# blairstar/NaturalDiffusion

Hardware: AMD Instinct MI355X
Metric: images/sec at 15-step Natural Inference (CIFAR10 32x32, NCSN++), 3-stream throughput (higher is better)
Workload: dtype bf16; 1 GPU; CIFAR10 NI 15-step step_15_weight_173.npz B=512/GPU NCSN++ 61.8M bf16, ni_step fp64 history; nfe=15, batch_per_gpu=512, streams=3

## Files before the change

### include/natinf_ncsnpp.h

```cpp
#ifndef NATINF_NCSNPP_H
#define NATINF_NCSNPP_H

#include <stdint.h>
#include "natinf.h"

#ifdef __cplusplus
extern "C" {
#endif

typedef struct natinf_ncsnpp* natinf_ncsnpp_t;

#define NATINF_NCSNPP_KEEP_ACTIVATIONS 1
#define NATINF_NCSNPP_DDPM 2

int64_t natinf_ncsnpp_param_count(void);
int64_t natinf_ncsnpp_packed_bytes(void);
int64_t natinf_ncsnpp_handle_param_count(natinf_ncsnpp_t h);
int64_t natinf_ncsnpp_handle_packed_bytes(natinf_ncsnpp_t h);
int64_t natinf_ncsnpp_workspace_bytes(natinf_ncsnpp_t h, int max_batch);

int natinf_ncsnpp_create(natinf_ncsnpp_t* out, int flags);
int natinf_ncsnpp_destroy(natinf_ncsnpp_t h);

int natinf_ncsnpp_describe(natinf_ncsnpp_t h, char* buf, int cap);

int natinf_ncsnpp_load(natinf_ncsnpp_t h, const float* params_f32, int64_t n_params,
                       void* packed, int64_t packed_bytes, natinf_stream_t stream);

int natinf_ncsnpp_share(natinf_ncsnpp_t h, natinf_ncsnpp_t loaded);

int natinf_ncsnpp_forward(natinf_ncsnpp_t h, const float* x, const float* labels, float* out, int B,
                          void* workspace, int64_t workspace_bytes, natinf_stream_t stream);

int natinf_ncsnpp_describe_gemms(natinf_ncsnpp_t h, int B, char* buf, int cap);

int natinf_debug_gemm(int variant, int M, int N, int K0, int K1, int taps, int logW, int batch,
                      const void* a0, const void* a1, const void* b, const float* bias_n, void* c, int c_f32, float scale,
                      int iters, natinf_stream_t stream);
int natinf_debug_quant_fp8_rows(const float* w, void* q, float* row_scale, int rows, int cols, natinf_stream_t stream);
int natinf_debug_gemm_fused(int variant, int M, int N, int K, const void* a, const void* b, const float* bias_n, const float* bias_m,
                            const float* rowvec, const float* gate, int log_rows_per_sample, const void* resid_bf16, const float* resid_f32,
                            float scale, int act, void* c, int c_f32, float* gn_part, int* bm_out, int fp32_slab, natinf_stream_t stream);
int natinf_debug_set_conv_operand(int logW, const void* a1, int c1);
int natinf_debug_gemm_fp8(int M, int N, int K, const void* a8, const float* a_scale, const void* a_mx, const void* b8, const float* b_scale,
                          const float* bias_n, void* c, void* c_mx, int c_mode, int iters, natinf_stream_t stream);
int natinf_debug_conv_gn_up(int flags);
int natinf_debug_conv_gn(int res, int B, int N, int cin, int c1, const void* x, const float* scale, const float* shift, const void* w_packed, void* w_frag,
                         const void* a1, const float* bias_n, const void* resid, float out_scale, void* out, float* gn_part, int iters,
                         natinf_stream_t stream);
#define NATINF_ATTN_BLOCK_OFF_WQKV 0
#define NATINF_ATTN_BLOCK_OFF_W3 393216
#define NATINF_ATTN_BLOCK_OFF_FOLD_WQK 524288
#define NATINF_ATTN_BLOCK_OFF_FOLD_WVO 786432
#define NATINF_ATTN_BLOCK_OFF_FOLD_CQ 1048576
#define NATINF_ATTN_BLOCK_OFF_FOLD_BO 1049600
#define NATINF_ATTN_BLOCK_OFF_WQK_PACKED 1050624
#define NATINF_ATTN_BLOCK_OFF_WVO_PACKED 1181696
#define NATINF_ATTN_BLOCK_PACKED_BYTES 1312768
#define NATINF_ATTN_BLOCK_SCRATCH_BYTES_PER_SAMPLE 393216
int natinf_debug_attn_block(int plan, int B, const void* x, int x_ld, const float* scale, const float* shift, const float* w, const float* bias,
                            void* packed, void* scratch, void* out, int o_ld, float out_scale, float* gn_part, natinf_stream_t stream);
int natinf_set_gemm_variant(int variant);
int natinf_set_gemm_epilogue(int fp32_slab);
int natinf_set_gemm_pref512(int on);
int natinf_set_gemm_half_issue(int on);
int natinf_set_gemm_round_model(int on);
int natinf_set_gemm_w128(int on);
int natinf_set_gemm_raster(int rows);
int natinf_set_fuse_gn(int on);
int natinf_set_conv_gn_wide(int mask);
int natinf_set_conv_gn_w128(int mask);
int natinf_set_conv_gn_w128_min_k(int shape, int k);
int natinf_set_conv_gn_regw(int on);
int natinf_set_fuse_up(int on);
int natinf_set_fuse_head(int on);
int natinf_set_fuse_gn8(int on);
int natinf_set_fuse_gn4(int on);
int natinf_set_fuse_fin(int on);
int natinf_set_conv_gn_warm(int mask);
int natinf_set_attn256(int on);
int natinf_set_attn_proj(int on);
int natinf_set_attn_waves8(int on);
int natinf_set_attn_block(int on);
int natinf_set_attn_qkv(int on);
int natinf_set_conv_gn8_tile(int one_image);
int natinf_set_gemm_splitk(int on);
int natinf_debug_set_splitk_workspace(float* ws, int max_slices);
int natinf_debug_timestamps(void* dev_buf16);

int natinf_ncsnpp_profile(natinf_ncsnpp_t h, int enable);
int natinf_ncsnpp_profile_read(natinf_ncsnpp_t h, double* ms_by_class , int64_t* launches_by_class );

int natinf_gemm_profile(int enable);
int natinf_gemm_profile_read(char* buf, int cap);

int natinf_ncsnpp_debug_tap(natinf_ncsnpp_t h, int module_idx, float* out, int64_t capacity_elems,
                            natinf_stream_t stream);

#ifdef __cplusplus
}
#endif
#endif
```

### naturaldiffusion_amd/_lib.py

```python
from __future__ import annotations

import ctypes as C
import os
from pathlib import Path

os.environ.setdefault("GPU_MAX_HW_QUEUES", "8")

_HERE = Path(__file__).resolve().parent
LIB_PATH = Path(os.environ.get("NATINF_LIB", _HERE / "libnatinf.so"))

if not LIB_PATH.exists():
    raise ImportError(
        f"{LIB_PATH} not found: build it with `make -C {_HERE / 'csrc'}` "
        "(or `python -c 'import __graft_entry__ as g; g.build()'`). "
        "naturaldiffusion_amd has no CPU or eager-PyTorch fallback.")

lib = C.CDLL(str(LIB_PATH))

_p, _i32, _i64, _f32, _f64 = C.c_void_p, C.c_int, C.c_int64, C.c_float, C.c_double

SIGNATURES = {
    "natinf_abi_version": (C.c_int, []),
    "natinf_strerror": (C.c_char_p, [_i32]),
    "natinf_probe": (C.c_int, []),
    "natinf_step_f64hist": (C.c_int, [_p, _p, _p, _p, _p, _p, _p, _i32, _f64, _i32, _f64, _f64, _f32, _f32, _i64, _p]),
    "natinf_step_f32hist": (C.c_int, [_p, _p, _p, _p, _p, _p, _p, _i32, _f32, _i32, _f32, _f32, _f32, _f32, _i64, _p]),
    "natinf_weighted_sum_f64": (C.c_int, [_p, _p, _p, _p, _i32, _i64, _p]),
    "natinf_randn_philox_f32": (C.c_int, [_p, _i64, _i64, _p, _i64, _i64, C.c_uint64, _p]),
    "natinf_randn_philox_col_f32": (C.c_int, [_p, _i64, _i64, _p, _i64, _i64, C.c_uint64, C.c_uint32, _p]),
    "natinf_step_f64hist_noise": (C.c_int, [_p, _p, _p, _p, _p, _p, _p, _i32, _f64, _p, _p, _i32, _i32, _f64, _f64, _f32,
                                            C.c_uint64, _p, _i64, _i64, _i64, _i64, _p]),
    "natinf_known_blend_f32": (C.c_int, [_p, _p, _p, _p, _i64, _i64, _f32, _f32, C.c_uint32, C.c_uint64, _p, _i64, _i64, _i64, _i64, _p]),
    "natinf_step_f64hist_inpaint": (C.c_int, [_p, _p, _p, _p, _p, _p, _p, _i32, _f64, _p, _p, _i32, _i32, _f64, _f64, _f32,
                                              C.c_uint64, _p, _i64, _i64, _i64, _i64, _p, _p, _i64, _i64, _f32, _f32, C.c_uint32, _p]),
    "natinf_color_blend_f32": (C.c_int, [_p, _p, _p, _i64, _p, _p, _f32, _f32, C.c_uint32, C.c_uint64, _p, _i64, _i64, _i64, _i64, _p]),
    "natinf_step_f64hist_colorize": (C.c_int, [_p, _p, _p, _p, _p, _p, _p, _i32, _f64, _p, _p, _i32, _i32, _f64, _f64, _f32,
                                               C.c_uint64, _p, _i64, _i64, _i64, _i64, _p, _i64, _p, _p, _f32, _f32, C.c_uint32, _p]),
    "natinf_to_pixel_u8": (C.c_int, [_p, _p, _i32, _i32, _i32, _i32, _i32, _p]),
    "natinf_step_f32prod": (C.c_int, [_p, _p, _p, _f32, _i64, _i64, _p, _p, _p, _p, _p, _i32, _f32, _p, _p, _i32,
                                      _i32, _f32, _f32, _i64, _p]),
    "natinf_step_f32prod_noise": (C.c_int, [_p, _p, _p, _f32, _i64, _i64, _p, _p, _p, _p, _p, _i32, _f32, _p, _p, _i32,
                                            _i32, _f32, _f32, C.c_uint64, _p, _i64, _i64, _i64, _p]),
    "natinf_step_f32prod_noise_guided": (C.c_int, [_p, _p, _p, _p, _p, _i32, _i64, _i64, _p, _p, _p, _p, _p, _i32, _f32, _p, _p, _i32,
                                                   _i32, _f32, _f32, C.c_uint64, _p, _i64, _i64, _i64, _p]),
    "natinf_weighted_sum_f32prod": (C.c_int, [_p, _p, _p, _p, _i32, _i64, _p]),
    "natinf_step_f16chain": (C.c_int, [_p, _p, _p, _p, _p, _p, _p, _p, _p, _i32, _f32, _f32, _i32, _f32, _f32, _f32,
                                       _f32, _i32, _i64, _p]),
    "natinf_step_f16chain_guided": (C.c_int, [_p, _p, _p, _p, _p, _i32, _i64, _p, _p, _p, _p, _p, _p, _i32, _f32, _f32, _i32, _f32, _f32,
                                              _f32, _i32, _i64, _p]),
    "natinf_weighted_mean_f16": (C.c_int, [_p, _p, _p, _p, _i32, _f32, _i64, _p]),
    "natinf_flow_input_f16": (C.c_int, [_p, _p, _p, _f32, _f32, _i64, _p]),
    "natinf_ncsnpp_param_count": (C.c_int64, []),
    "natinf_ncsnpp_workspace_bytes": (C.c_int64, [_p, _i32]),
    "natinf_ncsnpp_packed_bytes": (C.c_int64, []),
    "natinf_ncsnpp_handle_param_count": (_i64, [_p]),
    "natinf_ncsnpp_handle_packed_bytes": (_i64, [_p]),
    "natinf_ncsnpp_create": (C.c_int, [C.POINTER(_p), _i32]),
    "natinf_ncsnpp_describe": (C.c_int, [_p, C.c_char_p, _i32]),
    "natinf_ncsnpp_destroy": (C.c_int, [_p]),
    "natinf_ncsnpp_load": (C.c_int, [_p, _p, _i64, _p, _i64, _p]),
    "natinf_ncsnpp_share": (C.c_int, [_p, _p]),
    "natinf_ncsnpp_forward": (C.c_int, [_p, _p, _p, _p, _i32, _p, _i64, _p]),
    "natinf_ncsnpp_debug_tap": (C.c_int, [_p, _i32, _p, _i64, _p]),
    "natinf_ncsnpp_describe_gemms": (C.c_int, [_p, _i32, C.c_char_p, _i32]),
    "natinf_debug_gemm": (C.c_int, [_i32, _i32, _i32, _i32, _i32, _i32, _i32, _i32, _p, _p, _p, _p, _p, _i32, _f32, _i32, _p]),
    "natinf_set_gemm_variant": (C.c_int, [_i32]),
    "natinf_debug_timestamps": (C.c_int, [_p]),
    "natinf_set_gemm_epilogue": (C.c_int, [_i32]),
    "natinf_debug_gemm_fused": (C.c_int, [_i32, _i32, _i32, _i32, _p, _p, _p, _p, _p, _p, _i32, _p, _p, _f32, _i32, _p, _i32, _p, _p, _i32, _p]),
    "natinf_set_gemm_pref512": (C.c_int, [_i32]),
    "natinf_set_gemm_half_issue": (C.c_int, [_i32]),
    "natinf_set_gemm_raster": (C.c_int, [_i32]),
    "natinf_set_gemm_round_model": (C.c_int, [_i32]),
    "natinf_set_gemm_w128": (C.c_int, [_i32]),
    "natinf_set_fuse_gn": (C.c_int, [_i32]),
    "natinf_set_conv_gn_wide": (C.c_int, [_i32]),
    "natinf_set_attn_block": (C.c_int, [_i32]),
    "natinf_set_conv_gn_w128": (C.c_int, [_i32]),
    "natinf_set_conv_gn_w128_min_k": (C.c_int, [_i32, _i32]),
    "natinf_set_conv_gn_regw": (C.c_int, [_i32]),
    "natinf_set_fuse_up": (C.c_int, [_i32]),
    "natinf_set_fuse_head": (C.c_int, [_i32]),
    "natinf_set_fuse_gn8": (C.c_int, [_i32]),
    "natinf_set_fuse_gn4": (C.c_int, [_i32]),
    "natinf_set_fuse_fin": (C.c_int, [_i32]),
    "natinf_set_attn_proj": (C.c_int, [_i32]),
    "natinf_set_attn_waves8": (C.c_int, [_i32]),
    "natinf_set_attn_qkv": (C.c_int, [_i32]),
    "natinf_set_conv_gn_warm": (C.c_int, [_i32]),
    "natinf_set_attn256": (C.c_int, [_i32]),
    "natinf_set_conv_gn8_tile": (C.c_int, [_i32]),
    "natinf_set_gemm_splitk": (C.c_int, [_i32]),
    "natinf_debug_set_splitk_workspace": (C.c_int, [_p, _i32]),
    "natinf_debug_set_conv_operand": (C.c_int, [_i32, _p, _i32]),
    "natinf_debug_conv_gn": (C.c_int, [_i32, _i32, _i32, _i32, _i32, _p, _p, _p, _p, _p, _p, _p, _p, _f32, _p, _p, _i32, _p]),
    "natinf_debug_conv_gn_up": (C.c_int, [_i32]),
    "natinf_debug_attn_block": (C.c_int, [_i32, _i32, _p, _i32, _p, _p, _p, _p, _p, _p, _p, _i32, _f32, _p, _p]),
    "natinf_ncsnpp_profile": (C.c_int, [_p, _i32]),
    "natinf_ncsnpp_profile_read": (C.c_int, [_p, C.POINTER(C.c_double), C.POINTER(C.c_int64)]),
    "natinf_debug_quant_fp8_rows": (C.c_int, [_p, _p, _p, _i32, _i32, _p]),
    "natinf_debug_gemm_fp8": (C.c_int, [_i32, _i32, _i32, _p, _p, _p, _p, _p, _p, _p, _p, _i32, _i32, _p]),
    "natinf_dit_create": (C.c_int, [C.POINTER(_p), _i32, _i32, _i32, _i32]),
    "natinf_dit_create_sized": (C.c_int, [C.POINTER(_p), _i32, _i32, _i32, _i32, _i32]),
    "natinf_dit_input_size": (C.c_int, [_p]),
    "natinf_dit_attention_bf16": (C.c_int, [_p, _p, _p, _i32, _p, _i32, _i32, _i32, _i32, _i32, _i32, _p]),
    "natinf_dit_destroy": (C.c_int, [_p]),
    "natinf_dit_param_count": (C.c_int64, [_p]),
    "natinf_dit_packed_bytes": (C.c_int64, [_p]),
    "natinf_dit_workspace_bytes": (C.c_int64, [_p, _i32]),
    "natinf_dit_load": (C.c_int, [_p, _p, _i64, _p, _i64, _p]),
    "natinf_dit_forward": (C.c_int, [_p, _p, _p, _p, _p, _i32, _p, _i64, _p]),
    "natinf_dit_stream_sites": (C.c_int, [_p]),
    "natinf_dit_stream_status_reset": (C.c_int, [_p, _p, _p]),
    "natinf_dit_stream_status": (C.c_int, [_p, _p, _p, _p]),
    "natinf_mmdit_create": (C.c_int, [C.POINTER(_p), _i32, _i32, _i32, _i32, _i32, _i32, _i32, _i32]),
    "natinf_mmdit_destroy": (C.c_int, [_p]),
    "natinf_mmdit_param_count": (C.c_int64, [_p]),
    "natinf_mmdit_packed_bytes": (C.c_int64, [_p]),
    "natinf_mmdit_workspace_bytes": (C.c_int64, [_p, _i32]),
    "natinf_mmdit_load": (C.c_int, [_p, _p, _i64, _p, _i64, _p]),
    "natinf_mmdit_forward": (C.c_int, [_p, _p, _p, _p, _p, _p, _i32, _p, _i64, _p]),
    "natinf_mmdit_stream_sites": (C.c_int, [_p]),
    "natinf_mmdit_stream_status_reset": (C.c_int, [_p, _p, _p]),
    "natinf_mmdit_stream_status": (C.c_int, [_p, _p, _p, _p]),
    "natinf_attention_hd64_bf16": (C.c_int, [_p, _p, _i32, _i64, _p, _p, _i32, _i64, _i32, _i32, _i32, _i32, C.c_float, _p]),
    "natinf_inception_create": (C.c_int, [_p, _i32, _i32]),
    "natinf_inception_destroy": (C.c_int, [_p]),
    "natinf_set_inception_conv": (C.c_int, [_i32]),
    "natinf_debug_conv_ring": (C.c_int, [_i32] * 14 + [_p, _p, _p, _p, _p, _p, _i32, _p]),
    "natinf_inception_param_count": (_i64, [_p]),
    "natinf_inception_packed_bytes": (_i64, [_p]),
    "natinf_inception_workspace_bytes": (_i64, [_p, _i32]),
    "natinf_inception_load": (C.c_int, [_p, _p, _i64, _p, _i64, _p]),
    "natinf_inception_forward": (C.c_int, [_p, _p, _i32, _p, _i32, _p, _i64, _p]),
    "natinf_gemm_profile": (C.c_int, [_i32]),
    "natinf_gemm_profile_read": (C.c_int, [_p, _i32]),
    "natinf_set_mmdit_stream16": (C.c_int, [_i32]),
    "natinf_set_dit_stream16": (C.c_int, [_i32]),
    "natinf_set_mmdit_text_flat": (C.c_int, [_i32]),
    "natinf_attention_profile": (C.c_int, [_i32]),
    "natinf_set_mmdit_text_stream": (C.c_int, [_i32]),
    "natinf_set_flash_mode": (C.c_int, [_i32]),
    "natinf_attention_profile_read": (C.c_int, [_p, _p]),
    "natinf_vae_create": (C.c_int, [C.POINTER(_p), _i32, _i32]),
    "natinf_vae_destroy": (C.c_int, [_p]),
    "natinf_vae_param_count": (C.c_int64, [_p]),
    "natinf_vae_packed_bytes": (C.c_int64, [_p]),
    "natinf_vae_workspace_bytes": (C.c_int64, [_p, _i32]),
    "natinf_vae_load": (C.c_int, [_p, _p, _i64, _p, _i64, _p]),
    "natinf_vae_decode": (C.c_int, [_p, _p, _p, _i32, _p, _i64, _p]),
    "natinf_vae_enc_create": (C.c_int, [C.POINTER(_p), _i32, _i32]),
    "natinf_vae_enc_destroy": (C.c_int, [_p]),
    "natinf_vae_enc_param_count": (C.c_int64, [_p]),
    "natinf_vae_enc_packed_bytes": (C.c_int64, [_p]),
    "natinf_vae_enc_workspace_bytes": (C.c_int64, [_p, _i32]),
    "natinf_vae_enc_load": (C.c_int, [_p, _p, _i64, _p, _i64, _p]),
    "natinf_vae_posterior_f32": (C.c_int, [_p, _p, _i64, _i32, _i64, _i32, _f32, _f32, C.c_uint64, _p, _i64, _i64, _p]),
    "natinf_vae_encode": (C.c_int, [_p, _p, _p, _p, _i32, _i32, _f32, _f32, C.c_uint64, _p, _i64, _i64, _p, _i64, _p]),
}

for _name, (_res, _args) in SIGNATURES.items():
    try:
        _fn = getattr(lib, _name)
    except AttributeError as e:
        raise ImportError(f"{LIB_PATH} does not export {_name}; rebuild it") from e
    _fn.restype, _fn.argtypes = _res, _args

SD3_CFG_ON_VELOCITY = 1
DIT_UNFUSED_ATTENTION = 1
DIT_FP8 = 2
DIT_STREAM_GUARD = 16
MMDIT_FP8 = 1
MMDIT_STREAM_GUARD = 2


def check(rc: int, what: str) -> None:
    if rc != 0:
        raise RuntimeError(f"{what} failed: {lib.natinf_strerror(rc).decode()} ({rc})")


def stream_ptr(stream=None) -> int:
    import torch
    s = stream if stream is not None else torch.cuda.current_stream()
    return int(s.cuda_stream)


def ptr(t) -> int:
    return 0 if t is None else int(t.data_ptr())


class StreamGuardStatus:
    _guard_api = ""
    guard = False

    def _guard_entry(self, name):
        if not self.guard:
            raise RuntimeError("this engine was created without guard=True: it keeps no stream status")
        return getattr(lib, f"{self._guard_api}_{name}")

    @property
    def site_names(self):
        n = self._guard_entry("stream_sites")(self._h)
        check(min(n, 0), f"{self._guard_api}_stream_sites")
        return ["patch_embed"] + [f"blocks.{i // 2}.{'mlp' if i % 2 else 'attn'}" for i in range(n - 1)]

    def reset_stream_status(self) -> None:
        import torch
        with torch.cuda.device(self._ws.device):
            check(self._guard_entry("stream_status_reset")(self._h, ptr(self._ws), stream_ptr()), f"{self._guard_api}_stream_status_reset")

    def stream_status(self):
        import torch
        n = len(self.site_names)
        buf = torch.empty(2 * n, dtype=torch.int32, device=self._ws.device)
        with torch.cuda.device(self._ws.device):
            check(self._guard_entry("stream_status")(self._h, ptr(self._ws), ptr(buf), stream_ptr()), f"{self._guard_api}_stream_status")
        raw = buf.cpu().numpy().view("uint32").reshape(n, 2)
        return {"max_abs": raw[:, 0].copy().view("float32"), "clamped": raw[:, 1].copy()}


def require_gpu() -> None:
    import torch
    if not torch.cuda.is_available():
        raise RuntimeError("naturaldiffusion_amd needs an MI355X (gfx950) GPU: torch.cuda.is_available() is False "
                           "and there is no CPU fallback")
    check(lib.natinf_probe(), "natinf_probe")
```

### naturaldiffusion_amd/csrc/gemm_dma.h

```cpp
#pragma once
#include "ncsnpp_kernels.h"

#ifndef NATINF_SETPRIO
#define NATINF_SETPRIO 0
#endif

namespace ncsn {

template <int WM, int WN, int TM, int TN, int AVAIL>
struct EpiCfg {
    static constexpr int CROW = WN * TN * 16 + 4;
    static constexpr int bytes(int rb) { return WM * rb * 16 * CROW * 4; }
    static constexpr int RB = bytes(TM) <= AVAIL ? TM : (bytes(TM / 2) <= AVAIL ? TM / 2 : (bytes(TM / 4) <= AVAIL ? TM / 4 : 1));
    static constexpr int SLAB_ROWS = WM * RB * 16;
    static constexpr int SLAB_BYTES = bytes(RB);
    static_assert(TM % RB == 0 && SLAB_BYTES <= AVAIL, "epilogue staging does not fit");
    static constexpr int PROW = WN * TN * 16 * 2 + 16;
    static constexpr int PACK_SLAB = WM * TM * 16 * PROW;
    static constexpr int PACK_BYTES = PACK_SLAB + WM * WN * TN * 4 * 8;
    static constexpr bool PACK_OK = PACK_BYTES <= AVAIL;
    static constexpr int NEED = PACK_OK && PACK_BYTES > SLAB_BYTES ? PACK_BYTES : SLAB_BYTES;
};

template <int WM, int WN, int TM, int TN>
struct DmaCfg {
    static constexpr int NW = WM * WN, THREADS = NW * 64;
    static constexpr int BM_ = WM * TM * 16, BN_ = WN * TN * 16;
    static constexpr int STAGE_BYTES = (BM_ + BN_) * BK * 2;
    static constexpr int PA = BM_ / 8 / NW, PB = BN_ / 8 / NW;
    using Epi = EpiCfg<WM, WN, TM, TN, 2 * STAGE_BYTES + 8192>;
    static constexpr int LDS_BYTES = Epi::NEED > 2 * STAGE_BYTES ? Epi::NEED : 2 * STAGE_BYTES;
    static_assert(BM_ % (8 * NW) == 0 && BN_ % (8 * NW) == 0, "DMA pieces must divide evenly over the waves");
};

#ifdef NATINF_DEV
#define NATINF_TS(i) do { if (g.dbg_ts && tid == 0 && blockIdx.x == 0) g.dbg_ts[i] = __builtin_amdgcn_s_memtime(); } while (0)
#else
#define NATINF_TS(i) do { } while (0)
#endif
__device__ __forceinline__ float dpp_row_sum(float v) {
    asm volatile("s_nop 4" : "+v"(v));
    v += __builtin_bit_cast(float, __builtin_amdgcn_update_dpp(0, __builtin_bit_cast(int, v), 0xB1, 0xF, 0xF, true));
    asm volatile("" : "+v"(v));
    v += __builtin_bit_cast(float, __builtin_amdgcn_update_dpp(0, __builtin_bit_cast(int, v), 0x4E, 0xF, 0xF, true));
    asm volatile("" : "+v"(v));
    v += __builtin_bit_cast(float, __builtin_amdgcn_update_dpp(0, __builtin_bit_cast(int, v), 0x141, 0xF, 0xF, true));
    asm volatile("" : "+v"(v));
    v += __builtin_bit_cast(float, __builtin_amdgcn_update_dpp(0, __builtin_bit_cast(int, v), 0x140, 0xF, 0xF, true));
    asm volatile("" : "+v"(v));
    return v;
}
typedef __bf16 bf16x4_t __attribute__((ext_vector_type(4)));
template <class T> __device__ __forceinline__ __attribute__((address_space(1))) T* as_global(T* p) { return (__attribute__((address_space(1))) T*)p; }
typedef unsigned gu32x4 __attribute__((ext_vector_type(4)));
typedef float gf32x4 __attribute__((ext_vector_type(4)));
__device__ __forceinline__ uint4 gload_u4(const void* p) { const gu32x4 t = *as_global(reinterpret_cast<const gu32x4*>(p)); return make_uint4(t[0], t[1], t[2], t[3]); }
__device__ __forceinline__ float4 gload_f4(const void* p) { const gf32x4 t = *as_global(reinterpret_cast<const gf32x4*>(p)); return make_float4(t[0], t[1], t[2], t[3]); }
__device__ __forceinline__ void gstore_u4(void* p, uint4 v) { *as_global(reinterpret_cast<gu32x4*>(p)) = gu32x4{v.x, v.y, v.z, v.w}; }
template <int SW, int NSW, int RPS, int PROW, bool EDGE>
struct SlabCopy {
    template <class T>
    static __device__ __forceinline__ void run(const unsigned char* src, T* dst, int64_t ld, int m, int M) {
        const uint4 v = *reinterpret_cast<const uint4*>(src + SW * RPS * PROW);
        SlabCopy<SW + 1, NSW, RPS, PROW, EDGE>::run(src, dst, ld, m, M);
        if (!EDGE || m + SW * RPS < M) gstore_u4(dst + (int64_t)(SW * RPS) * ld, v);
    }
};
template <int NSW, int RPS, int PROW, bool EDGE>
struct SlabCopy<NSW, NSW, RPS, PROW, EDGE> {
    template <class T> static __device__ __forceinline__ void run(const unsigned char*, T*, int64_t, int, int) {}
};
template <int WM, int WN, int TM, int TN, class Cfg, int ACT, bool GN, bool RES, bool DEQ = false, bool OUT8 = false, int NSAMP = 1, bool FIN = false, bool PAIR = false, bool SCALE_ALWAYS = false>
__device__ __forceinline__ void packed_tile_epilogue(const GemmArgs& g, unsigned char* smem, f32x4 (&acc)[TM][TN],
                                                     int m0, int n0, int z, int tid, int lane, int wm, int wn)
{
    constexpr int BN_ = WN * TN * 16, BM_ = WM * TM * 16, THREADS = WM * WN * 64, PROW = OUT8 ? BN_ + 16 : Cfg::PROW;
    static_assert(!OUT8 || (!GN && !RES && TN % 2 == 0), "fp8 output: plain column terms only");
    static_assert(!PAIR || (TN % 2 == 0 && !OUT8 && !DEQ), "interleaved n-tile pairs: bf16 output");
    static_assert(NSAMP == 1 || ((NSAMP == 2 || NSAMP == 4) && WM == 1 && TM % NSAMP == 0 && !DEQ && !OUT8), "several samples per tile: one wave row, bf16 output");
    constexpr bool ACT8 = (ACT == ACT_GELU_TANH || ACT == ACT_SILU) && !GN && TN % 2 == 0 && NSAMP == 1;
    const int r = lane & 15, q = lane >> 4;
    auto ncol = [&](int j) __attribute__((always_inline)) { return PAIR ? 32 * (j >> 1) + 8 * q + 4 * (j & 1) : 16 * j + 4 * q; };
    float dn[DEQ ? TN : 1][4], rsc[DEQ ? TM : 1], rbm[DEQ ? TM : 1];
    if constexpr (DEQ) {
#pragma unroll
        for (int j = 0; j < TN; ++j) {
            const int n = n0 + wn * TN * 16 + j * 16 + q * 4;
            float4 d = make_float4(1.f, 1.f, 1.f, 1.f);
            if (g.deq_n && n < g.N) d = *reinterpret_cast<const float4*>(g.deq_n + (int64_t)z * g.deq_n_bs + n);
            dn[j][0] = d.x; dn[j][1] = d.y; dn[j][2] = d.z; dn[j][3] = d.w;
        }
#pragma unroll
        for (int i = 0; i < TM; ++i) {
            const int m = min(m0 + wm * TM * 16 + i * 16 + r, g.M - 1);
            rsc[i] = g.deq_m ? g.deq_m[(int64_t)z * g.deq_m_bs + m] : 1.f;
            rbm[i] = g.bias_m ? g.bias_m[m] : 0.f;
        }
    }
    constexpr bool LAZY_RV = NSAMP > 2 && !RES;
    constexpr int NCT = (NSAMP > 1 && !RES && !LAZY_RV) ? NSAMP : 1;
    float ct[NCT][TN][4];
#pragma unroll
    for (int sm = 0; sm < NCT; ++sm)
#pragma unroll
    for (int j = 0; j < TN; ++j) {
        const int n = n0 + wn * TN * 16 + ncol(j);
        float4 b = make_float4(0.f, 0.f, 0.f, 0.f), rv = make_float4(0.f, 0.f, 0.f, 0.f);
        if (n < g.N) {
            if (g.bias_n) b = gload_f4(g.bias_n + n);
            const int srow = NSAMP > 1 ? min(m0 + sm * (BM_ / NSAMP), g.M - 1) : m0;
            if (g.rowvec && !LAZY_RV) rv = gload_f4(g.rowvec + (int64_t)((srow >> g.log_rows_per_sample) + z * g.z_samples) * g.rowvec_ld + n);
        }
        ct[sm][j][0] = b.x + rv.x; ct[sm][j][1] = b.y + rv.y; ct[sm][j][2] = b.z + rv.z; ct[sm][j][3] = b.w + rv.w;
    }
    uint2 rs[RES ? TM : 1][RES ? TN : 1];
    if constexpr (RES) {
        const bf16* rb = g.resid + (int64_t)z * g.c_bs + n0 + wn * TN * 16;
#pragma unroll
        for (int i = 0; i < TM; ++i) {
            const int m = min(m0 + wm * TM * 16 + i * 16 + r, g.M - 1);
            if constexpr (PAIR) {
#pragma unroll
                for (int p = 0; p < TN / 2; ++p) {
                    const uint4 v = n0 + wn * TN * 16 + ncol(2 * p) < g.N ? gload_u4(rb + (int64_t)m * g.resid_ld + ncol(2 * p)) : make_uint4(0u, 0u, 0u, 0u);
                    rs[i][2 * p] = make_uint2(v.x, v.y); rs[i][2 * p + 1] = make_uint2(v.z, v.w);
                }
            } else {
#pragma unroll
                for (int j = 0; j < TN; ++j)
                    rs[i][j] = n0 + wn * TN * 16 + ncol(j) < g.N ? *reinterpret_cast<const uint2*>(rb + (int64_t)m * g.resid_ld + ncol(j)) : make_uint2(0u, 0u);
            }
        }
    }
    float gs[NSAMP][TN], gq[NSAMP][TN];
#pragma unroll
    for (int sm = 0; sm < NSAMP; ++sm)
#pragma unroll
        for (int j = 0; j < TN; ++j) { gs[sm][j] = 0.f; gq[sm][j] = 0.f; }
    const float scale = g.scale;
    float4 lrv[LAZY_RV ? TN : 1];
    auto fetch_rowvec = [&](int i) __attribute__((always_inline)) {
        if constexpr (LAZY_RV) {
            const int srow = min(m0 + (i / (TM / NSAMP)) * (BM_ / NSAMP), g.M - 1);
#pragma unroll
            for (int j = 0; j < TN; ++j) {
                const int n = n0 + wn * TN * 16 + ncol(j);
                lrv[j] = (g.rowvec && n < g.N) ? *reinterpret_cast<const float4*>(g.rowvec + (int64_t)(srow >> g.log_rows_per_sample) * g.rowvec_ld + n) : make_float4(0.f, 0.f, 0.f, 0.f);
            }
        }
    };
    auto value = [&](int i, int j, float (&v)[4]) __attribute__((always_inline)) {
        const int sm = NSAMP > 1 ? i / (TM / NSAMP) : 0;
        const int sc_ = NCT > 1 ? sm : 0;
#pragma unroll
        for (int e = 0; e < 4; ++e) {
            if constexpr (DEQ) v[e] = __builtin_fmaf(acc[i][j][e] * rsc[i], dn[j][e], ct[sc_][j][e]);
            else v[e] = acc[i][j][e] + ct[sc_][j][e];
        }
        if constexpr (DEQ && !OUT8) {
            if (g.bias_m) {
                asm volatile("");
#pragma unroll
                for (int e = 0; e < 4; ++e) v[e] += rbm[i];
            }
        }
        if constexpr (LAZY_RV) { v[0] += lrv[j].x; v[1] += lrv[j].y; v[2] += lrv[j].z; v[3] += lrv[j].w; }
        if constexpr (RES) {
            const bf16x4_t x = __builtin_bit_cast(bf16x4_t, rs[i][j]);
#pragma unroll
            for (int e = 0; e < 4; ++e) v[e] += (float)x[e];
        }
        if constexpr (SCALE_ALWAYS) {
#pragma unroll
            for (int e = 0; e < 4; ++e) v[e] *= scale;
        } else if (!OUT8 && scale != 1.0f) {
            asm volatile("");
#pragma unroll
            for (int e = 0; e < 4; ++e) v[e] *= scale;
        }
        if constexpr (ACT != ACT_NONE && !ACT8) apply_act4(v, ACT);
        if constexpr (GN) {
            gs[sm][j] += (v[0] + v[1]) + (v[2] + v[3]);
            gq[sm][j] += (v[0] * v[0] + v[1] * v[1]) + (v[2] * v[2] + v[3] * v[3]);
        }
    };
    auto act8 = [&](float (&v0)[4], float (&v1)[4]) __attribute__((always_inline)) {
        float v8[8] = {v0[0], v0[1], v0[2], v0[3], v1[0], v1[1], v1[2], v1[3]};
        if constexpr (ACT == ACT_GELU_TANH) gelu_tanh_fast8(v8); else silu_fast8(v8);
#pragma unroll
        for (int e = 0; e < 4; ++e) { v0[e] = v8[e]; v1[e] = v8[4 + e]; }
    };
    constexpr int EB = OUT8 ? 1 : 2;
    unsigned char* wbase = smem + (wm * TM * 16 + r) * PROW + (wn * TN * 16 + q * 4) * EB;
    if constexpr (!OUT8 && PAIR) {
        unsigned char* wb2 = smem + (wm * TM * 16 + r) * PROW + (wn * TN * 16) * 2;
#pragma unroll
        for (int i = 0; i < TM; ++i) {
            fetch_rowvec(i);
#pragma unroll
            for (int p = 0; p < TN / 2; ++p) {
                float v0[4], v1[4];
                value(i, 2 * p, v0);
                value(i, 2 * p + 1, v1);
                if constexpr (ACT8) act8(v0, v1);
                bf16x4_t o0, o1;
#pragma unroll
                for (int e = 0; e < 4; ++e) { o0[e] = (bf16)v0[e]; o1[e] = (bf16)v1[e]; }
                const uint2 a = __builtin_bit_cast(uint2, o0), b = __builtin_bit_cast(uint2, o1);
                *reinterpret_cast<uint4*>(wb2 + i * 16 * PROW + ncol(2 * p) * 2) = make_uint4(a.x, a.y, b.x, b.y);
            }
        }
    } else if constexpr (!OUT8) {
#pragma unroll
        for (int i = 0; i < TM; ++i) {
            fetch_rowvec(i);
            if constexpr (ACT8) {
#pragma unroll
                for (int j = 0; j < TN; j += 2) {
                    float v0[4], v1[4];
                    value(i, j, v0);
                    value(i, j + 1, v1);
                    act8(v0, v1);
                    bf16x4_t o0, o1;
#pragma unroll
                    for (int e = 0; e < 4; ++e) { o0[e] = (bf16)v0[e]; o1[e] = (bf16)v1[e]; }
                    *reinterpret_cast<uint2*>(wbase + i * 16 * PROW + j * 32) = __builtin_bit_cast(uint2, o0);
                    *reinterpret_cast<uint2*>(wbase + i * 16 * PROW + (j + 1) * 32) = __builtin_bit_cast(uint2, o1);
                }
            } else {
#pragma unroll
            for (int j = 0; j < TN; ++j) {
                float v[4];
                value(i, j, v);
                bf16x4_t o;
#pragma unroll
                for (int e = 0; e < 4; ++e) o[e] = (bf16)v[e];
                *reinterpret_cast<uint2*>(wbase + i * 16 * PROW + j * 32) = __builtin_bit_cast(uint2, o);
            }
            }
        }
    } else {
#pragma unroll
        for (int i = 0; i < TM; ++i) {
            const int m = m0 + wm * TM * 16 + i * 16 + r;
            unsigned e8pair = 0;
#pragma unroll
            for (int b = 0; b < TN / 2; ++b) {
                float v0[4], v1[4];
                value(i, 2 * b, v0);
                value(i, 2 * b + 1, v1);
                if constexpr (ACT8) act8(v0, v1);
                float amax = fmaxf(fmaxf(fmaxf(fabsf(v0[0]), fabsf(v0[1])), fmaxf(fabsf(v0[2]), fabsf(v0[3]))),
                                   fmaxf(fmaxf(fabsf(v1[0]), fabsf(v1[1])), fmaxf(fabsf(v1[2]), fabsf(v1[3]))));
                amax = group4_max_nonneg(amax);
                float inv;
                const unsigned e8 = mx_scale_of(amax, inv);
                *reinterpret_cast<unsigned*>(wbase + i * 16 * PROW + (2 * b) * 16) = pack_fp8x4<false>(v0[0] * inv, v0[1] * inv, v0[2] * inv, v0[3] * inv);
                *reinterpret_cast<unsigned*>(wbase + i * 16 * PROW + (2 * b + 1) * 16) = pack_fp8x4<false>(v1[0] * inv, v1[1] * inv, v1[2] * inv, v1[3] * inv);
                e8pair |= e8 << (8 * b);
            }
            static_assert(TN == 4, "scale bytes are stored as one 16-bit pair per row and wave");
            const int nb = n0 + wn * 64;
            if (q == 0 && m < g.M && nb < g.N)
                *reinterpret_cast<unsigned short*>(g.c_mx + (int64_t)z * g.c_mx_bs + ((int64_t)(nb >> 7) * g.c_mx_ld + m) * 4 + ((nb >> 5) & 3)) = (unsigned short)e8pair;
        }
    }
    float2* const sred = reinterpret_cast<float2*>(smem + Cfg::PACK_SLAB);
    if constexpr (GN) {
#pragma unroll
        for (int sm = 0; sm < NSAMP; ++sm)
#pragma unroll
            for (int j = 0; j < TN; ++j) { gs[sm][j] = dpp_row_sum(gs[sm][j]); gq[sm][j] = dpp_row_sum(gq[sm][j]); }
        if (r == 0) {
#pragma unroll
            for (int sm = 0; sm < NSAMP; ++sm)
#pragma unroll
                for (int j = 0; j < TN; ++j) sred[(NSAMP > 1 ? sm : wm) * (BN_ / 4) + wn * TN * 4 + (ncol(j) >> 2)] = make_float2(gs[sm][j], gq[sm][j]);
        }
    }
    __syncthreads();
    NATINF_TS(3);
    constexpr int CPR = BN_ * EB / 16, RPS = THREADS / CPR, NSW = BM_ / RPS;
    const int cchunk = tid % CPR, rsub = tid / CPR, n = n0 + cchunk * (16 / EB);
    if (n < g.N) {
        const unsigned char* src = smem + rsub * PROW + cchunk * 16;
        if constexpr (OUT8) {
            uint8_t* dst = reinterpret_cast<uint8_t*>(g.c) + (int64_t)z * g.c_bs + (int64_t)(m0 + rsub) * g.c_ld + n;
            if (m0 + BM_ <= g.M) SlabCopy<0, NSW, RPS, PROW, false>::run(src, dst, g.c_ld, m0 + rsub, g.M);
            else SlabCopy<0, NSW, RPS, PROW, true>::run(src, dst, g.c_ld, m0 + rsub, g.M);
        } else {
            bf16* dst = reinterpret_cast<bf16*>(g.c) + (int64_t)z * g.c_bs + (int64_t)(m0 + rsub) * g.c_ld + n;
            if (m0 + BM_ <= g.M) SlabCopy<0, NSW, RPS, PROW, false>::run(src, dst, g.c_ld, m0 + rsub, g.M);
            else SlabCopy<0, NSW, RPS, PROW, true>::run(src, dst, g.c_ld, m0 + rsub, g.M);
        }
    }
    NATINF_TS(4);
    if constexpr (GN) {
        if (tid < BN_ / 4 && n0 + tid * 4 < g.N) {
            if constexpr (NSAMP > 1) {
#pragma unroll
                for (int sm = 0; sm < NSAMP; ++sm)
                    if (m0 + sm * (BM_ / NSAMP) < g.M)
                        reinterpret_cast<float2*>(g.gn_part)[(int64_t)((m0 / BM_) * NSAMP + sm) * g.gn_quads + (n0 >> 2) + tid] = sred[sm * (BN_ / 4) + tid];
            } else {
                float s = 0.f, qq = 0.f;
#pragma unroll
                for (int w = 0; w < WM; ++w) { s += sred[w * (BN_ / 4) + tid].x; qq += sred[w * (BN_ / 4) + tid].y; }
                reinterpret_cast<float2*>(g.gn_part)[(int64_t)(m0 / BM_) * g.gn_quads + (n0 >> 2) + tid] = make_float2(s, qq);
            }
        }
        if constexpr (FIN) {
            static_assert((WM == 1 || NSAMP == 1) && BN_ <= THREADS, "one channel per thread; several samples per tile: one wave row");
            const int n = n0 + tid;
            if (g.fin_scale && tid < BN_ && n < g.N) {
                constexpr int HWS = BM_ / NSAMP;
                const int cg = g.fin_cg, qpg = cg >> 2, q0 = (n / cg) * qpg - (n0 >> 2);
                const float inv = 1.0f / (float)(cg * HWS), ga = g.fin_gamma[n], be = g.fin_beta[n];
#pragma unroll
                for (int sm = 0; sm < NSAMP; ++sm) {
                    if (m0 + sm * HWS >= g.M) break;
                    float s = 0.f, qq = 0.f;
                    for (int i = 0; i < qpg; ++i) {
                        if constexpr (NSAMP == 1 && WM > 1) {
                            float ps = 0.f, pq = 0.f;
#pragma unroll
                            for (int w = 0; w < WM; ++w) { ps += sred[w * (BN_ / 4) + q0 + i].x; pq += sred[w * (BN_ / 4) + q0 + i].y; }
                            s += ps; qq += pq;
                        } else { const float2 v = sred[sm * (BN_ / 4) + q0 + i]; s += v.x; qq += v.y; }
                    }
                    const float mean = s * inv;
                    float var = qq * inv - mean * mean;
                    var = var < 0.f ? 0.f : var;
                    const float sc = (1.0f / sqrtf(var + g.fin_eps)) * ga;
                    const int64_t o = (int64_t)(m0 / HWS + sm) * g.fin_ld + n;
                    g.fin_scale[o] = sc * g.fin_mul;
                    g.fin_shift[o] = (be - mean * sc) * g.fin_mul;
                }
            }
        }
    }
}

template <int WM, int WN, int TM, int TN, class Cfg>
__device__ __forceinline__ void dma_tile_epilogue(const GemmArgs& g, unsigned char* smem, f32x4 (&acc)[TM][TN],
                                                  int m0, int n0, int z, int tid, int lane, int wm, int wn)
{
    constexpr int BN_ = WN * TN * 16, BM_ = WM * TM * 16, THREADS = WM * WN * 64;
    float* sC = reinterpret_cast<float*>(smem);
    NATINF_TS(2);
#ifdef NATINF_DEV
    if (g.c_mode == 102) {
        float t = 0.f;
#pragma unroll
        for (int i = 0; i < TM; ++i)
#pragma unroll
            for (int j = 0; j < TN; ++j) t += acc[i][j][0] + acc[i][j][1] + acc[i][j][2] + acc[i][j][3];
        if (t == 123.456f) reinterpret_cast<float*>(g.c)[tid] = t;
        return;
    }
#endif
    float st[4] = {0.f, 0.f, 0.f, 0.f};
    constexpr int CROW = Cfg::CROW, RB = Cfg::RB, CPR = BN_ / 8;
    constexpr int ROWS_PER_SWEEP = THREADS / CPR;
    constexpr int NP = TM / RB, NSW = Cfg::SLAB_ROWS / ROWS_PER_SWEEP;
    uint4 keep[NSW][2];
    const int cchunk = tid % CPR, rsub = tid / CPR;
    const int n = n0 + cchunk * 8;
    const bool n_in = n < g.N;
    float bn[8];
#pragma unroll
    for (int q = 0; q < 8; ++q) bn[q] = 0.f;
    if (g.bias_n && n_in && g.c_mode != OUT_F32_NCHW) {
        const float4 u = *reinterpret_cast<const float4*>(g.bias_n + n), w = *reinterpret_cast<const float4*>(g.bias_n + n + 4);
        bn[0] = u.x; bn[1] = u.y; bn[2] = u.z; bn[3] = u.w; bn[4] = w.x; bn[5] = w.y; bn[6] = w.z; bn[7] = w.w;
    }
    float dn[8];
#pragma unroll
    for (int q = 0; q < 8; ++q) dn[q] = 1.f;
    if (g.deq_n && n_in) {
        const float* pd = g.deq_n + (int64_t)z * g.deq_n_bs + n;
        const float4 u = *reinterpret_cast<const float4*>(pd), w = *reinterpret_cast<const float4*>(pd + 4);
        dn[0] = u.x; dn[1] = u.y; dn[2] = u.z; dn[3] = u.w; dn[4] = w.x; dn[5] = w.y; dn[6] = w.z; dn[7] = w.w;
    }
    asm volatile("s_waitcnt vmcnt(0)" : "+v"(dn[0]), "+v"(dn[1]), "+v"(dn[2]), "+v"(dn[3]), "+v"(dn[4]), "+v"(dn[5]), "+v"(dn[6]), "+v"(dn[7]));
    asm volatile("s_waitcnt vmcnt(0)" : "+v"(bn[0]), "+v"(bn[1]), "+v"(bn[2]), "+v"(bn[3]), "+v"(bn[4]), "+v"(bn[5]), "+v"(bn[6]), "+v"(bn[7]));
#pragma unroll
    for (int pass = 0; pass < NP; ++pass) {
        if (pass) __syncthreads();
#pragma unroll
        for (int ii = 0; ii < RB; ++ii)
#pragma unroll
            for (int j = 0; j < TN; ++j)
                *reinterpret_cast<f32x4*>(sC + (wm * RB * 16 + ii * 16 + (lane & 15)) * CROW + wn * TN * 16 + j * 16 + (lane >> 4) * 4) = acc[pass * RB + ii][j];
        __syncthreads();
        NATINF_TS(3 + 3 * pass);
        if (g.c_mode == OUT_F32_NCHW) {
            float* out = reinterpret_cast<float*>(g.c);
            const int nvalid = min(BN_, g.N - n0);
            for (int e = tid; e < Cfg::SLAB_ROWS * nvalid; e += THREADS) {
                const int s = e % Cfg::SLAB_ROWS, nn = e / Cfg::SLAB_ROWS;
                const int m = m0 + (s / (RB * 16)) * (TM * 16) + pass * RB * 16 + s % (RB * 16);
                if (m < g.M) {
                    float v = sC[s * CROW + nn];
                    if (g.bias_n) v += g.bias_n[n0 + nn];
                    v *= g.scale;
                    const int b = m >> g.logHW, p = m & ((1 << g.logHW) - 1);
                    out[((int64_t)b * g.N + n0 + nn) * ((int64_t)1 << g.logHW) + p] = v;
                }
            }
            continue;
        }
#pragma unroll
        for (int sw = 0; sw < NSW; ++sw) {
            const int s = sw * ROWS_PER_SWEEP + rsub;
            const int m = m0 + (s / (RB * 16)) * (TM * 16) + pass * RB * 16 + s % (RB * 16);
            if (m >= g.M || !n_in) continue;
            const float4 u = *reinterpret_cast<const float4*>(sC + s * CROW + cchunk * 8);
            const float4 w = *reinterpret_cast<const float4*>(sC + s * CROW + cchunk * 8 + 4);
            float v[8] = {u.x, u.y, u.z, u.w, w.x, w.y, w.z, w.w};
            if (g.deq_m || g.deq_n) {
                const float dm = g.deq_m ? g.deq_m[(int64_t)z * g.deq_m_bs + m] : 1.f;
#pragma unroll
                for (int q = 0; q < 8; ++q) v[q] *= dm * dn[q];
            }
#pragma unroll
            for (int q = 0; q < 8; ++q) v[q] += bn[q];
            if (g.bias_m) {
                const float bm = g.bias_m[m];
#pragma unroll
                for (int q = 0; q < 8; ++q) v[q] += bm;
            }
            if (g.rowvec) {
                const float* rv = g.rowvec + (int64_t)((m >> g.log_rows_per_sample) + z * g.z_samples) * g.rowvec_ld + n;
                const float4 s4 = *reinterpret_cast<const float4*>(rv), t4 = *reinterpret_cast<const float4*>(rv + 4);
                v[0] += s4.x; v[1] += s4.y; v[2] += s4.z; v[3] += s4.w; v[4] += t4.x; v[5] += t4.y; v[6] += t4.z; v[7] += t4.w;
            }
            if (g.gate) {
                const float* gv = g.gate + (int64_t)((m >> g.log_rows_per_sample) + z * g.z_samples) * g.gate_ld + n;
                const float4 s4 = *reinterpret_cast<const float4*>(gv), t4 = *reinterpret_cast<const float4*>(gv + 4);
                v[0] *= s4.x; v[1] *= s4.y; v[2] *= s4.z; v[3] *= s4.w; v[4] *= t4.x; v[5] *= t4.y; v[6] *= t4.z; v[7] *= t4.w;
            }
            if (g.resid) {
                const bf16x8 rs = *reinterpret_cast<const bf16x8*>(g.resid + (int64_t)z * g.c_bs + (int64_t)m * g.resid_ld + n);
#pragma unroll
                for (int q = 0; q < 8; ++q) v[q] += (float)rs[q];
            }
            if (g.resid_f32) {
                const float* rp = g.resid_f32 + (int64_t)z * g.c_bs + (int64_t)m * g.resid_f32_ld + n;
                const float4 s4 = *reinterpret_cast<const float4*>(rp), t4 = *reinterpret_cast<const float4*>(rp + 4);
                v[0] += s4.x; v[1] += s4.y; v[2] += s4.z; v[3] += s4.w; v[4] += t4.x; v[5] += t4.y; v[6] += t4.z; v[7] += t4.w;
            }
#pragma unroll
            for (int q = 0; q < 8; ++q) v[q] *= g.scale;
            apply_act8(v, g.act);
            if (g.gn_part) {
                st[0] += (v[0] + v[1]) + (v[2] + v[3]); st[1] += (v[0] * v[0] + v[1] * v[1]) + (v[2] * v[2] + v[3] * v[3]);
                st[2] += (v[4] + v[5]) + (v[6] + v[7]); st[3] += (v[4] * v[4] + v[5] * v[5]) + (v[6] * v[6] + v[7] * v[7]);
            }
            if (g.c_mode == OUT_BF16) {
                bf16x8 o;
#pragma unroll
// ... 41 lines not shown
    if (g.gn_part) {
        __syncthreads();
        float* sred = reinterpret_cast<float*>(smem);
        *reinterpret_cast<float4*>(sred + (rsub * CPR + cchunk) * 4) = make_float4(st[0], st[1], st[2], st[3]);
        __syncthreads();
        if (tid < CPR * 2 && n0 + tid * 4 < g.N) {
            const int ch = tid >> 1, hf = (tid & 1) * 2;
            float s = 0.f, q = 0.f;
#pragma unroll 4
            for (int r = 0; r < ROWS_PER_SWEEP; ++r) { s += sred[(r * CPR + ch) * 4 + hf]; q += sred[(r * CPR + ch) * 4 + hf + 1]; }
            reinterpret_cast<float2*>(g.gn_part)[(int64_t)(m0 / BM_) * g.gn_quads + (n0 >> 2) + tid] = make_float2(s, q);
        }
    }
}

template <int WM, int WN, int TM, int TN, bool DEQ = false, int HI_ = 0, bool GUARD = false>
__device__ __forceinline__ void direct_f32_epilogue(const GemmArgs& g, f32x4 (&acc)[TM][TN], int m0, int n0, int z, int lane, int wm, int wn)
{
    const int r = lane & 15, q = lane >> 4;
    const int64_t sample = (int64_t)((m0 >> g.log_rows_per_sample) + z * g.z_samples);
    float ct[TN][4], gt[TN][4];
    float dn[DEQ ? TN : 1][4], rsc[DEQ ? TM : 1];
    if constexpr (DEQ) {
#pragma unroll
        for (int j = 0; j < TN; ++j) {
            const int n = n0 + wn * TN * 16 + j * 16 + q * 4;
            float4 d = make_float4(1.f, 1.f, 1.f, 1.f);
            if (g.deq_n && n < g.N) d = *reinterpret_cast<const float4*>(g.deq_n + (int64_t)z * g.deq_n_bs + n);
            dn[j][0] = d.x; dn[j][1] = d.y; dn[j][2] = d.z; dn[j][3] = d.w;
        }
#pragma unroll
        for (int i = 0; i < TM; ++i)
            rsc[i] = g.deq_m ? g.deq_m[(int64_t)z * g.deq_m_bs + min(m0 + wm * TM * 16 + i * 16 + r, g.M - 1)] : 1.f;
    }
    bool n_ok[TN];
#pragma unroll
    for (int j = 0; j < TN; ++j) {
        const int n = n0 + wn * TN * 16 + j * 16 + q * 4;
        n_ok[j] = n < g.N;
        float4 b = make_float4(0.f, 0.f, 0.f, 0.f), rv = make_float4(0.f, 0.f, 0.f, 0.f), gv = make_float4(1.f, 1.f, 1.f, 1.f);
        if (n_ok[j]) {
            if (g.bias_n) b = gload_f4(g.bias_n + n);
            if (g.rowvec) rv = *reinterpret_cast<const float4*>(g.rowvec + sample * g.rowvec_ld + n);
            if (g.gate) gv = *reinterpret_cast<const float4*>(g.gate + sample * g.gate_ld + n);
        }
        ct[j][0] = b.x + rv.x; ct[j][1] = b.y + rv.y; ct[j][2] = b.z + rv.z; ct[j][3] = b.w + rv.w;
        gt[j][0] = gv.x; gt[j][1] = gv.y; gt[j][2] = gv.z; gt[j][3] = gv.w;
    }
    const float scale = g.scale;
    const int64_t eoff = (int64_t)z * g.c_bs + n0 + wn * TN * 16 + q * 4;
    constexpr int HI = HI_ > 0 ? HI_ : (DEQ ? (TM > 2 ? 2 : TM) : (TM > 4 ? TM / 2 : TM));
    typedef _Float16 f16x4_ds __attribute__((ext_vector_type(4)));
    StreamGuardAcc ga;
    auto sweep = [&](auto f16_tag) __attribute__((always_inline)) {
        constexpr bool F16 = decltype(f16_tag)::value;
        const float* rb = g.resid_f32 + eoff;
        float* cb = reinterpret_cast<float*>(g.c) + eoff;
        const _Float16* rbh = reinterpret_cast<const _Float16*>(g.resid_f32) + eoff;
        _Float16* cbh = reinterpret_cast<_Float16*>(g.c) + eoff;
#pragma unroll
        for (int h = 0; h < TM / HI; ++h) {
            f32x4 rs[F16 ? 1 : HI][F16 ? 1 : TN];
            uint2 rh[F16 ? HI : 1][F16 ? TN : 1];
#pragma unroll
            for (int i = 0; i < HI; ++i) {
                const int m = min(m0 + wm * TM * 16 + (h * HI + i) * 16 + r, g.M - 1);
#pragma unroll
                for (int j = 0; j < TN; ++j) {
                    if constexpr (F16) rh[i][j] = n_ok[j] ? *reinterpret_cast<const uint2*>(rbh + (int64_t)m * g.resid_f32_ld + j * 16) : make_uint2(0u, 0u);
                    else rs[i][j] = n_ok[j] ? *reinterpret_cast<const f32x4*>(rb + (int64_t)m * g.resid_f32_ld + j * 16) : f32x4{0.f, 0.f, 0.f, 0.f};
                }
            }
#pragma unroll
            for (int i = 0; i < HI; ++i) {
                const int m = m0 + wm * TM * 16 + (h * HI + i) * 16 + r;
#pragma unroll
                for (int j = 0; j < TN; ++j) {
                    f32x4 v;
                    f16x4_ds xh;
                    if constexpr (F16) xh = __builtin_bit_cast(f16x4_ds, rh[i][j]);
#pragma unroll
                    for (int e = 0; e < 4; ++e) {
                        const float a0 = DEQ ? acc[h * HI + i][j][e] * (rsc[h * HI + i] * dn[j][e]) : acc[h * HI + i][j][e];
                        float x_;
                        if constexpr (F16) x_ = (float)xh[e]; else x_ = rs[i][j][e];
                        v[e] = ((a0 + ct[j][e]) * gt[j][e] + x_) * scale;
                    }
                    if (m < g.M && n_ok[j]) {
                        if constexpr (GUARD) {
#pragma unroll
                            for (int e = 0; e < 4; ++e) v[e] = stream_guard_value<F16>(ga, v[e]);
                        }
                        if constexpr (F16) {
                            const f16x4_ds o = {(_Float16)v[0], (_Float16)v[1], (_Float16)v[2], (_Float16)v[3]};
                            *reinterpret_cast<uint2*>(cbh + (int64_t)m * g.c_ld + j * 16) = __builtin_bit_cast(uint2, o);
                        } else *reinterpret_cast<f32x4*>(cb + (int64_t)m * g.c_ld + j * 16) = v;
                    }
                }
            }
        }
    };
    auto sweep16 = [&]() __attribute__((always_inline)) {
        static_assert(TN % 2 == 0 || TN == 1, "tile pairs");
        const int jt_off = (q & 1) * 16 + (q >> 1) * 8 - q * 4;
        const _Float16* rbh = reinterpret_cast<const _Float16*>(g.resid_f32) + eoff + jt_off;
        _Float16* cbh = reinterpret_cast<_Float16*>(g.c) + eoff + jt_off;
        constexpr int NP = TN / 2 > 0 ? TN / 2 : 1;
#pragma unroll
        for (int h = 0; h < TM / HI; ++h) {
            uint4 rq[HI][NP];
#pragma unroll
            for (int i = 0; i < HI; ++i) {
                const int m = min(m0 + wm * TM * 16 + (h * HI + i) * 16 + r, g.M - 1);
#pragma unroll
                for (int p = 0; p < NP; ++p) rq[i][p] = *reinterpret_cast<const uint4*>(rbh + (int64_t)m * g.resid_f32_ld + p * 32);
            }
#pragma unroll
            for (int i = 0; i < HI; ++i) {
                const int m = m0 + wm * TM * 16 + (h * HI + i) * 16 + r;
#pragma unroll
                for (int p = 0; p < NP; ++p) {
                    auto s0 = __builtin_amdgcn_permlane16_swap(rq[i][p].x, rq[i][p].z, false, false);
                    auto s1 = __builtin_amdgcn_permlane16_swap(rq[i][p].y, rq[i][p].w, false, false);
                    const f16x4_ds x0 = __builtin_bit_cast(f16x4_ds, make_uint2(s0[0], s1[0])), x1 = __builtin_bit_cast(f16x4_ds, make_uint2(s0[1], s1[1]));
                    f16x4_ds o0, o1;
#pragma unroll
                    for (int e = 0; e < 4; ++e) {
                        const float a0 = DEQ ? acc[h * HI + i][2 * p][e] * (rsc[h * HI + i] * dn[2 * p][e]) : acc[h * HI + i][2 * p][e];
                        const float a1 = DEQ ? acc[h * HI + i][2 * p + 1][e] * (rsc[h * HI + i] * dn[2 * p + 1][e]) : acc[h * HI + i][2 * p + 1][e];
                        float v0 = ((a0 + ct[2 * p][e]) * gt[2 * p][e] + (float)x0[e]) * scale, v1 = ((a1 + ct[2 * p + 1][e]) * gt[2 * p + 1][e] + (float)x1[e]) * scale;
                        if constexpr (GUARD) {
                            if (m < g.M) { v0 = stream_guard_value<true>(ga, v0); v1 = stream_guard_value<true>(ga, v1); }
                        }
                        o0[e] = (_Float16)v0;
                        o1[e] = (_Float16)v1;
                    }
                    const uint2 u0 = __builtin_bit_cast(uint2, o0), u1 = __builtin_bit_cast(uint2, o1);
                    auto t0 = __builtin_amdgcn_permlane16_swap(u0.x, u1.x, false, false);
                    auto t1 = __builtin_amdgcn_permlane16_swap(u0.y, u1.y, false, false);
                    if (m < g.M) *reinterpret_cast<uint4*>(cbh + (int64_t)m * g.c_ld + p * 32) = make_uint4(t0[0], t1[0], t0[1], t1[1]);
                }
            }
        }
    };
    if (g.stream_f16) {
        bool wide = false;
        if constexpr (TN % 2 == 0) wide = n0 + (wn + 1) * TN * 16 <= g.N && g.resid_f32_ld % 8 == 0 && g.c_ld % 8 == 0;
        if (wide) { if constexpr (TN % 2 == 0) sweep16(); }
        else sweep(std::integral_constant<bool, true>{});
    } else sweep(std::integral_constant<bool, false>{});
    if constexpr (GUARD) stream_guard_commit(ga, g.stream_guard);
}

template <int WM, int WN, int TM, int TN, class Cfg, int EPI, int NSAMP = 1, bool FIN = false, bool PAIR = false>
__device__ __forceinline__ void tile_epilogue(const GemmArgs& g, unsigned char* smem, f32x4 (&acc)[TM][TN],
                                              int m0, int n0, int z, int tid, int lane, int wm, int wn)
{
    if constexpr (EPI == 0) dma_tile_epilogue<WM, WN, TM, TN, Cfg>(g, smem, acc, m0, n0, z, tid, lane, wm, wn);
    else if constexpr (EPI == 7) direct_f32_epilogue<WM, WN, TM, TN>(g, acc, m0, n0, z, lane, wm, wn);
    else if constexpr (EPI == 10) direct_f32_epilogue<WM, WN, TM, TN, false, 0, true>(g, acc, m0, n0, z, lane, wm, wn);
    else {
        static_assert(Cfg::PACK_OK, "packed epilogue needs the whole bf16 tile in LDS");
        NATINF_TS(2);
        packed_tile_epilogue<WM, WN, TM, TN, Cfg, EPI == 3 ? ACT_SILU : (EPI == 4 ? ACT_GELU_TANH : ACT_NONE), EPI == 2 || EPI == 6, EPI == 5 || EPI == 6, EPI == 8, false, NSAMP, FIN && (EPI == 2 || EPI == 6), PAIR>(
            g, smem, acc, m0, n0, z, tid, lane, wm, wn);
    }
}

typedef unsigned u32x4 __attribute__((ext_vector_type(4)));
template <int OFF> __device__ __forceinline__ u32x4 lds_read16(unsigned addr) {
    u32x4 v;
    asm volatile(NATINF_PAD_PRE "ds_read_b128 %0, %1 offset:%2" NATINF_PAD_POST : "=v"(v) : "v"(addr), "n"(OFF) : "memory");
    return v;
}
template <int N> __device__ __forceinline__ void wait_lgkmcnt() {
    asm volatile("s_waitcnt lgkmcnt(%0)" :: "n"(N) : "memory");
    __builtin_amdgcn_sched_barrier(0);
}
constexpr int pipe_lgkm_after(int TM, int st) {
    int n = 6, pos_fa[40] = {4, 5}, pos_fb1_last = -1;
    for (int s = 0; s <= st; ++s) {
        if (s + 2 < 2 * TM) pos_fa[s + 2] = n++;
        if (s / TM == 0 && s % TM >= TM - 4) pos_fb1_last = n++;
    }
    int need = pos_fa[st];
    if (st >= TM && pos_fb1_last > need) need = pos_fb1_last;
    return n - 1 - need;
}
template <int TM, int ST>
struct PipeStep {
    static __device__ __forceinline__ void run(u32x4 (&fa)[3], u32x4 (&fb)[2][4], f32x4 (&acc)[TM][4],
                                               unsigned a0, unsigned a1, unsigned b1) {
        constexpr int S = 2 * TM, ks = ST / TM, i = ST % TM;
        if constexpr (ST + 2 < S) {
            constexpr int ks2 = (ST + 2) / TM, i2 = (ST + 2) % TM;
            fa[(ST + 2) % 3] = lds_read16<i2 * 2048>(ks2 ? a1 : a0);
        }
        if constexpr (ks == 0 && i >= TM - 4) fb[1][i - (TM - 4)] = lds_read16<(i - (TM - 4)) * 2048>(b1);
        wait_lgkmcnt<pipe_lgkm_after(TM, ST)>();
#pragma unroll
        for (int j = 0; j < 4; ++j)
            acc[i][j] = __builtin_amdgcn_mfma_f32_16x16x32_bf16(__builtin_bit_cast(bf16x8, fb[ks][j]),
                                                                __builtin_bit_cast(bf16x8, fa[ST % 3]), acc[i][j], 0, 0, 0);
        if constexpr (ST + 1 < S) PipeStep<TM, ST + 1>::run(fa, fb, acc, a0, a1, b1);
    }
};

template <int WM, int WN, int TM, int TN, int SPREAD = 0, int EPI = 0>
__global__ __launch_bounds__(WM * WN * 64, 2) void k_gemm_dma(const GemmArgs g)
{
    static_assert(SPREAD == 2 || SPREAD == 6, "the shipped K loops: hand pipeline (2), one issuing wave per SIMD (6)");
    using Cfg = DmaCfg<WM, WN, TM, TN>;
    constexpr int BM_ = Cfg::BM_, BN_ = Cfg::BN_, THREADS = Cfg::THREADS;
    extern __shared__ __attribute__((aligned(16))) unsigned char smem[];
    lds_poison();
    const int tid = threadIdx.x, lane = tid & 63;
    const int wave = __builtin_amdgcn_readfirstlane(tid >> 6);
    const int wm = wave / WN, wn = wave % WN;
    const int nN = (g.N + BN_ - 1) / BN_, nM = (g.M + BM_ - 1) / BM_;
    const int tile = xcd_remap(blockIdx.x, nM * nN);
    NATINF_TS(0);
    int mt_, nt_;
    tile_coords(tile, nM, nN, g.raster_g, mt_, nt_);
    const int m0 = mt_ * BM_, n0 = nt_ * BN_;
    const int z = blockIdx.z;

    const bf16* a0 = g.a0 + (int64_t)z * g.a_bs;
    const bf16* a1 = g.a1 ? g.a1 + (int64_t)z * g.a_bs : nullptr;
    const bf16* bp = g.b + (int64_t)z * g.b_bs;
    const int K0 = g.taps * g.a0_C, K1 = g.a1 ? g.a1_C : 0;
    const int nk0 = K0 / BK, nk = nk0 + K1 / BK;
    const int Wp = (1 << g.logW) + 2, Hp = (1 << (g.logHW - g.logW)) + 2;

    constexpr bool HALF = SPREAD == 6;
    constexpr int PAI = HALF ? 2 * Cfg::PA : Cfg::PA, PBI = HALF ? 2 * Cfg::PB : Cfg::PB;
    const bool issuer = !HALF || wave < Cfg::NW / 2;
    uint64_t a_row[PAI], a_delta[PAI], b_row[PBI];
    typedef __attribute__((address_space(3))) void lds_void;
    const int64_t ashift0 = g.taps == 9 ? (int64_t)(-Wp - 1) * g.a0_ld * 2 : 0;
#pragma unroll
    for (int j = 0; j < PAI; ++j) {
        const int r = (wave * PAI + j) * 8 + (lane >> 3);
        const int lchunk = ((lane & 7) ^ ((r >> 1) & 7)) << 3;
        const int m = min(m0 + r, g.M - 1);
        int64_t off0;
        if (g.taps == 9) {
            const int b = m >> g.logHW, p = m & ((1 << g.logHW) - 1), y = p >> g.logW, x = p & ((1 << g.logW) - 1);
            off0 = ((int64_t)(b * Hp + y + 1) * Wp + x + 1) * g.a0_ld;
        } else {
            off0 = (int64_t)m * g.a0_ld;
        }
        a_row[j] = reinterpret_cast<uint64_t>(a0 + off0 + lchunk);
        a_delta[j] = a1 ? reinterpret_cast<uint64_t>(a1 + (int64_t)m * g.a1_ld + lchunk) - a_row[j] : 0;
        if (issuer)
            __builtin_amdgcn_global_load_lds(reinterpret_cast<const void*>(a_row[j] + (uint64_t)ashift0),
                                             (lds_void*)(smem + wave * (PAI * 1024) + j * 1024), 16, 0, 0);
    }
#pragma unroll
    for (int j = 0; j < PBI; ++j) {
        const int r = (wave * PBI + j) * 8 + (lane >> 3);
        const int lchunk = ((lane & 7) ^ ((r >> 1) & 7)) << 3;
        b_row[j] = reinterpret_cast<uint64_t>(bp + (int64_t)min(n0 + r, g.N - 1) * g.b_ld + lchunk);
        if (issuer)
            __builtin_amdgcn_global_load_lds(reinterpret_cast<const void*>(b_row[j]), (lds_void*)(smem + BM_ * BK * 2 + wave * (PBI * 1024) + j * 1024), 16, 0, 0);
    }

    f32x4 acc[TM][TN];
#pragma unroll
    for (int i = 0; i < TM; ++i)
#pragma unroll
        for (int j = 0; j < TN; ++j) acc[i][j] = f32x4{0.f, 0.f, 0.f, 0.f};

    asm volatile("s_waitcnt vmcnt(0)" ::: "memory");
    __syncthreads();
    NATINF_TS(1);

    const int frow = lane & 15, fq = lane >> 4, fswz = (frow >> 1) & 7;
    constexpr int NP = PAI + PBI;
    for (int kt = 0; kt < nk; ++kt) {
        const int cur = kt & 1;
        const bool more = kt + 1 < nk;
        const int kn = kt + 1;
        const bool seg0n = kn < nk0;
        int64_t ashiftn; int kkn;
        if (seg0n) {
            int tap = 0, c0 = kn * BK;
            if (g.taps == 9) { const int cch = kn / 9; tap = kn - 9 * cch; c0 = cch * BK; }
            const int dy = g.taps == 9 ? tap / 3 - 1 : 0, dx = g.taps == 9 ? tap % 3 - 1 : 0;
            ashiftn = ((int64_t)(dy * Wp + dx) * g.a0_ld + c0) * 2; kkn = kn * BK;
        } else {
            ashiftn = (int64_t)(kn - nk0) * BK * 2; kkn = K0 + (kn - nk0) * BK;
        }
        unsigned char* dAn = smem + (cur ^ 1) * Cfg::STAGE_BYTES + wave * (PAI * 1024);
        unsigned char* dBn = smem + (cur ^ 1) * Cfg::STAGE_BYTES + BM_ * BK * 2 + wave * (PBI * 1024);
        auto issue_piece = [&](int p) __attribute__((always_inline)) {
            if (p < PAI) {
                const uint64_t pa = a_row[p] + (seg0n ? 0 : a_delta[p]) + (uint64_t)ashiftn;
                __builtin_amdgcn_global_load_lds(reinterpret_cast<const void*>(pa), (lds_void*)(dAn + p * 1024), 16, 0, 0);
            } else {
                const uint64_t pb = b_row[p - PAI] + (uint64_t)kkn * 2;
                __builtin_amdgcn_global_load_lds(reinterpret_cast<const void*>(pb), (lds_void*)(dBn + (p - PAI) * 1024), 16, 0, 0);
            }
        };
        if (more && issuer) {
#pragma unroll
            for (int p = 0; p < NP; ++p) issue_piece(p);
        }
        const bf16* ta = reinterpret_cast<const bf16*>(smem + cur * Cfg::STAGE_BYTES) + (wm * TM * 16 + frow) * LDS_ROW;
        const bf16* tb = reinterpret_cast<const bf16*>(smem + cur * Cfg::STAGE_BYTES + BM_ * BK * 2) + (wn * TN * 16 + frow) * LDS_ROW;
        {
            static_assert(TN == 4, "the hand-counted pipeline is written for TN = 4");
            typedef __attribute__((address_space(3))) unsigned char lds_u8;
            const unsigned a_lds = (unsigned)(uintptr_t)((lds_u8*)(unsigned char*)const_cast<bf16*>(ta));
            const unsigned b_lds = (unsigned)(uintptr_t)((lds_u8*)(unsigned char*)const_cast<bf16*>(tb));
            const unsigned ko0 = ((0 | fq) ^ fswz) << 4, ko1 = ((4 | fq) ^ fswz) << 4;
            u32x4 fa[3], fb[2][4];
            fb[0][0] = lds_read16<0>(b_lds + ko0); fb[0][1] = lds_read16<2048>(b_lds + ko0);
            fb[0][2] = lds_read16<4096>(b_lds + ko0); fb[0][3] = lds_read16<6144>(b_lds + ko0);
            fa[0] = lds_read16<0>(a_lds + ko0); fa[1] = lds_read16<2048>(a_lds + ko0);
            PipeStep<TM, 0>::run(fa, fb, acc, a_lds + ko0, a_lds + ko1, b_lds + ko1);
        }
        asm volatile("s_waitcnt vmcnt(0)" ::: "memory");
        __syncthreads();
    }
    tile_epilogue<WM, WN, TM, TN, typename Cfg::Epi, EPI>(g, smem, acc, m0, n0, z, tid, lane, wm, wn);
}


template <int WM, int WN, int TM, int TN, int NS>
struct RingCfg {
    static constexpr int BKR = 32;
    static constexpr int NW = WM * WN, THREADS = NW * 64;
    static constexpr int BM_ = WM * TM * 16, BN_ = WN * TN * 16;
    static constexpr int STAGE_BYTES = (BM_ + BN_) * BKR * 2;
    static constexpr int PA = BM_ / 16 / NW, PB = BN_ / 16 / NW;
    static constexpr int DPT = PA + PB;
    using Epi = EpiCfg<WM, WN, TM, TN, NS * STAGE_BYTES + 4096>;
    static constexpr int LDS_BYTES = Epi::NEED > NS * STAGE_BYTES ? Epi::NEED : NS * STAGE_BYTES;
    static_assert(BM_ % (16 * NW) == 0 && BN_ % (16 * NW) == 0, "DMA pieces must divide evenly over the waves");
    static_assert((NS - 2) * DPT <= 63 && NS >= 3, "vmcnt immediate is 6 bits");
};

template <int N> __device__ __forceinline__ void wait_vmcnt_barrier() {
    asm volatile("s_waitcnt vmcnt(%0)\n\ts_barrier" :: "n"(N) : "memory");
}

template <int WM, int WN, int TM, int TN, int NS, int EPI = 0>
__global__ __launch_bounds__(WM * WN * 64, 2) void k_gemm_ring(const GemmArgs g)
{
    using Cfg = RingCfg<WM, WN, TM, TN, NS>;
    constexpr int BM_ = Cfg::BM_, BN_ = Cfg::BN_, BKR = Cfg::BKR, ROW = 32;
    extern __shared__ __attribute__((aligned(16))) unsigned char smem[];
    lds_poison();
    const int tid = threadIdx.x, lane = tid & 63;
    const int wave = __builtin_amdgcn_readfirstlane(tid >> 6);
    const int wm = wave / WN, wn = wave % WN;
    const int nN = (g.N + BN_ - 1) / BN_, nM = (g.M + BM_ - 1) / BM_;
    const int tile = xcd_remap(blockIdx.x, nM * nN);
    int mt_, nt_;
    tile_coords(tile, nM, nN, g.raster_g, mt_, nt_);
    const int m0 = mt_ * BM_, n0 = nt_ * BN_;
    const int z = EPI == 9 ? 0 : blockIdx.z;

    const bf16* a0 = g.a0 + (int64_t)z * g.a_bs;
    const bf16* a1 = g.a1 ? g.a1 + (int64_t)z * g.a_bs : nullptr;
    const bf16* bp = g.b + (int64_t)z * g.b_bs;
    const int K0 = g.taps * g.a0_C, K1 = g.a1 ? g.a1_C : 0;
    const int nk0 = K0 / BKR, nk_all = nk0 + K1 / BKR;
    const int Wp = (1 << g.logW) + 2, Hp = (1 << (g.logHW - g.logW)) + 2;
    const int kt_lo = EPI == 9 ? (int)((int64_t)nk_all * blockIdx.z / g.splitk) : 0;
    const int nk = EPI == 9 ? (int)((int64_t)nk_all * (blockIdx.z + 1) / g.splitk) - kt_lo : nk_all;

    uint64_t a_row[Cfg::PA], a_delta[Cfg::PA], b_row[Cfg::PB];
#pragma unroll
    for (int j = 0; j < Cfg::PA; ++j) {
        const int r = (wave * Cfg::PA + j) * 16 + (lane >> 2);
        const int t4 = (r >> 2) & 3;
        const int lchunk = ((lane & 3) ^ ((0x1320 >> (t4 * 4)) & 3)) << 3;
        const int m = min(m0 + r, g.M - 1);
        int64_t off0;
        if (g.taps == 9) {
            const int b = m >> g.logHW, p = m & ((1 << g.logHW) - 1), y = p >> g.logW, x = p & ((1 << g.logW) - 1);
            off0 = ((int64_t)(b * Hp + y + 1) * Wp + x + 1) * g.a0_ld;
        } else {
            off0 = (int64_t)m * g.a0_ld;
        }
        a_row[j] = reinterpret_cast<uint64_t>(a0 + off0 + lchunk);
        a_delta[j] = a1 ? reinterpret_cast<uint64_t>(a1 + (int64_t)m * g.a1_ld + lchunk) - a_row[j] : 0;
    }
#pragma unroll
    for (int j = 0; j < Cfg::PB; ++j) {
        const int r = (wave * Cfg::PB + j) * 16 + (lane >> 2);
        const int t4 = (r >> 2) & 3;
        const int lchunk = ((lane & 3) ^ ((0x1320 >> (t4 * 4)) & 3)) << 3;
        b_row[j] = reinterpret_cast<uint64_t>(bp + (int64_t)min(n0 + r, g.N - 1) * g.b_ld + lchunk);
    }

    typedef __attribute__((address_space(3))) void lds_void;
    auto issue_tile = [&](int kt_rel) __attribute__((always_inline)) {
        const int slot = kt_rel % NS, kt = kt_lo + kt_rel;
        unsigned char* dA = smem + slot * Cfg::STAGE_BYTES + wave * (Cfg::PA * 1024);
        unsigned char* dB = smem + slot * Cfg::STAGE_BYTES + BM_ * BKR * 2 + wave * (Cfg::PB * 1024);
        const bool seg0 = kt < nk0;
        int64_t ashift;
        if (seg0) {
            int tap = 0, c0 = kt * BKR;
            if (g.taps == 9) { const int q = kt >> 1, cch = q / 9; tap = q - 9 * cch; c0 = cch * 64 + (kt & 1) * BKR; }
            const int dy = g.taps == 9 ? tap / 3 - 1 : 0, dx = g.taps == 9 ? tap % 3 - 1 : 0;
            ashift = ((int64_t)(dy * Wp + dx) * g.a0_ld + c0) * 2;
        } else {
            ashift = (int64_t)(kt - nk0) * BKR * 2;
        }
        const uint64_t kk2 = (uint64_t)kt * BKR * 2;
#pragma unroll
        for (int j = 0; j < Cfg::PA; ++j) {
            const uint64_t pa = a_row[j] + (seg0 ? 0 : a_delta[j]) + (uint64_t)ashift;
            __builtin_amdgcn_global_load_lds(reinterpret_cast<const void*>(pa), (lds_void*)(dA + j * 1024), 16, 0, 0);
        }
#pragma unroll
        for (int j = 0; j < Cfg::PB; ++j)
            __builtin_amdgcn_global_load_lds(reinterpret_cast<const void*>(b_row[j] + kk2), (lds_void*)(dB + j * 1024), 16, 0, 0);
    };

    f32x4 acc[TM][TN];
#pragma unroll
    for (int i = 0; i < TM; ++i)
#pragma unroll
        for (int j = 0; j < TN; ++j) acc[i][j] = f32x4{0.f, 0.f, 0.f, 0.f};

#pragma unroll
    for (int t = 0; t < NS - 1; ++t)
        if (t < nk) issue_tile(t);

    const int frow = lane & 15, fq = lane >> 4;
    const int fko = (fq ^ ((0x1320 >> (((frow >> 2) & 3) * 4)) & 3)) << 3;
    for (int kt = 0; kt < nk; ++kt) {
        if (kt + NS - 1 <= nk) wait_vmcnt_barrier<(NS - 2) * Cfg::DPT>();
        else                   wait_vmcnt_barrier<0>();
        if (kt + NS - 1 < nk) issue_tile(kt + NS - 1);
        const int slot = kt % NS;
        const bf16* ta = reinterpret_cast<const bf16*>(smem + slot * Cfg::STAGE_BYTES) + (wm * TM * 16 + frow) * ROW + fko;
        const bf16* tb = reinterpret_cast<const bf16*>(smem + slot * Cfg::STAGE_BYTES + BM_ * BKR * 2) + (wn * TN * 16 + frow) * ROW + fko;
        bf16x8 fb[TN];
#pragma unroll
        for (int j = 0; j < TN; ++j) fb[j] = *reinterpret_cast<const bf16x8*>(tb + j * 16 * ROW);
#if NATINF_SETPRIO
        __builtin_amdgcn_s_setprio(1);
#endif
#pragma unroll
        for (int i = 0; i < TM; ++i) {
            const bf16x8 fa = *reinterpret_cast<const bf16x8*>(ta + i * 16 * ROW);
#pragma unroll
            for (int j = 0; j < TN; ++j)
                acc[i][j] = __builtin_amdgcn_mfma_f32_16x16x32_bf16(fb[j], fa, acc[i][j], 0, 0, 0);
        }
#if NATINF_SETPRIO
        __builtin_amdgcn_s_setprio(0);
#endif
    }
    __syncthreads();
    if constexpr (EPI == 9) {
        float* part = reinterpret_cast<float*>(g.c) + (int64_t)blockIdx.z * g.M * g.N;
        const int r = lane & 15, q = lane >> 4;
#pragma unroll
        for (int i = 0; i < TM; ++i) {
            const int m = m0 + wm * TM * 16 + i * 16 + r;
#pragma unroll
            for (int j = 0; j < TN; ++j) {
                const int n = n0 + wn * TN * 16 + j * 16 + q * 4;
                if (m < g.M && n < g.N) *reinterpret_cast<f32x4*>(part + (int64_t)m * g.N + n) = acc[i][j];
            }
        }
    } else {
        tile_epilogue<WM, WN, TM, TN, typename Cfg::Epi, EPI>(g, smem, acc, m0, n0, z, tid, lane, wm, wn);
    }
}

constexpr int SPLITK_ROWS = 16;
__global__ __launch_bounds__(256) void k_splitk_reduce(const float* __restrict__ part, int S, int M, int N, const float* __restrict__ bias_n,
// ... 57 lines not shown
```

### naturaldiffusion_amd/csrc/gemm_launch.h

```cpp
#pragma once
#include <hip/hip_runtime.h>
#include <stdint.h>
#include <stdio.h>
#include <string.h>
#include <string>
#include <type_traits>
#include <utility>
#include <vector>

#include "ncsnpp_kernels.h"
#include "gemm_dma.h"
#include "gemm_w128.h"
#include "conv_gn2.h"
#include "gemm_fp8.h"

using namespace ncsn;

bool configure_conv_ring();
namespace { bool configure_ncsnpp_kernels();
            bool configure_dit_attention();
            bool configure_flash_attention(); }
namespace ncsn_sg { bool configure(); bool has_tile(int variant); void launch_tile(const void* gemm_args, int variant, int raster, void* stream);
                    void launch_fp8(const void* gemm_args, int mxa, int w128, int raster, void* stream); void launch_splitk_reduce(const void* gemm_args, int slices, void* stream);
                    void launch_patch_embed(const float* z, const float* Wt, const float* bias, const float* pos, float* x, int C, int g, int D, int64_t rows, int x_f16, uint32_t* guard, void* stream); }
namespace ncsn_cg3 { bool configure(); int tile_rows(int shape); int tile_cols(int shape); void launch(const void* gemm_args, int shape, int epi, void* stream); }

namespace {

int g_epi_fp32_slab = 0;
GemmArgs gemm_defaults() {
    GemmArgs g;
    memset(&g, 0, sizeof(g));
    g.epi_fp32_slab = g_epi_fp32_slab;
    g.taps = 1; g.batch = 1; g.scale = 1.0f; g.act = ACT_NONE; g.c_mode = OUT_BF16;
    return g;
}
constexpr int NUM_CU = 256;
enum GemmVariant {
    V_AUTO = 0, V_GENERIC = 1,
    V_DMA_256x256 = 2, V_DMA_256x128 = 3, V_DMA_128x128 = 4,
    V_RING_256x256 = 5, V_RING_256x128 = 6, V_RING_128x128 = 7,
    V_RING_64x128 = 8,
    V_RING_256x128_W4 = 9,
    V_DMA_256x128_W4 = 10,
    V_DMA_256x256_S = 11, V_DMA_128x128_S = 12,
    V_DMA_512x128 = 13,
    V_PATCH_256x256 = 14, V_PATCH_256x128 = 15,
    V_DMA_256x256_P = 16, V_DMA_256x128W4_P = 18,
    V_DMA_128x128_P = 17,
    V_8PH_256x256 = 19, V_8PH_NOPRIO = 20, V_8PH_READFIRST = 21, V_8PH_BOTH = 22,
    V_FP8_256x256 = 23,
    V_ABL_NODMA = 24, V_ABL_NOMFMA = 25,
    V_DMA_256x256_H = 26, V_DMA_512x128_H = 27,
    V_CONV_GN = 28,
    V_W128 = 29,
    V_W128_A = 30, V_W128_D = 31, V_W128_X = 32,
    V_COUNT
};
const char* variant_name(int v) {
    static const char* n[] = {"auto", "generic128", "dma256x256", "dma256x128", "dma128x128", "ring256x256", "ring256x128",
                              "ring128x128", "ring64x128", "ring256x128w4", "dma256x128w4", "dma256x256s", "dma128x128s", "dma512x128", "patch256x256", "patch256x128", "dma256x256p", "dma128x128p", "dma256x128w4p", "gemm8ph", "gemm8ph_np", "gemm8ph_rf", "gemm8ph_nprf", "fp8_256x256", "abl_nodma", "abl_nomfma", "dma256x256h", "dma512x128h", "conv_gn", "w128_256x256", "w128_a", "w128_d", "w128_x"};
    return v >= 0 && v < V_COUNT ? n[v] : "?";
}
unsigned long long* g_dbg_ts = nullptr;
int g_force_variant = V_AUTO;
int g_round_model = 1;
int g_round_model_w128 = 13;
int g_pref_512 = 1;
std::string* g_record = nullptr;

int g_raster_g = 8;
template <class Cfg, class K>
inline void launch_tiles(K kernel, const GemmArgs& g0, hipStream_t s) {
    const int nM = (g0.M + Cfg::BM_ - 1) / Cfg::BM_, nN = (g0.N + Cfg::BN_ - 1) / Cfg::BN_;
    GemmArgs g = g0;
    g.raster_g = (g_raster_g > 1 && nN >= 8 && nM >= g_raster_g) ? g_raster_g : 0;
    hipLaunchKernelGGL(kernel, dim3(nM * nN, 1, g.batch), dim3(Cfg::THREADS), Cfg::LDS_BYTES, s, g);
}
template <class Cfg, class K>
inline bool set_lds(K kernel) {
    return hipFuncSetAttribute(reinterpret_cast<const void*>(kernel), hipFuncAttributeMaxDynamicSharedMemorySize, Cfg::LDS_BYTES) == hipSuccess;
}
int g_cg_warm = 15;

constexpr unsigned EPI_ALL = 0x1FF;
template <unsigned MASK, int E, class F> inline void epi_case(F&& f) { if constexpr ((MASK >> E) & 1u) f(std::integral_constant<int, E>{}); }
template <unsigned MASK, class F> inline bool for_each_epi(F&& f) {
    bool ok = true;
    auto one = [&](auto tag) { ok = ok && f(tag); };
    epi_case<MASK, 0>(one); epi_case<MASK, 1>(one); epi_case<MASK, 2>(one); epi_case<MASK, 3>(one); epi_case<MASK, 4>(one);
    epi_case<MASK, 5>(one); epi_case<MASK, 6>(one); epi_case<MASK, 7>(one); epi_case<MASK, 8>(one);
    return ok;
}
#define NATINF_EPI_OF(tag) decltype(tag)::value

template <class... F> struct FamList {};
template <class Fam> bool configure_family() {
    return for_each_epi<Fam::EPI>([](auto t) { return set_lds<typename Fam::Cfg>(Fam::template kernel<NATINF_EPI_OF(t)>()); });
}
template <class... F> bool configure_families(FamList<F...>) { return (configure_family<F>() && ...); }
template <class Fam> void launch_family(int e, const GemmArgs& g, hipStream_t s) {
    for_each_epi<Fam::EPI>([&](auto t) {
        if (NATINF_EPI_OF(t) != e) return true;
        launch_tiles<typename Fam::Cfg>(Fam::template kernel<NATINF_EPI_OF(t)>(), g, s);
        return false;
    });
}

using CfgD256x256 = DmaCfg<2, 4, 8, 4>;
struct FamD128  { static constexpr int V = V_DMA_128x128_P;    using Cfg = DmaCfg<2, 2, 4, 4>;     static constexpr unsigned EPI = EPI_ALL;
                  template <int E> static constexpr auto kernel() { return &k_gemm_dma<2, 2, 4, 4, 2, E>; } };
struct FamRW4   { static constexpr int V = V_RING_256x128_W4;  using Cfg = RingCfg<2, 2, 8, 4, 3>; static constexpr unsigned EPI = EPI_ALL & ~(1u << 3);
                  template <int E> static constexpr auto kernel() { return &k_gemm_ring<2, 2, 8, 4, 3, E>; } };
struct FamR64   { static constexpr int V = V_RING_64x128;      using Cfg = RingCfg<2, 2, 2, 4, 4>; static constexpr unsigned EPI = EPI_ALL;
                  template <int E> static constexpr auto kernel() { return &k_gemm_ring<2, 2, 2, 4, 4, E>; } };
struct FamD256H { static constexpr int V = V_DMA_256x256_H;    using Cfg = CfgD256x256;            static constexpr unsigned EPI = EPI_ALL & ~(1u << 3);
                  template <int E> static constexpr auto kernel() { return &k_gemm_dma<2, 4, 8, 4, 6, E>; } };
struct FamD512H { static constexpr int V = V_DMA_512x128_H;    using Cfg = DmaCfg<4, 2, 8, 4>;     static constexpr unsigned EPI = EPI_ALL & ~((1u << 3) | (1u << 4) | (1u << 7) | (1u << 8));
                  template <int E> static constexpr auto kernel() { return &k_gemm_dma<4, 2, 8, 4, 6, E>; } };
struct FamW128  { static constexpr int V = V_W128;             using Cfg = W128Cfg;                static constexpr unsigned EPI = EPI_ALL & ~((1u << 2) | (1u << 3) | (1u << 6));
                  template <int E> static constexpr auto kernel() { return &k_gemm_w128<E>; } };
using GemmFamilies = FamList<FamD128, FamRW4, FamR64, FamD256H, FamD512H, FamW128>;
using CfgR128x128 = RingCfg<2, 2, 4, 4, 4>;

template <class F, class... Fam> constexpr bool with_family(int v, F&& f, FamList<Fam...>) { return ((v == Fam::V && (f(Fam{}), true)) || ...); }
template <class F> constexpr bool with_family(int v, F&& f) { return with_family(v, f, GemmFamilies{}); }
constexpr bool variant_shipped(int v) {
    return v == V_AUTO || v == V_GENERIC || v == V_FP8_256x256 || v == V_CONV_GN || with_family(v, [](auto) {});
}
constexpr unsigned epi_mask(int v) { unsigned m = 1u; with_family(v, [&](auto f) { m = decltype(f)::EPI; }); return m; }
constexpr int variant_bm(int v) {
    int bm = (v == V_CONV_GN || v == V_FP8_256x256) ? 256 : 128;
    with_family(v, [&](auto f) { bm = decltype(f)::Cfg::BM_; });
    return bm;
}
static_assert(variant_bm(V_RING_64x128) == 64 && variant_bm(V_DMA_128x128_P) == 128 && variant_bm(V_RING_256x128_W4) == 256 && variant_bm(V_DMA_256x256_H) == 256 &&
              variant_bm(V_DMA_512x128_H) == 512 && variant_bm(V_W128) == 256 && variant_bm(V_GENERIC) == 128, "the block-tile rows choose_variant and the GroupNorm partial tables count on");
static_assert(variant_shipped(V_W128) && !variant_shipped(V_DMA_256x256) && !variant_shipped(V_W128_X) && epi_mask(V_GENERIC) == 1u, "retired ids stay refused");

constexpr unsigned EPI_CONV_GN = (1u << 1) | (1u << 2) | (1u << 5) | (1u << 6);
template <int RES_, bool WIDE, int TM = 8, int NG = 1, int TN = 4> struct CgShape {
    static constexpr int RES = RES_; using Cfg = ConvGn2Cfg<RES_, WIDE, TM, NG, TN>; static constexpr unsigned EPI = EPI_CONV_GN;
    template <int E> static constexpr auto kernel() { return &k_conv_gn2<RES_, WIDE, E, TM, NG, TN>; }
    static bool takes(int res, int bm) { return res == RES_ && (RES_ <= 8 || WIDE == (bm == 128)); }
};
using CgH4T = CgShape<4, true, 4, 2, 2>;
using ConvGnShapes = FamList<CgShape<32, false>, CgShape<32, true>, CgShape<16, false>, CgShape<16, true>, CgShape<8, true, 4>, CgH4T>;
template <class... S> void launch_conv_gn2(FamList<S...>, int res, int bm, int e, const GemmArgs& g, hipStream_t s) {
    ((S::takes(res, bm) && (launch_family<S>(e, g, s), true)) || ...);
}

constexpr unsigned EPI_FP8 = 0xF;
template <bool MXA> struct FamF8     { using Cfg = CfgD256x256; static constexpr unsigned EPI = EPI_FP8; template <int E> static constexpr auto kernel() { return &k_gemm_fp8<MXA, E>; } };
template <bool MXA> struct FamF8W128 { using Cfg = W128F8Cfg;   static constexpr unsigned EPI = EPI_FP8; template <int E> static constexpr auto kernel() { return &k_gemm_w128_fp8<MXA, E>; } };
using Fp8Families = FamList<FamF8<false>, FamF8<true>, FamF8W128<false>, FamF8W128<true>>;

bool configure_gemm_kernels() {
    bool ok = hipFuncSetAttribute(reinterpret_cast<const void*>(&k_gemm_bf16), hipFuncAttributeMaxDynamicSharedMemorySize,
                                  GEMM_LDS_BYTES) == hipSuccess;
    ok = ok && set_lds<CfgR128x128>(&k_gemm_ring<2, 2, 4, 4, 4, 9>) && set_lds<W128Cfg>(&k_gemm_w128<9>) &&
         configure_families(GemmFamilies{}) && configure_families(ConvGnShapes{}) && configure_families(Fp8Families{}) &&
         ncsn_cg3::configure() && ncsn_sg::configure() && ::configure_conv_ring() && configure_ncsnpp_kernels() && configure_dit_attention() && configure_flash_attention();
    if (!ok) (void)hipGetLastError();
    return ok;
}


int packed_epi(const GemmArgs& g, int bm);
int g_cg3 = 7;
int g_cg_wide = 3;
int g_cg3_min_k[3] = {2304, 0, 2304};
inline int conv_gn3_shape(const GemmArgs& g) {
    const int res = 1 << g.logW;
    if (!g_cg3 || !g.b_frag || g.N % 128) return -1;
    int sh = -1;
    if (res == 32) sh = g.N % 256 ? ((g_cg3 & 1) ? 0 : -1) : ((g_cg3 & 2) ? 1 : -1);
    else if (res == 16) sh = (g.N % 256 == 0 && (g_cg3 & 4)) ? 2 : -1;
    if (sh >= 0 && 9 * g.a0_C + (g.a1 ? g.a1_C : 0) < g_cg3_min_k[sh]) sh = -1;
    return sh;
}
inline int conv_gn_bm(const GemmArgs& g) {
    const int res = 1 << g.logW;
    if (const int sh3 = conv_gn3_shape(g); sh3 >= 0) return ncsn_cg3::tile_rows(sh3);
    if (res == 8 || res == 4) return 64;
    if (res == 32) return ((g_cg_wide & 2) && g.N % 256 == 0 && g.b_frag) ? 128 : 256;
    return ((g_cg_wide & 1) && res == 16 && g.N % 256 == 0) ? 128 : 256;
}
inline int conv_gn_part_rows(const GemmArgs& g) { const int res = 1 << g.logW; return res <= 8 ? res * res : conv_gn_bm(g); }
inline bool conv_gn_regw(const GemmArgs& g) { return g.b_frag && (conv_gn3_shape(g) >= 0 || g.N % ((conv_gn_bm(g) <= 128 && (1 << g.logW) != 4) ? 256 : 128) == 0); }
inline int conv_gn_epi(const GemmArgs& g) { GemmArgs t = g; t.epi_fp32_slab = 0; return packed_epi(t, conv_gn_part_rows(g)); }
inline bool conv_gn_ok(const GemmArgs& g) {
    if (!g.gn_scale || !g.gn_shift || !g.gn_folded || g.taps != 9 || g.batch != 1 || g.a0_C % BK || (g.a1 && g.a1_C % BK)) return false;
    const int res = 1 << g.logW;
    if (g.logHW != 2 * g.logW || (res != 32 && res != 16 && res != 8 && res != 4) || g.N % 8) return false;
    if (res == 4 && (g.a0_C % (64 * CgH4T::Cfg::NG) || (g.a1 && g.a1_C % (64 * CgH4T::Cfg::NG)))) return false;
    if (res <= 8 ? (g.M % (res * res) || g.N % (res == 4 ? 128 : 256) || g.a0_up || g.a1_up || (g.resid && g.rowvec)) : g.M % std::max(256, conv_gn_bm(g)) != 0) return false;
    if (!conv_gn_regw(g)) return false;
    const int e = conv_gn_epi(g);
    return e == 1 || e == 2 || e == 5 || e == 6;
}
int g_w128 = 1;
bool w128_ok(const GemmArgs& g) {
    if (g.taps != 1 || g.a1 || g.gn_scale || g.deq_m || g.deq_n || g.splitk > 1) return false;
    if (g.a0_C % BK || g.a0_C < 2 * BK || g.N % 8 || g.M % 8) return false;
    return (int64_t)g.M * g.a0_ld * 2 < (int64_t)1 << 32 && (int64_t)g.N * g.b_ld * 2 < (int64_t)1 << 32;
}
int choose_variant(const GemmArgs& g) {
    if (g.gn_scale) return V_CONV_GN;
    const int K0 = g.taps * g.a0_C, K1 = g.a1 ? g.a1_C : 0;
    const bool dma = K0 % BK == 0 && K1 % BK == 0 && (g.taps == 1 || (g.a0_padded && g.a0_C % BK == 0));
    if (!dma) return V_GENERIC;
    if (g_force_variant == V_W128) {
        if (w128_ok(g) && (!g.gn_part || (1 << g.logHW) % 256 == 0)) return V_W128;
    }
    else if (g_force_variant > V_GENERIC && g_force_variant != V_CONV_GN && g_force_variant != V_FP8_256x256) {
        if (!g.gn_part || ((g.taps == 9 || g.logHW > 0) && (1 << g.logHW) % variant_bm(g_force_variant) == 0)) return g_force_variant;
    }
    const int64_t mt256 = (g.M + 255) / 256, mt128 = (g.M + 127) / 128;
    const int64_t nt128 = (g.N + 127) / 128;
    const bool w128 = g_w128 && w128_ok(g) && (!g.gn_part || (1 << g.logHW) % 256 == 0);
    const int64_t nt256 = (g.N + 255) / 256;
    const bool n_ok256 = g.N % 256 == 0 || (w128 && g.N % 128 == 0);
    if (g_round_model && g.taps == 1 && !g.gn_part && g.batch == 1 && n_ok256 && K0 + K1 >= 1024 && mt256 * nt256 < 2 * NUM_CU) {
        const int64_t r256 = (mt256 * nt256 + NUM_CU - 1) / NUM_CU, r128 = (mt128 * nt128 + 2 * NUM_CU - 1) / (2 * NUM_CU);
        const int64_t c256 = w128 ? g_round_model_w128 : 15;
        if (mt128 * nt128 >= NUM_CU / 2) return c256 * r256 < 10 * r128 ? (w128 ? V_W128 : V_DMA_256x256_H) : V_DMA_128x128_P;
    }
    if (n_ok256 && K0 + K1 >= 1024 && mt256 * nt256 * g.batch >= NUM_CU) return w128 ? V_W128 : V_DMA_256x256_H;
    if (g_pref_512 && g.N <= 128 && K0 + K1 >= 1024 && ((g.M + 511) / 512) * g.batch >= 2 * NUM_CU &&
        (!g.gn_part || (g.taps == 9 && (1 << g.logHW) % 512 == 0)))
        return V_DMA_512x128_H;
    if (mt256 * nt128 * g.batch >= 2 * NUM_CU) return V_RING_256x128_W4;
    if (mt128 * nt128 * g.batch >= NUM_CU) return V_DMA_128x128_P;
    return V_RING_64x128;
}

int fp8_epi(const GemmArgs& g) {
    if (g.epi_fp32_slab || g.resid || g.gn_part) return 0;
    if ((g.rowvec || g.gate) && g.log_rows_per_sample < 30 && ((1 << g.log_rows_per_sample) % 256 != 0)) return 0;
    if (g.c_mode == OUT_F32 && g.resid_f32 && !g.bias_m && g.act == ACT_NONE && g.resid_f32_ld % 4 == 0 && g.c_ld % 4 == 0) return 3;
    if (g.resid_f32 || g.gate) return 0;
    if (g.c_mode == OUT_BF16 && g.act == ACT_NONE) return 1;
    if (g.c_mode == OUT_FP8_MX && g.act == ACT_GELU_TANH && g.c_mx && g.N % 32 == 0 && !g.bias_m && g.scale == 1.0f) return 2;
    return 0;
}
bool w128_fp8_ok(const GemmArgs& g) {
    return g.taps == 1 && !g.a1 && g.a0_C % 256 == 0 && g.N % 8 == 0 && g.M % 8 == 0 && (!g.a_mx || g.M % 256 == 0) &&
           (int64_t)g.M * g.a0_ld < (int64_t)1 << 32 && (int64_t)g.N * g.b_ld < (int64_t)1 << 32;
}
bool fp8_on_w128(const GemmArgs& g) { return g_w128 && w128_fp8_ok(g) && (fp8_epi(g) != 2 || g_w128 != 2); }
template <bool MXA>
void launch_gemm_fp8_t(const GemmArgs& g, hipStream_t s) {
    if (fp8_on_w128(g)) launch_family<FamF8W128<MXA>>(fp8_epi(g), g, s);
    else launch_family<FamF8<MXA>>(fp8_epi(g), g, s);
}
std::string gemm_row(int M, int N, int K0, int K1, int taps, int batch, const std::string& name, int epi) {
    char line[160];
    snprintf(line, sizeof(line), "%d %d %d %d %d %d %s/e%d", M, N, K0, K1, taps, batch, name.c_str(), epi);
    return line;
}
void record_gemm(const GemmArgs& g, const std::string& name, int epi) { *g_record += gemm_row(g.M, g.N, g.taps * g.a0_C, g.a1 ? g.a1_C : 0, g.taps, g.batch, name, epi) + "\n"; }
struct GemmProf {
    struct Rec { hipEvent_t a, b; std::string tag; };
    bool on = false; std::vector<Rec> ev; std::vector<std::pair<hipEvent_t, hipEvent_t>> pool;
    bool begin(Rec& r, hipStream_t s) {
        r.a = r.b = nullptr;
        if (!pool.empty()) { r.a = pool.back().first; r.b = pool.back().second; pool.pop_back(); }
        else if (hipEventCreate(&r.a) != hipSuccess || hipEventCreate(&r.b) != hipSuccess) { r.a = r.b = nullptr; (void)hipGetLastError(); return false; }
        (void)hipEventRecord(r.a, s);
        return true;
    }
    void end(Rec& r, hipStream_t s) { (void)hipEventRecord(r.b, s); ev.push_back(std::move(r)); }
} g_gemm_prof;
thread_local int g_launch_error = 0;
void launch_gemm_fp8(const GemmArgs& g, hipStream_t s) {
    if (g.stream_guard && fp8_epi(g) != 3) { g_launch_error = 1; return; }
    GemmProf::Rec r;
    const bool prof = g_gemm_prof.on && !g_record && g_gemm_prof.begin(r, s);
    if (prof) r.tag = gemm_row(g.M, g.N, g.taps * g.a0_C, 0, g.taps, g.batch, std::string(fp8_on_w128(g) ? "w128_fp8" : "fp8_256x256") + (g.a_mx ? "_mxa" : ""), g.stream_guard ? 4 : fp8_epi(g));
    if (g.stream_guard) ncsn_sg::launch_fp8(&g, g.a_mx != nullptr, fp8_on_w128(g), g_raster_g, (void*)s);
    else if (g.a_mx) launch_gemm_fp8_t<true>(g, s); else launch_gemm_fp8_t<false>(g, s);
    if (prof) g_gemm_prof.end(r, s);
}

int packed_epi(const GemmArgs& g, int bm) {
    if (g.epi_fp32_slab || g.deq_m || g.deq_n || g.act == ACT_RELU) return 0;
    if (g.bias_m) return (g.c_mode == OUT_BF16 && !g.resid && !g.resid_f32 && !g.gate && !g.rowvec && !g.gn_part && g.act == ACT_NONE) ? 8 : 0;
    if ((g.rowvec || g.gate) && g.log_rows_per_sample < 30 && ((1 << g.log_rows_per_sample) % bm != 0)) return 0;
    if (g.c_mode == OUT_F32 && g.resid_f32 && !g.resid && !g.gn_part && g.act == ACT_NONE && g.resid_f32_ld % 4 == 0 && g.c_ld % 4 == 0) return 7;
    if (g.c_mode != OUT_BF16 || g.resid_f32 || g.gate) return 0;
    if (g.resid && (g.act != ACT_NONE || g.resid_ld % 4 != 0)) return 0;
    if (g.gn_part) return (g.act == ACT_NONE && g.M % bm == 0) ? (g.resid ? 6 : 2) : 0;
    if (g.resid) return 5;
    return g.act == ACT_NONE ? 1 : (g.act == ACT_SILU ? 3 : 4);
}
inline int effective_epi(int v, const GemmArgs& g) { const int e = packed_epi(g, variant_bm(v)); return ((epi_mask(v) >> e) & 1u) ? e : 0; }

thread_local bool g_fin_written = false;
int g_splitk = 1;
float* g_dbg_splitk_ws = nullptr; int g_dbg_splitk_max = 0;
int splitk_slices(const GemmArgs& g) {
    if (!g_splitk || !g.splitk_ws || g.splitk_max < 2 || g.batch != 1 || g.gn_scale || g.c_mode != OUT_BF16 || g.N % 8 || 256 % (g.N / 8)) return 1;
    if (g.gn_part && (g.M % SPLITK_ROWS || g.act != ACT_NONE || (g.taps == 9 && (1 << g.logHW) % SPLITK_ROWS))) return 1;
    if (g.bias_m || g.gate || g.resid_f32 || g.deq_m || g.deq_n) return 1;
    const int K0 = g.taps * g.a0_C, K1 = g.a1 ? g.a1_C : 0;
    if (K0 % 64 || K1 % 64 || (g.taps == 9 && !g.a0_padded) || K0 + K1 < 2048) return 1;
    const int64_t tiles = ((g.M + 127) / 128) * ((g.N + 127) / 128);
    if (tiles >= 2 * NUM_CU) return 1;
    int S = (int)((2 * NUM_CU + tiles - 1) / tiles);
    if (S > g.splitk_max) S = g.splitk_max;
    while (S > 1 && (K0 + K1) / 32 / S < 16) --S;
    return S;
}
int w128_splitk_slices(const GemmArgs& g) {
    if (!g_splitk || !g_w128 || !g.splitk_ws || g.splitk_max < 2 || g.batch != 1 || !w128_ok(g) || g.a0_C < 3072) return 1;
    if (g.c_mode != OUT_F32 || !g.resid_f32 || g.resid || g.rowvec || g.bias_m || g.gn_part || g.act != ACT_NONE || g.epi_fp32_slab || g.N % 4 || g.c_ld % 4 || g.resid_f32_ld % 4) return 1;
    const int64_t tiles = (int64_t)((g.M + 255) / 256) * ((g.N + 255) / 256) * g.batch;
    if (tiles * 2 > NUM_CU) return 1;
    int S = (int)(NUM_CU / tiles);
    if (S > g.splitk_max) S = g.splitk_max;
    while (S > 1 && g.a0_C / BK / S < 16) --S;
    return S;
}
int launch_gemm_run(const GemmArgs& g0, hipStream_t s);
int launch_gemm(const GemmArgs& g0, hipStream_t s) {
    if (!g_gemm_prof.on || g_record) return launch_gemm_run(g0, s);
    GemmProf::Rec r;
    std::string tag;
    g_record = &tag; (void)launch_gemm_run(g0, s); g_record = nullptr;
    while (!tag.empty() && tag.back() == '\n') tag.pop_back();
    if (!g_gemm_prof.begin(r, s)) return launch_gemm_run(g0, s);
    r.tag = std::move(tag);
    const int bm = launch_gemm_run(g0, s);
    g_gemm_prof.end(r, s);
    return bm;
}
int launch_gemm_run(const GemmArgs& g0, hipStream_t s) {
    if (g_force_variant == V_AUTO) {
        const int S8 = w128_splitk_slices(g0);
        if (S8 > 1) {
            if (g_record) { record_gemm(g0, "splitk" + std::to_string(S8) + "_w128_256x256", 7); return 256; }
            GemmArgs p = g0;
            p.splitk = S8; p.c = g0.splitk_ws; p.c_mode = OUT_F32;
            const int nM = (p.M + 255) / 256, nN = (p.N + 255) / 256;
            p.raster_g = 0;
            hipLaunchKernelGGL((k_gemm_w128<9>), dim3(nM * nN, S8, p.batch), dim3(256), W128Cfg::LDS_BYTES, s, p);
            const int64_t per = (int64_t)g0.M * (g0.N / 4);
            if (g0.stream_guard) ncsn_sg::launch_splitk_reduce(&g0, S8, (void*)s);
            else
            hipLaunchKernelGGL(k_splitk_reduce_f32, dim3((unsigned)((per + 255) / 256), (unsigned)g0.batch), dim3(256), 0, s, g0.splitk_ws, S8, (int64_t)g0.batch * g0.M * g0.N, g0.M, g0.N,
                               g0.bias_n, g0.gate, g0.gate_ld, g0.log_rows_per_sample, g0.z_samples, g0.resid_f32, g0.resid_f32_ld, g0.c_bs, g0.scale,
                               reinterpret_cast<float*>(g0.c), g0.c_ld, g0.stream_f16);
            return 256;
        }
    }
    const int S = g_force_variant == V_AUTO ? splitk_slices(g0) : 1;
    if (S > 1) {
        if (g_record) { record_gemm(g0, "splitk" + std::to_string(S) + "_ring128x128", 9); return SPLITK_ROWS; }
        GemmArgs p = g0;
        p.splitk = S; p.c = g0.splitk_ws; p.c_mode = OUT_F32; p.batch = S;
        p.bias_n = nullptr; p.rowvec = nullptr; p.resid = nullptr; p.scale = 1.0f; p.act = ACT_NONE; p.gn_part = nullptr;
        launch_tiles<CfgR128x128>(&k_gemm_ring<2, 2, 4, 4, 4, 9>, p, s);
        hipLaunchKernelGGL(k_splitk_reduce, dim3((unsigned)((g0.M + SPLITK_ROWS - 1) / SPLITK_ROWS)), dim3(256), 0, s, g0.splitk_ws, S, g0.M, g0.N,
                           g0.bias_n, g0.rowvec, g0.rowvec_ld, g0.log_rows_per_sample, reinterpret_cast<const bf16*>(g0.resid), g0.resid_ld, g0.scale,
                           g0.act, reinterpret_cast<bf16*>(g0.c), g0.c_ld, reinterpret_cast<float2*>(g0.gn_part), g0.gn_quads);
        return SPLITK_ROWS;
    }
    const GemmArgs& g = g0;
    const int v = choose_variant(g);
    if (g.taps == 9 && v != V_CONV_GN && g.a0_C % BK) {
        if (g_record) record_gemm(g, "invalid_conv3x3", 0); else g_launch_error = 1;
        return 256;
    }
    if (v == V_CONV_GN && !conv_gn_ok(g)) {
        if (g_record) record_gemm(g, "invalid_conv_gn", 0); else g_launch_error = 1;
        return 256;
    }
    const bool guarded = g.stream_guard != nullptr;
    if (guarded && !g_record && (!ncsn_sg::has_tile(v) || effective_epi(v, g) != 7)) { g_launch_error = 1; return 256; }
    if (g_record) {
        record_gemm(g, v == V_CONV_GN && conv_gn3_shape(g) >= 0 ? "conv_gn3" : variant_name(v), v == V_CONV_GN ? conv_gn_epi(g) : (guarded && effective_epi(v, g) == 7 ? 10 : effective_epi(v, g)));
        return v == V_CONV_GN ? conv_gn_part_rows(g) : variant_bm(v);
    }
    if (guarded) ncsn_sg::launch_tile(&g, v, g_raster_g, (void*)s);
    else if (v == V_GENERIC) {
        const int nM = (g.M + BM - 1) / BM, nN = (g.N + BN - 1) / BN;
        hipLaunchKernelGGL(k_gemm_bf16, dim3(nM * nN, 1, g.batch), dim3(256), GEMM_LDS_BYTES, s, g);
    } else if (v == V_CONV_GN) {
        GemmArgs gw = g0;
        gw.w_warm = (g_cg_warm >> (g0.logW - 2)) & 1;
        const int e = conv_gn_epi(gw);
        if (const int sh3 = conv_gn3_shape(gw); sh3 >= 0) {
            ncsn_cg3::launch(&gw, sh3, e, (void*)s);
            g_fin_written = sh3 == 2 && gw.fin_scale && (e == 2 || e == 6) && gw.N == 256;
        } else launch_conv_gn2(ConvGnShapes{}, 1 << gw.logW, conv_gn_bm(gw), e, gw, s);
        return conv_gn_part_rows(gw);
    } else with_family(v, [&](auto f) { launch_family<decltype(f)>(effective_epi(v, g), g, s); });
    return variant_bm(v);
}
inline int grid1d(int64_t n, int block = 256, int cap = 4096) {
    int64_t g = (n + block - 1) / block; return (int)(g < 1 ? 1 : (g > cap ? cap : g));
}

}
```

### naturaldiffusion_amd/csrc/ncsnpp.hip

```cpp
#include <hip/hip_runtime.h>
#include <stdint.h>
#include <stdio.h>
#include <string.h>
#include <stdlib.h>
#include <functional>
#include <map>
#include <memory>
#include <string>
#include <vector>

#include "natinf_ncsnpp.h"
#include "gemm_launch.h"
#include "engine_core.h"
#include "head_conv.h"
#include "attn256.h"
#include "attn_qkv.h"
#include "attn_blk256.h"

namespace {

constexpr int NF = 128, IMG = 32, TEMB = 512, NLEVEL = 4;
constexpr int CH_MULT[NLEVEL] = {1, 2, 2, 2};
constexpr float GN_EPS = 1e-6f;
constexpr float INV_SQRT2 = 0.70710678118654752440f;
inline bool attn_at(int res) { return res == 16; }

enum Kind { K_LIN, K_CONV, K_RES, K_ATTN, K_GN, K_DOWN, K_UP };
const char* kind_name(int k) { static const char* n[] = {"lin", "conv", "res", "attn", "gn", "down", "up"}; return n[k]; }

struct Mod { int idx, kind, cin, cout, up, down, res; int64_t poff; };

enum { CLS_GEMM = 0, CLS_OTHER = 1, CLS_CONV_GN = 2, CLS_CONV_GN8 = 3, N_CLS = 4 };

int g_fuse_head = 1;
constexpr int ATTN_BLK_DEFAULT = 2;
int g_attn_blk = ATTN_BLK_DEFAULT;
int g_attn_qkv = 1;
int g_attn_w8 = 1;
int g_attn_proj = 1;
int g_fuse_gn8 = 1;
int g_fuse_fin = 3;
int g_fuse_gn4 = 1;
int g_fuse_gn = 1;
int g_fuse_up = 1;

}

struct natinf_ncsnpp : EngineCore {
    int flags = 0;
    std::vector<Mod> mods;
    std::vector<int> op_cls;
    bool prof = false;
    struct Rec { hipEvent_t a, b; int cls; };
    std::vector<Rec> recs;
    std::vector<hipEvent_t> pool;
    std::map<int, TRef> taps;
    uint64_t plan_sig = 0;
    int last_B = 0; unsigned char* last_ws = nullptr;
    std::vector<unsigned char> fin_done;
};

namespace {

bool configure_ncsnpp_kernels() {
    return hipFuncSetAttribute(reinterpret_cast<const void*>(&k_head_conv), hipFuncAttributeMaxDynamicSharedMemorySize, HeadConvCfg::LDS_BYTES) == hipSuccess &&
           hipFuncSetAttribute(reinterpret_cast<const void*>(&k_qkv256), hipFuncAttributeMaxDynamicSharedMemorySize, QKV_LDS_BYTES) == hipSuccess &&
           hipFuncSetAttribute(reinterpret_cast<const void*>(&k_attn256<false>), hipFuncAttributeMaxDynamicSharedMemorySize, A256_LDS_BYTES) == hipSuccess &&
           hipFuncSetAttribute(reinterpret_cast<const void*>(&k_attn256<true>), hipFuncAttributeMaxDynamicSharedMemorySize, A256_LDS_BYTES) == hipSuccess &&
           hipFuncSetAttribute(reinterpret_cast<const void*>(&k_attn256<true, 8>), hipFuncAttributeMaxDynamicSharedMemorySize, A256_LDS_BYTES) == hipSuccess &&
           hipFuncSetAttribute(reinterpret_cast<const void*>(&k_attn_blk256), hipFuncAttributeMaxDynamicSharedMemorySize, ABLK_LDS_BYTES) == hipSuccess &&
           hipFuncSetAttribute(reinterpret_cast<const void*>(&k_attn_blk256_v2), hipFuncAttributeMaxDynamicSharedMemorySize, ABLK2_LDS_BYTES) == hipSuccess;
}

struct AttnBlk256 {
    int plan = 0;
    int B = 0;
    const bf16* x = nullptr; int x_ld = 0;
    const float* sc = nullptr; const float* sh = nullptr;
    const bf16* wqkvf = nullptr; const float* bqk = nullptr; const float* bv = nullptr; bf16* qk = nullptr; bf16* vT = nullptr;
    const bf16* w3f = nullptr; const float* b3 = nullptr;
    const bf16* wqf2 = nullptr; const float* cq2 = nullptr; const bf16* wvof2 = nullptr; const float* bo2 = nullptr;
    bf16* out = nullptr; int o_ld = 0; float out_scale = 1.0f;
    float2* gn_part = nullptr; int gn_quads = 0;
};
void pack_attn_qkv_w(const float* w0, const float* w1, const float* w2, bf16* wqkvf, hipStream_t s) {
    hipLaunchKernelGGL(k_pack_qkv_w, dim3(3 * 256), dim3(256), 0, s, w0, w1, w2, wqkvf);
}
void pack_attn_w3(const float* w3, bf16* w3f, hipStream_t s) { hipLaunchKernelGGL(k_pack_attn_w3, dim3(256), dim3(256), 0, s, w3, w3f); }
void pack_attn_fold(const float* w0, const float* w1, const float* w2, const float* w3, const float* b0, const float* b2, const float* b3,
                    float* fq, float* cq, float* fv, float* bo, bf16* wqf2, bf16* wvof2, hipStream_t s) {
    hipLaunchKernelGGL(k_attn_fold_w, dim3(257), dim3(256), 0, s, w0, w1, w2, w3, b0, b2, b3, fq, cq, fv, bo);
    hipLaunchKernelGGL(k_pack_qkv_w, dim3(256), dim3(256), 0, s, (const float*)fq, (const float*)fq, (const float*)fq, wqf2, 1);
    hipLaunchKernelGGL(k_pack_attn_w3, dim3(256), dim3(256), 0, s, (const float*)fv, wvof2);
}
void launch_attn_qkv256(const AttnBlk256& a, hipStream_t s) {
    hipLaunchKernelGGL(k_qkv256, dim3((unsigned)a.B), dim3(512), QKV_LDS_BYTES, s, a.x, a.x_ld, a.sc, a.sh, a.wqkvf, a.bqk, a.bv, a.qk, a.vT);
}
int launch_attn_blk256(const AttnBlk256& a, hipStream_t s) {
    constexpr int C = 256;
    if (a.plan == 2) {
        hipLaunchKernelGGL(k_attn_blk256_v2, dim3((unsigned)a.B), dim3(512), ABLK2_LDS_BYTES, s, a.x, a.x_ld, a.sc, a.sh,
                           a.wqf2, a.cq2, 1.0f / sqrtf((float)C), a.wvof2, a.bo2, a.out, a.o_ld, a.out_scale, a.gn_part, a.gn_quads);
        return 256;
    }
    if (a.plan == 1) {
        hipLaunchKernelGGL(k_attn_blk256, dim3((unsigned)a.B), dim3(512), ABLK_LDS_BYTES, s, a.x, a.x_ld, a.sc, a.sh,
                           a.wqkvf, a.bqk, a.bv, a.qk, a.vT, 1.0f / sqrtf((float)C), a.w3f, a.b3, a.out, a.o_ld, a.out_scale, a.gn_part, a.gn_quads);
        return 256;
    }
    if (g_attn_w8) {
        hipLaunchKernelGGL((k_attn256<true, 8>), dim3((unsigned)a.B), dim3(512), A256_LDS_BYTES, s, (const bf16*)a.qk, 2 * C, C, (const bf16*)a.vT, a.out, a.o_ld,
                           1.0f / sqrtf((float)C), a.w3f, a.b3, a.x, a.x_ld, a.out_scale, a.gn_part, a.gn_quads);
        return 256;
    }
    hipLaunchKernelGGL(k_attn256<true>, dim3((unsigned)(2 * a.B)), dim3(256), A256_LDS_BYTES, s, (const bf16*)a.qk, 2 * C, C, (const bf16*)a.vT, a.out, a.o_ld,
                       1.0f / sqrtf((float)C), a.w3f, a.b3, a.x, a.x_ld, a.out_scale, a.gn_part, a.gn_quads);
    return 128;
}

struct Builder : PlanBuilder {
    natinf_ncsnpp& E;
    int dense_total = 0; int64_t dense_w = 0, dense_b = 0, dense_out = 0;

    const bool ddpm;
    const int NUM_RES;
    const float res_scale;
    explicit Builder(natinf_ncsnpp& e) : PlanBuilder(e), E(e), ddpm((e.flags & NATINF_NCSNPP_DDPM) != 0), NUM_RES(ddpm ? 2 : 4), res_scale(ddpm ? 1.0f : INV_SQRT2) {
        arena.keep = (e.flags & NATINF_NCSNPP_KEEP_ACTIVATIONS) != 0;
    }

    void op(int cls, OpFn f) { E.ops.push_back(std::move(f)); E.op_cls.push_back(cls); }

    void pack_conv(int64_t src, int64_t dst, int N, int Cin, int taps, int dst_ld, int koff, int tapstride, float wmul = 1.0f) {
        const int chunked = taps == 9 && Cin % BK == 0;
        E.packs.push_back([=](const PackCtx& p) {
            const int64_t n = (int64_t)N * Cin * taps;
            hipLaunchKernelGGL(k_pack_conv, dim3(grid1d(n, 256, 1 << 30)), dim3(256), 0, p.stream, p.params + src,
                               reinterpret_cast<bf16*>(p.packed + dst), N, Cin, taps, dst_ld, koff, tapstride, chunked, wmul);
        });
    }
    void pack_frag(int64_t src_packed, int64_t dst, int N, int ld, int cin, int c1) {
        E.packs.push_back([=](const PackCtx& p) {
            const int64_t n = (int64_t)(N / 16) * (9 * (cin / 32) + c1 / 32) * 64;
            hipLaunchKernelGGL(k_pack_frag, dim3(grid1d(n, 256, 1 << 30)), dim3(256), 0, p.stream, reinterpret_cast<const bf16*>(p.packed + src_packed),
                               reinterpret_cast<bf16*>(p.packed + dst), N, ld, cin, c1);
        });
    }
    void pack_transpose(int64_t src, int64_t dst, int K, int N, int dst_ld) {
        E.packs.push_back([=](const PackCtx& p) {
            hipLaunchKernelGGL(k_pack_transpose, dim3(grid1d((int64_t)K * N, 256, 1 << 30)), dim3(256), 0, p.stream,
                               p.params + src, reinterpret_cast<bf16*>(p.packed + dst), K, N, dst_ld);
        });
    }
    void pack_zero(int64_t dst, int64_t n) {
        E.packs.push_back([=](const PackCtx& p) {
            hipLaunchKernelGGL(k_fill_bf16_zero, dim3(grid1d(n, 256, 1 << 30)), dim3(256), 0, p.stream,
                               reinterpret_cast<bf16*>(p.packed + dst), n);
        });
    }

    struct GN { int64_t gamma, beta; };
    GN take_gn(int C) { GN g; g.gamma = pack_f32(take(C), C); g.beta = pack_f32(take(C), C); return g; }

    void emit_gn_stats(const TRef& x, GN gn, int64_t& sc, int64_t& sh, float out_mul = 1.0f) {
        if (emit_gn_from_parts(x, gn, sc, sh, out_mul)) return;
        const int HW = x.res * x.res;
        op(CLS_OTHER, [=](const Ctx& c) {
            hipLaunchKernelGGL(k_gn_stats, dim3(c.B), dim3(256), 0, c.stream, c.act(x), x.ld, x.C, HW,
                               c.w<float>(gn.gamma), c.w<float>(gn.beta), c.at<float>(sc), c.at<float>(sh), GN_EPS, out_mul);
        });
    }
    void emit_gn_apply(const TRef& x, int64_t sc, int64_t sh, const TRef& y, const TRef* xr, int act, int mode) {
        const int logW = ilog2(x.res), logHW = 2 * logW;
        const int rd = mode == RS_UP ? 2 * x.res : (mode == RS_DOWN ? x.res / 2 : x.res);
        const int rows_per_img = rd + 2 * y.pad;
        const TRef xrr = xr ? *xr : TRef();
        op(CLS_OTHER, [=](const Ctx& c) {
            hipLaunchKernelGGL(k_gn_apply, dim3((unsigned)((rows_per_img + GN_ROWS - 1) / GN_ROWS), (unsigned)c.B), dim3(256), 0, c.stream, c.act(x), x.ld, x.C,
                               logW, logHW, c.at<float>(sc), c.at<float>(sh), c.act(y),
                               xrr.off >= 0 ? c.act(xrr) : (bf16*)nullptr, act, mode, y.pad);
        });
    }
    TRef new_act(int res, int C, int pad = 0) {
        TRef t; t.off = arena.alloc((int64_t)(res + 2 * pad) * (res + 2 * pad) * C * 2); t.C = C; t.ld = C; t.res = res; t.pad = pad;
        return t;
    }

    void emit_res(const Mod& m, const TRef& x, const TRef& out) {
        const int cin = m.cin, cout = m.cout;
        const int ro = m.up ? m.res * 2 : (m.down ? m.res / 2 : m.res);
        const bool shortcut = cin != cout || m.up || m.down;
        const GN gn0 = take_gn(cin);
        const int64_t p_c0w = take((int64_t)cout * cin * 9), p_c0b = take(cout);
        const int64_t p_dw = take((int64_t)cout * TEMB), p_db = take(cout);
        const GN gn1 = take_gn(cout);
        const int64_t p_c1w = take((int64_t)cout * cout * 9), p_c1b = take(cout);
        const int64_t p_c2w = shortcut ? take((int64_t)cout * cin) : -1, p_c2b = shortcut ? take(cout) : -1;

        const int K0a = 9 * cin, K1tot = 9 * cout + (shortcut ? cin : 0);
        const bool fusable_res = g_fuse_gn && (ro == 32 || ro == 16 || (ro == 8 && g_fuse_gn8 && cout % 256 == 0) || (ro == 4 && g_fuse_gn4 && cout % 256 == 0));
        const bool fuse1 = fusable_res && cout % BK == 0;
        const bool fuse_up = fuse1 && ro > 8 && g_fuse_up && m.up && cin % BK == 0 && cout % 128 == 0;
        const bool fuse = (fusable_res && !m.up && !m.down && cin % BK == 0) || fuse_up;
        const float LOG2E = 1.4426950408889634f, LN2 = 0.6931471805599453f;
        const float gn_mul = fuse ? -LOG2E : 1.0f, w_mul = fuse ? -LN2 : 1.0f, gn_mul1 = fuse1 ? -LOG2E : 1.0f, w_mul1 = fuse1 ? -LN2 : 1.0f;
        const int64_t w0 = wres((int64_t)cout * K0a * 2), w1 = wres((int64_t)cout * K1tot * 2);
        pack_conv(p_c0w, w0, cout, cin, 9, K0a, 0, cin, w_mul);
        pack_conv(p_c1w, w1, cout, cout, 9, K1tot, 0, cout, w_mul1);
        if (shortcut && !ddpm) pack_conv(p_c2w, w1, cout, cin, 1, K1tot, 9 * cout, cin);
        if (shortcut && ddpm) pack_transpose(p_c2w, w1 + (int64_t)9 * cout * 2, cin, cout, K1tot);
        const int64_t w0f = (fuse && cout % 16 == 0) ? wres((int64_t)cout * K0a * 2) : -1, w1f = (fuse1 && cout % 16 == 0) ? wres((int64_t)cout * K1tot * 2) : -1;
        if (w0f >= 0) pack_frag(w0, w0f, cout, K0a, cin, 0);
        if (w1f >= 0) pack_frag(w1, w1f, cout, K1tot, cout, shortcut ? cin : 0);
        const int64_t b0 = pack_f32(p_c0b, cout), b1 = pack_f32(p_c1b, cout, shortcut ? p_c2b : -1);
        const int drow = dense_rows_next;
        pack_conv(p_dw, dense_w + (int64_t)drow * TEMB * 2, cout, TEMB, 1, TEMB, 0, TEMB);
        pack_f32_at(p_db, cout, dense_b + (int64_t)drow * 4);
        dense_rows_next += cout;

        const int64_t own_sc = arena.alloc((int64_t)std::max(cin, cout) * 4), own_sh = arena.alloc((int64_t)std::max(cin, cout) * 4);
        int64_t sc = own_sc, sh = own_sh;
        emit_gn_stats(x, gn0, sc, sh, gn_mul);
        TRef h, xr;
        if (!fuse) {
            h = new_act(ro, cin, 1);
            if (m.up || m.down) xr = new_act(ro, cin);
            emit_gn_apply(x, sc, sh, h, (m.up || m.down) ? &xr : nullptr, ACT_SILU, m.up ? RS_UP : (m.down ? RS_DOWN : RS_NONE));
        }

        const int SK_MAX = 4;
        const int64_t skws = (ro <= 8) ? arena.alloc((int64_t)SK_MAX * ro * ro * cout * 4) : -1;
        TRef t = new_act(ro, cout);
        const Part pt = register_output(t, fuse);
        const int logW = ilog2(ro), logHW = 2 * logW, HWo = ro * ro;
        const int dtotal = dense_total; const int64_t dout = dense_out;
        op(fuse ? (ro <= 8 ? CLS_CONV_GN8 : CLS_CONV_GN) : CLS_GEMM, [=](const Ctx& c) {
            GemmArgs g = gemm_defaults();
            if (fuse) { g.a0 = c.act(x); g.a0_ld = x.ld; g.gn_scale = c.at<float>(sc); g.gn_shift = c.at<float>(sh); g.gn_ld = cin; g.gn_folded = 1; g.a0_up = fuse_up; }
            else { g.a0 = c.act(h); g.a0_ld = h.ld; g.a0_padded = 1; }
            g.a0_C = cin; g.taps = 9; g.logW = logW; g.logHW = logHW;
            g.M = c.B * HWo; g.N = cout; g.b = c.w<bf16>(w0); g.b_ld = K0a;
            if (w0f >= 0) g.b_frag = c.w<bf16>(w0f);
            g.bias_n = c.w<float>(b0);
            g.rowvec = c.at<float>(dout) + drow; g.rowvec_ld = dtotal; g.log_rows_per_sample = logHW;
            if (skws >= 0) { g.splitk_ws = c.at<float>(skws); g.splitk_max = SK_MAX; }
            g.c = c.act(t); g.c_ld = t.ld;
            if (pt.valid) { g.gn_part = c.at<float>(pt.off); g.gn_quads = pt.quads; set_fin(g, pt, c); }
            g_fin_written = false;
            const int bm = launch_gemm(g, c.stream);
            if (pt.valid) c.part_bm[pt.id] = bm;
            if (pt.fin && pt.fin->check) c.fin_done[pt.id] = g_fin_written;
        });
        if (!fuse) arena.release(h.off);
        int64_t sc1 = own_sc, sh1 = own_sh;
        emit_gn_stats(t, gn1, sc1, sh1, gn_mul1);
        TRef u;
        if (!fuse1) {
            u = new_act(ro, cout, 1);
            emit_gn_apply(t, sc1, sh1, u, nullptr, ACT_SILU, RS_NONE);
            arena.release(t.off);
        }
        if (pt.valid) arena.release(pt.off);
        const TRef xs = ((m.up || m.down) && !fuse_up) ? xr : x;
        const float rs = res_scale;
        const Part po = register_output(out, fuse1);
        op(fuse1 ? (ro <= 8 ? CLS_CONV_GN8 : CLS_CONV_GN) : CLS_GEMM, [=](const Ctx& c) {
            GemmArgs g = gemm_defaults();
            if (fuse1) { g.a0 = c.act(t); g.a0_ld = t.ld; g.gn_scale = c.at<float>(sc1); g.gn_shift = c.at<float>(sh1); g.gn_ld = cout; g.gn_folded = 1; }
            else { g.a0 = c.act(u); g.a0_ld = u.ld; g.a0_padded = 1; }
            g.a0_C = cout; g.taps = 9; g.logW = logW; g.logHW = logHW;
            if (shortcut) { g.a1 = c.act(xs); g.a1_ld = xs.ld; g.a1_C = cin; g.a1_up = fuse_up; }
            else { g.resid = c.act(xs); g.resid_ld = xs.ld; }
            g.M = c.B * HWo; g.N = cout; g.b = c.w<bf16>(w1); g.b_ld = K1tot;
            if (w1f >= 0) g.b_frag = c.w<bf16>(w1f);
            g.bias_n = c.w<float>(b1); g.scale = rs;
            if (skws >= 0) { g.splitk_ws = c.at<float>(skws); g.splitk_max = SK_MAX; }
            g.c = c.act(out); g.c_ld = out.ld;
            if (po.valid) { g.gn_part = c.at<float>(po.off); g.gn_quads = po.quads; set_fin(g, po, c); }
            g_fin_written = false;
            const int bm = launch_gemm(g, c.stream);
            if (po.valid) c.part_bm[po.id] = bm;
            if (po.fin && po.fin->check) c.fin_done[po.id] = g_fin_written;
        });
        if (skws >= 0) arena.release(skws);
        if (fuse1) arena.release(t.off); else arena.release(u.off);
        if ((m.up || m.down) && !fuse_up) arena.release(xr.off);
        arena.release(own_sc); arena.release(own_sh);
        if (sc != own_sc) { arena.release(sc); arena.release(sh); }
        if (sc1 != own_sc) { arena.release(sc1); arena.release(sh1); }
        E.taps[m.idx] = out;
    }

    void emit_attn(const Mod& m, const TRef& x, const TRef& out) {
        const int C = m.cin, T = m.res * m.res;
        const GN gn = take_gn(C);
        int64_t pw[4], pb[4];
        for (int i = 0; i < 4; ++i) { pw[i] = take((int64_t)C * C); pb[i] = take(C); }
        const int64_t wqk = wres((int64_t)2 * C * C * 2), wv = wres((int64_t)C * C * 2), w3 = wres((int64_t)C * C * 2);
        pack_transpose(pw[0], wqk, C, C, C);
        pack_transpose(pw[1], wqk + (int64_t)C * C * 2, C, C, C);
        pack_transpose(pw[2], wv, C, C, C);
        pack_transpose(pw[3], w3, C, C, C);
        const int64_t bqk = wres((int64_t)2 * C * 4);
        pack_f32_at(pb[0], C, bqk); pack_f32_at(pb[1], C, bqk + (int64_t)C * 4);
        const int64_t bv = pack_f32(pb[2], C), b3 = pack_f32(pb[3], C);

        const int64_t own_sc = arena.alloc((int64_t)C * 4), own_sh = arena.alloc((int64_t)C * 4);
        int64_t sc = own_sc, sh = own_sh;
        emit_gn_stats(x, gn, sc, sh);
        const bool fuse_qkv = T == 256 && C == 256 && g_attn_qkv;
        TRef h = new_act(m.res, C);
        if (!fuse_qkv) emit_gn_apply(x, sc, sh, h, nullptr, ACT_NONE, RS_NONE);
        const int64_t qk = arena.alloc((int64_t)T * 2 * C * 2), vT = arena.alloc((int64_t)C * T * 2);
        const bool blk = fuse_qkv && g_attn_proj && g_attn_w8 && g_attn_blk;
        int64_t wqkvf = -1;
        const int64_t sc_q = sc, sh_q = sh;
        if (fuse_qkv) {
            wqkvf = wres((int64_t)3 * C * C * 2);
            const int64_t s0 = pw[0], s1 = pw[1], s2 = pw[2];
            E.packs.push_back([=](const PackCtx& p) { pack_attn_qkv_w(p.params + s0, p.params + s1, p.params + s2, reinterpret_cast<bf16*>(p.packed + wqkvf), p.stream); });
            const int64_t sc_ = sc, sh_ = sh;
            if (!blk)
            op(CLS_GEMM, [=](const Ctx& c) {
                if (g_record) return;
                AttnBlk256 a;
                a.B = c.B; a.x = c.act(x); a.x_ld = x.ld; a.sc = c.at<float>(sc_); a.sh = c.at<float>(sh_);
                a.wqkvf = c.w<bf16>(wqkvf); a.bqk = c.w<float>(bqk); a.bv = c.w<float>(bv); a.qk = c.at<bf16>(qk); a.vT = c.at<bf16>(vT);
                launch_attn_qkv256(a, c.stream);
            });
        }
        if (!fuse_qkv)
        op(CLS_GEMM, [=](const Ctx& c) {
            GemmArgs g = gemm_defaults();
            g.a0 = c.act(h); g.a0_ld = C; g.a0_C = C; g.M = c.B * T; g.N = 2 * C;
            g.b = c.w<bf16>(wqk); g.b_ld = C; g.bias_n = c.w<float>(bqk);
            g.c = c.at<bf16>(qk); g.c_ld = 2 * C;
            launch_gemm(g, c.stream);
        });
        if (!fuse_qkv)
        op(CLS_GEMM, [=](const Ctx& c) {
            GemmArgs g = gemm_defaults();
            g.a0 = c.w<bf16>(wv); g.a0_ld = C; g.a0_C = C; g.a_bs = 0; g.M = C; g.N = T;
            g.b = c.act(h); g.b_ld = C; g.b_bs = (int64_t)T * C; g.bias_m = c.w<float>(bv);
            g.c = c.at<bf16>(vT); g.c_ld = T; g.c_bs = (int64_t)C * T; g.batch = c.B;
            launch_gemm(g, c.stream);
        });
        arena.release(h.off);
        const bool proj = T == 256 && C == 256 && g_attn_proj;
        int64_t w3f = -1;
        if (proj) {
            w3f = wres((int64_t)C * C * 2);
            const int64_t src = pw[3];
            E.packs.push_back([=](const PackCtx& p) { pack_attn_w3(p.params + src, reinterpret_cast<bf16*>(p.packed + w3f), p.stream); });
        }
        const bool blk2 = blk && g_attn_blk == 2;
        int64_t wqf2 = -1, wvof2 = -1, cq2 = -1, bo2 = -1;
        if (blk2) {
            const int64_t fq = wres((int64_t)C * C * 4), fv = wres((int64_t)C * C * 4);
            cq2 = wres((int64_t)C * 4); bo2 = wres((int64_t)C * 4);
            wqf2 = wres((int64_t)C * C * 2); wvof2 = wres((int64_t)C * C * 2);
            const int64_t w0_ = pw[0], w1_ = pw[1], w2_ = pw[2], w3_ = pw[3], b0_ = pb[0], b2_ = pb[2], b3_ = pb[3], cq_ = cq2, bo_ = bo2, wq_ = wqf2, wv_ = wvof2;
            E.packs.push_back([=](const PackCtx& p) {
                pack_attn_fold(p.params + w0_, p.params + w1_, p.params + w2_, p.params + w3_, p.params + b0_, p.params + b2_, p.params + b3_,
                               reinterpret_cast<float*>(p.packed + fq), reinterpret_cast<float*>(p.packed + cq_), reinterpret_cast<float*>(p.packed + fv),
                               reinterpret_cast<float*>(p.packed + bo_), reinterpret_cast<bf16*>(p.packed + wq_), reinterpret_cast<bf16*>(p.packed + wv_), p.stream);
            });
        }
        const Part po_attn = proj ? register_output(out) : Part();
        const float rs_attn = res_scale;
        TRef O = new_act(m.res, C);
        if (T == 256 && C == 256) {
            op(CLS_GEMM, [=](const Ctx& c) {
                if (g_record) return;
                if (proj) {
                    AttnBlk256 a;
                    a.plan = blk2 ? 2 : (blk ? 1 : 0); a.B = c.B; a.x = c.act(x); a.x_ld = x.ld; a.sc = c.at<float>(sc_q); a.sh = c.at<float>(sh_q);
                    if (wqkvf >= 0) a.wqkvf = c.w<bf16>(wqkvf);
                    a.bqk = c.w<float>(bqk); a.bv = c.w<float>(bv); a.qk = c.at<bf16>(qk); a.vT = c.at<bf16>(vT); a.w3f = c.w<bf16>(w3f); a.b3 = c.w<float>(b3);
                    if (blk2) { a.wqf2 = c.w<bf16>(wqf2); a.cq2 = c.w<float>(cq2); a.wvof2 = c.w<bf16>(wvof2); a.bo2 = c.w<float>(bo2); }
                    a.out = c.act(out); a.o_ld = out.ld; a.out_scale = rs_attn;
                    if (po_attn.valid) { a.gn_part = c.at<float2>(po_attn.off); a.gn_quads = po_attn.quads; }
                    const int rows = launch_attn_blk256(a, c.stream);
                    if (po_attn.valid) c.part_bm[po_attn.id] = rows;
                }
                else
                    hipLaunchKernelGGL(k_attn256<false>, dim3((unsigned)(2 * c.B)), dim3(256), A256_LDS_BYTES, c.stream, c.at<bf16>(qk), 2 * C, C, c.at<bf16>(vT), c.act(O), C,
                                       1.0f / sqrtf((float)C), (const bf16*)nullptr, (const float*)nullptr, (const bf16*)nullptr, 0, 1.0f, (float2*)nullptr, 0);
            });
            arena.release(vT); arena.release(qk);
        } else {
// ... 273 lines not shown
            pack_zero(w, (int64_t)NF * 64);
            pack_conv(pw, w, NF, 3, 9, 64, 0, 3);
            const int64_t b = pack_f32(pb, NF);
            const int64_t a0 = arena.alloc((int64_t)IMG * IMG * 64 * 2);
            const TRef dst = cur;
            const Part po = register_output(dst);
            op(CLS_OTHER, [=](const Ctx& c) {
                const int64_t rows = (int64_t)c.B * IMG * IMG;
                hipLaunchKernelGGL(k_stem_im2col, dim3((unsigned)((rows * 8 + 255) / 256)), dim3(256), 0, c.stream, c.x, c.at<bf16>(a0), rows);
            });
            op(CLS_GEMM, [=](const Ctx& c) {
                const int64_t rows = (int64_t)c.B * IMG * IMG;
                GemmArgs g = gemm_defaults();
                g.a0 = c.at<bf16>(a0); g.a0_ld = 64; g.a0_C = 64; g.M = (int)rows; g.N = NF;
                g.b = c.w<bf16>(w); g.b_ld = 64; g.bias_n = c.w<float>(b);
                g.c = c.act(dst); g.c_ld = dst.ld;
                if (po.valid) { g.gn_part = c.at<float>(po.off); g.gn_quads = po.quads; }
                const int bm = launch_gemm(g, c.stream);
                if (po.valid) c.part_bm[po.id] = bm;
            });
            arena.release(a0);
            E.taps[m.idx] = dst;
        }
        int res = IMG;
        for (int l = 0; l < NLEVEL; ++l) {
            for (int b = 0; b < NUM_RES; ++b) {
                const Mod& m = M[mi++];
                const TRef dst = skip_slot(si++);
                if (attn_at(res)) {
                    TRef tmp = new_act(res, m.cout);
                    emit_res(m, cur, tmp);
                    emit_attn(M[mi++], tmp, dst);
                    arena.release(tmp.off);
                } else {
                    emit_res(m, cur, dst);
                }
                cur = dst;
            }
            if (l != NLEVEL - 1) {
                const Mod& m = M[mi++];
                const TRef dst = skip_slot(si++);
                if (ddpm) emit_downconv(m, cur, dst); else emit_res(m, cur, dst);
                cur = dst; res /= 2;
            }
        }
        {
            TRef a = new_act(res, cur.C), b = new_act(res, cur.C);
            emit_res(M[mi++], cur, a);
            emit_attn(M[mi++], a, b);
            arena.release(a.off);
            emit_res(M[mi++], b, h_slot(0));
            arena.release(b.off);
        }
        int j = 0;
        TRef last;
        for (int l = NLEVEL - 1; l >= 0; --l) {
            for (int b = 0; b < NUM_RES + 1; ++b) {
                const Mod& m = M[mi++];
                const bool level_end = b == NUM_RES;
                TRef in = cats[j].buf;
                TRef dst = level_end ? new_act(res, m.cout) : h_slot(j + 1);
                emit_res(m, in, dst);
                arena.release(cats[j].buf.off);
                last = dst; ++j;
            }
            if (attn_at(res)) {
                TRef dst = new_act(res, last.C);
                emit_attn(M[mi++], last, dst);
                arena.release(last.off);
                last = dst;
            }
            if (l != 0) {
                const Mod& m = M[mi++];
                if (ddpm) emit_upconv(m, last, h_slot(j)); else emit_res(m, last, h_slot(j));
                arena.release(last.off);
                res *= 2;
            }
        }
        {
            const Mod& mg = M[mi++]; const Mod& mc = M[mi++];
            const GN gn = take_gn(mg.cin);
            const int64_t pw = take((int64_t)3 * mc.cin * 9), pb = take(3);
            const int Kf = 9 * mc.cin;
            const int64_t w = wres((int64_t)3 * Kf * 2);
            pack_conv(pw, w, 3, mc.cin, 9, Kf, 0, mc.cin);
            const int64_t b = pack_f32(pb, 3);
            int64_t sc = arena.alloc((int64_t)mg.cin * 4), sh = arena.alloc((int64_t)mg.cin * 4);
            const int logW = ilog2(res), cinf = mc.cin;
            if (g_fuse_head && res == HeadConvCfg::RES && mc.cin == HeadConvCfg::C) {
                const int64_t w16 = wres((int64_t)16 * Kf * 2);
                pack_zero(w16, (int64_t)16 * Kf);
                pack_conv(pw, w16, 3, mc.cin, 9, Kf, 0, mc.cin, -0.6931471805599453f);
                emit_gn_stats(last, gn, sc, sh, -1.4426950408889634f);
                const TRef src = last;
                op(CLS_GEMM, [=](const Ctx& c) {
                    if (g_record) { *g_record += gemm_row(c.B * res * res, 3, Kf, 0, 9, 1, "head_conv", 0) + "\n"; return; }
                    hipLaunchKernelGGL(k_head_conv, dim3((unsigned)(c.B * (HeadConvCfg::RES / HeadConvCfg::ROWS))), dim3(256), HeadConvCfg::LDS_BYTES, c.stream,
                                       c.act(src), src.ld, c.at<float>(sc), c.at<float>(sh), c.w<bf16>(w16), c.w<float>(b), c.out);
                });
            } else {
            emit_gn_stats(last, gn, sc, sh);
            TRef u = new_act(res, mg.cin, 1);
            emit_gn_apply(last, sc, sh, u, nullptr, ACT_SILU, RS_NONE);
            op(CLS_GEMM, [=](const Ctx& c) {
                GemmArgs g = gemm_defaults();
                g.a0 = c.act(u); g.a0_ld = u.ld; g.a0_C = cinf; g.taps = 9; g.logW = logW; g.logHW = 2 * logW; g.a0_padded = 1;
                g.M = c.B * res * res; g.N = 3; g.b = c.w<bf16>(w); g.b_ld = Kf; g.bias_n = c.w<float>(b);
                g.c = c.out; g.c_mode = OUT_F32_NCHW;
                launch_gemm(g, c.stream);
            });
            }
            E.taps[mg.idx] = last;
        }
        finish();
        E.part_bm.assign(n_parts > 0 ? n_parts : 1, 128);
        E.fin_done.assign(n_parts > 0 ? n_parts : 1, 0);
    }
};

int64_t module_param_count(const Mod& m) {
    switch (m.kind) {
        case K_LIN: return (int64_t)m.cout * m.cin + m.cout;
        case K_CONV: return (int64_t)m.cout * m.cin * 9 + m.cout;
        case K_GN: return 2 * (int64_t)m.cin;
        case K_DOWN: case K_UP: return (int64_t)m.cout * m.cin * 9 + m.cout;
        case K_ATTN: return 2 * (int64_t)m.cin + 4 * ((int64_t)m.cin * m.cin + m.cin);
        case K_RES: {
            int64_t n = 2 * (int64_t)m.cin + (int64_t)m.cout * m.cin * 9 + m.cout + (int64_t)m.cout * TEMB + m.cout +
                        2 * (int64_t)m.cout + (int64_t)m.cout * m.cout * 9 + m.cout;
            if (m.cin != m.cout || m.up || m.down) n += (int64_t)m.cout * m.cin + m.cout;
            return n;
        }
    }
    return 0;
}

natinf_ncsnpp* make_engine(int flags) {
    natinf_ncsnpp* e = new natinf_ncsnpp();
    e->flags = flags;
    Builder b(*e);
    b.build();
    int64_t off = 0;
    for (auto& m : e->mods) { m.poff = off; off += module_param_count(m); }
    if (off != e->n_params) { delete e; return nullptr; }
    return e;
}

const natinf_ncsnpp& reference_engine() {
    static natinf_ncsnpp* e = [] {
        int* knobs[] = {&g_fuse_gn, &g_fuse_up, &g_fuse_head, &g_fuse_gn8, &g_fuse_gn4, &g_fuse_fin, &g_attn_qkv, &g_attn_proj};
        int saved[sizeof(knobs) / sizeof(knobs[0])];
        for (size_t i = 0; i < sizeof(knobs) / sizeof(knobs[0]); ++i) { saved[i] = *knobs[i]; *knobs[i] = 1; }
        g_fuse_fin = 3;
        natinf_ncsnpp* r = make_engine(0);
        for (size_t i = 0; i < sizeof(knobs) / sizeof(knobs[0]); ++i) *knobs[i] = saved[i];
        return r;
    }();
    return *e;
}

}

extern "C" {

int64_t natinf_ncsnpp_param_count(void) { return reference_engine().n_params; }
int64_t natinf_ncsnpp_packed_bytes(void) { return reference_engine().packed_bytes; }

int64_t natinf_ncsnpp_handle_param_count(natinf_ncsnpp_t h) { return h ? h->n_params : NATINF_EINVAL; }
int64_t natinf_ncsnpp_handle_packed_bytes(natinf_ncsnpp_t h) { return h ? h->packed_bytes : NATINF_EINVAL; }

int64_t natinf_ncsnpp_workspace_bytes(natinf_ncsnpp_t h, int max_batch) {
    if (!h || max_batch <= 0) return NATINF_EINVAL;
    return h->ws_per_image * (int64_t)max_batch;
}

static uint64_t plan_signature() {
    const int k[] = {g_fuse_head, g_attn_qkv, g_attn_w8, g_attn_proj, g_fuse_gn8, g_fuse_fin, g_fuse_gn4, g_fuse_gn, g_cg_wide, g_fuse_up,
                     g_attn_blk , g_cg3 };
    uint64_t h = 1469598103934665603ull;
    for (int v : k) h = (h ^ (uint64_t)(v & 0xff)) * 1099511628211ull;
    return h;
}

int natinf_ncsnpp_create(natinf_ncsnpp_t* out, int flags) {
    if (!out || (flags & ~(NATINF_NCSNPP_KEEP_ACTIVATIONS | NATINF_NCSNPP_DDPM))) return NATINF_EINVAL;
    natinf_ncsnpp* e = make_engine(flags);
    if (!e) return NATINF_ESTATE;
    e->plan_sig = plan_signature();
    *out = e;
    return NATINF_OK;
}

int natinf_ncsnpp_destroy(natinf_ncsnpp_t h) {
    if (!h) return NATINF_EINVAL;
    for (auto& r : h->recs) { (void)hipEventDestroy(r.a); (void)hipEventDestroy(r.b); }
    for (auto e : h->pool) (void)hipEventDestroy(e);
    delete h;
    return NATINF_OK;
}

int natinf_ncsnpp_describe(natinf_ncsnpp_t h, char* buf, int cap) {
    if (!h || !buf || cap <= 0) return NATINF_EINVAL;
    std::string s;
    char line[160];
    for (const auto& m : h->mods) {
        snprintf(line, sizeof(line), "%d %s %d %d %d %d %d %lld\n", m.idx, kind_name(m.kind), m.cin, m.cout, m.up, m.down, m.res,
                 (long long)m.poff);
        s += line;
    }
    if ((int)s.size() + 1 > cap) return NATINF_EINVAL;
    memcpy(buf, s.c_str(), s.size() + 1);
    return (int)s.size();
}

int natinf_ncsnpp_load(natinf_ncsnpp_t h, const float* params_f32, int64_t n_params, void* packed, int64_t packed_bytes,
                       natinf_stream_t stream) {
    return h ? h->load(params_f32, n_params, packed, packed_bytes, (hipStream_t)stream) : NATINF_EINVAL;
}

int natinf_ncsnpp_share(natinf_ncsnpp_t h, natinf_ncsnpp_t loaded) {
    if (!h || !loaded || h == loaded) return NATINF_EINVAL;
    if (!loaded->packed) return NATINF_ESTATE;
    if ((h->flags & NATINF_NCSNPP_DDPM) != (loaded->flags & NATINF_NCSNPP_DDPM) || h->n_params != loaded->n_params || h->packed_bytes != loaded->packed_bytes ||
        h->packs.size() != loaded->packs.size() || h->plan_sig != loaded->plan_sig)
        return NATINF_EINVAL;
    h->packed = loaded->packed;
    return NATINF_OK;
}

int natinf_ncsnpp_forward(natinf_ncsnpp_t h, const float* x, const float* labels, float* out, int B, void* workspace,
                          int64_t workspace_bytes, natinf_stream_t stream) {
    if (!h || !x || !labels || !out || !workspace || B <= 0) return NATINF_EINVAL;
    if (!h->packed) return NATINF_ESTATE;
    if (workspace_bytes < h->ws_per_image * (int64_t)B || (int64_t)B * IMG * IMG >= (1LL << 31)) return NATINF_EINVAL;
    if (!h->configured) {
        if (!configure_gemm_kernels()) return NATINF_ENODEV;
        h->configured = true;
    }
    Ctx c{B, reinterpret_cast<unsigned char*>(workspace), h->packed, (hipStream_t)stream, x, labels, out, h->part_bm.data()};
    c.fin_done = h->fin_done.data();
    g_launch_error = 0;
    if (!h->prof) {
        for (const auto& f : h->ops) f(c);
    } else {
        for (size_t i = 0; i < h->ops.size(); ++i) {
            natinf_ncsnpp::Rec r; r.cls = h->op_cls[i];
            for (hipEvent_t* e : {&r.a, &r.b}) {
                if (!h->pool.empty()) { *e = h->pool.back(); h->pool.pop_back(); }
                else if (hipEventCreate(e) != hipSuccess) return NATINF_ELAUNCH;
            }
            (void)hipEventRecord(r.a, c.stream);
            h->ops[i](c);
            (void)hipEventRecord(r.b, c.stream);
            h->recs.push_back(r);
        }
    }
    h->last_B = B; h->last_ws = c.ws;
    if (g_launch_error) { g_launch_error = 0; return NATINF_ESTATE; }
    return hipGetLastError() == hipSuccess ? NATINF_OK : NATINF_ELAUNCH;
}

int natinf_ncsnpp_describe_gemms(natinf_ncsnpp_t h, int B, char* buf, int cap) {
    if (!h || !buf || cap <= 0 || B <= 0) return NATINF_EINVAL;
    std::string out;
    g_record = &out;
    std::vector<int> scratch_bm(h->part_bm.size(), 128);
    std::vector<unsigned char> scratch_done(h->part_bm.size(), 0);
    Ctx c{B, reinterpret_cast<unsigned char*>(4096), reinterpret_cast<const unsigned char*>(4096), nullptr, nullptr, nullptr, nullptr, scratch_bm.data()};
    c.fin_done = scratch_done.data();
    for (size_t i = 0; i < h->ops.size(); ++i)
        if (h->op_cls[i] == CLS_GEMM || h->op_cls[i] == CLS_CONV_GN || h->op_cls[i] == CLS_CONV_GN8) h->ops[i](c);
    g_record = nullptr;
    if ((int)out.size() + 1 > cap) return NATINF_EINVAL;
    memcpy(buf, out.c_str(), out.size() + 1);
    return (int)out.size();
}

int natinf_debug_gemm(int variant, int M, int N, int K0, int K1, int taps, int logW, int batch,
                      const void* a0, const void* a1, const void* b, const float* bias_n, void* c, int c_f32, float scale,
                      int iters, natinf_stream_t stream) {
    if (variant < 0 || variant >= V_COUNT || !a0 || !b || !c || M <= 0 || N <= 0 || K0 <= 0 || K1 < 0 || iters <= 0 || (taps != 1 && taps != 9)) return NATINF_EINVAL;
    if (K0 % taps || N % 8 || (a1 != nullptr) != (K1 > 0)) return NATINF_EINVAL;
    if (taps == 9 && ((K0 / 9) % BK || logW < 1 || logW > 12 || M % (1 << (2 * logW)) || batch != 1)) return NATINF_EINVAL;
    if (!variant_shipped(variant) || variant == V_CONV_GN || variant == V_FP8_256x256) return NATINF_ESTATE;
#ifndef NATINF_DEV
    if (c_f32 >= 2) return NATINF_ESTATE;
#endif
    static bool configured = false;
    if (!configured) { if (!configure_gemm_kernels()) return NATINF_ENODEV; configured = true; }
    GemmArgs g = gemm_defaults();
    g.a0 = (const bf16*)a0; g.a0_C = K0 / taps; g.a0_ld = g.a0_C; g.taps = taps; g.logW = logW; g.logHW = 2 * logW; g.a0_padded = taps == 9;
    if (a1) { g.a1 = (const bf16*)a1; g.a1_C = K1; g.a1_ld = K1; }
    g.M = M; g.N = N; g.b = (const bf16*)b; g.b_ld = K0 + (a1 ? K1 : 0); g.batch = batch;
    if (batch > 1) { g.a_bs = (int64_t)M * g.a0_ld; g.b_bs = (int64_t)N * g.b_ld; g.c_bs = (int64_t)M * N; }
    g.bias_n = bias_n; g.scale = scale; g.c = c; g.c_ld = N; g.c_mode = c_f32 == 1 ? OUT_F32 : (c_f32 >= 2 ? 100 + c_f32 : OUT_BF16);
    g.dbg_ts = g_dbg_ts;
    g.splitk_ws = g_dbg_splitk_ws; g.splitk_max = g_dbg_splitk_max;
    const int saved = g_force_variant;
    g_force_variant = variant;
    g_launch_error = 0;
    for (int i = 0; i < iters; ++i) launch_gemm(g, (hipStream_t)stream);
    g_force_variant = saved;
    if (g_launch_error) { g_launch_error = 0; return NATINF_EINVAL; }
    return hipGetLastError() == hipSuccess ? NATINF_OK : NATINF_ELAUNCH;
}

int g_dbg_conv_logW = 0; const void* g_dbg_conv_a1 = nullptr; int g_dbg_conv_c1 = 0;
int natinf_debug_set_conv_operand(int logW, const void* a1, int c1) {
    if (logW < 0 || logW > 12 || c1 < 0 || c1 % BK || (c1 > 0) != (a1 != nullptr) || (logW == 0 && a1)) return NATINF_EINVAL;
    g_dbg_conv_logW = logW; g_dbg_conv_a1 = a1; g_dbg_conv_c1 = c1;
    return NATINF_OK;
}

int natinf_debug_gemm_fused(int variant, int M, int N, int K, const void* a, const void* b, const float* bias_n, const float* bias_m,
                            const float* rowvec, const float* gate, int log_rows_per_sample, const void* resid_bf16, const float* resid_f32,
                            float scale, int act, void* c, int c_f32, float* gn_part, int* bm_out, int fp32_slab, natinf_stream_t stream) {
    const int logW = g_dbg_conv_logW, c1 = g_dbg_conv_c1;
    const void* a1 = g_dbg_conv_a1;
    g_dbg_conv_logW = 0; g_dbg_conv_a1 = nullptr; g_dbg_conv_c1 = 0;
    if (variant < 0 || variant >= V_COUNT || !a || !b || !c || M <= 0 || N <= 0 || K <= 0 || c_f32 < 0 || c_f32 > 2) return NATINF_EINVAL;
    if (c_f32 == 2) {
        if (!logW || bias_m || rowvec || gate || resid_bf16 || resid_f32 || gn_part || act != ACT_NONE) return NATINF_EINVAL;
    } else if (N % 8) return NATINF_EINVAL;
    if (logW && (K % 9 || (K / 9) % BK || M % (1 << (2 * logW)))) return NATINF_EINVAL;
    if (!variant_shipped(variant) || variant == V_CONV_GN || variant == V_FP8_256x256) return NATINF_ESTATE;
    if (!configure_gemm_kernels()) return NATINF_ENODEV;
    GemmArgs g = gemm_defaults();
    g.a0 = (const bf16*)a; g.a0_C = K; g.a0_ld = K; g.M = M; g.N = N; g.b = (const bf16*)b; g.b_ld = K;
    if (logW) {
        g.taps = 9; g.a0_C = g.a0_ld = K / 9; g.logW = logW; g.logHW = 2 * logW; g.a0_padded = 1; g.b_ld = K + c1;
        if (a1) { g.a1 = (const bf16*)a1; g.a1_C = g.a1_ld = c1; }
    }
    g.bias_n = bias_n; g.bias_m = bias_m; g.rowvec = rowvec; g.rowvec_ld = N; g.gate = gate; g.gate_ld = N; g.log_rows_per_sample = log_rows_per_sample;
    g.resid = (const bf16*)resid_bf16; g.resid_ld = N; g.resid_f32 = resid_f32; g.resid_f32_ld = N;
    g.scale = scale; g.act = act; g.c = c; g.c_ld = N; g.c_mode = c_f32 == 2 ? OUT_F32_NCHW : (c_f32 ? OUT_F32 : OUT_BF16);
    g.gn_part = gn_part; g.gn_quads = N / 4; g.epi_fp32_slab = fp32_slab != 0;
    g.splitk_ws = g_dbg_splitk_ws; g.splitk_max = g_dbg_splitk_max;
    g.dbg_ts = g_dbg_ts;
    const int saved = g_force_variant;
    g_force_variant = variant;
    g_launch_error = 0;
    const int bm = launch_gemm(g, (hipStream_t)stream);
    g_force_variant = saved;
    if (bm_out) *bm_out = bm;
    if (g_launch_error) { g_launch_error = 0; return NATINF_EINVAL; }
    return hipGetLastError() == hipSuccess ? NATINF_OK : NATINF_ELAUNCH;
}

int g_dbg_cg_up = 0;
int natinf_debug_conv_gn_up(int flags) { if (flags & ~3) return NATINF_EINVAL; g_dbg_cg_up = flags; return NATINF_OK; }
int natinf_debug_conv_gn(int res, int B, int N, int cin, int c1, const void* x, const float* scale, const float* shift, const void* w_packed,
                         void* w_frag, const void* a1, const float* bias_n, const void* resid, float out_scale, void* out, float* gn_part, int iters,
                         natinf_stream_t stream) {
    if ((res != 32 && res != 16 && res != 8 && res != 4) || B <= 0 || N <= 0 || N % 8 || cin <= 0 || cin % 64 || c1 < 0 || c1 % 64 || (c1 > 0) != (a1 != nullptr) ||
        !x || !scale || !shift || !w_packed || !out || iters <= 0) return NATINF_EINVAL;
    static bool configured = false;
    if (!configured) { if (!configure_gemm_kernels()) return NATINF_ENODEV; configured = true; }
    GemmArgs g = gemm_defaults();
    g.a0 = (const bf16*)x; g.a0_ld = cin; g.a0_C = cin; g.taps = 9; g.logW = ilog2(res); g.logHW = 2 * g.logW;
    g.gn_scale = scale; g.gn_shift = shift; g.gn_ld = cin; g.gn_folded = 1;
    if (a1) { g.a1 = (const bf16*)a1; g.a1_ld = c1; g.a1_C = c1; }
    g.M = B * res * res; g.N = N; g.b = (const bf16*)w_packed; g.b_ld = 9 * cin + c1; g.bias_n = bias_n;
    g.resid = (const bf16*)resid; g.resid_ld = N; g.scale = out_scale; g.c = out; g.c_ld = N;
    g.gn_part = gn_part; g.gn_quads = N / 4;
    g.dbg_ts = g_dbg_ts;
    g.a0_up = g_dbg_cg_up & 1; g.a1_up = (a1 && (g_dbg_cg_up & 2)) ? 1 : 0;
    if (w_frag && N % 16 == 0) g.b_frag = (const bf16*)w_frag;
    if (!conv_gn_ok(g)) return NATINF_EINVAL;
    if (g.b_frag) {
        const int64_t n = (int64_t)(N / 16) * (9 * (cin / 32) + c1 / 32) * 64;
        hipLaunchKernelGGL(k_pack_frag, dim3(grid1d(n, 256, 1 << 30)), dim3(256), 0, (hipStream_t)stream, (const bf16*)w_packed, (bf16*)w_frag, N, g.b_ld, cin, c1);
    }
    for (int i = 0; i < iters; ++i) launch_gemm(g, (hipStream_t)stream);
    return hipGetLastError() == hipSuccess ? NATINF_OK : NATINF_ELAUNCH;
}

int natinf_debug_attn_block(int plan, int B, const void* x, int x_ld, const float* scale, const float* shift, const float* w, const float* bias,
                            void* packed, void* scratch, void* out, int o_ld, float out_scale, float* gn_part, natinf_stream_t stream) {
    if (plan < 0 || plan > 2 || B < 1 || !x || !scale || !shift || !w || !bias || !packed || !out || x_ld < 256 || x_ld % 8 || o_ld < 256 || o_ld % 8 ||
        (plan != 2 && !scratch)) return NATINF_EINVAL;
    static bool configured = false;
    if (!configured) { if (!configure_gemm_kernels()) return NATINF_ENODEV; configured = true; }
    constexpr int64_t WW = 256 * 256;
    unsigned char* pk = reinterpret_cast<unsigned char*>(packed);
    hipStream_t s = (hipStream_t)stream;
    AttnBlk256 a;
    a.plan = plan; a.B = B; a.x = (const bf16*)x; a.x_ld = x_ld; a.sc = scale; a.sh = shift;
    a.out = (bf16*)out; a.o_ld = o_ld; a.out_scale = out_scale; a.gn_part = reinterpret_cast<float2*>(gn_part); a.gn_quads = 64;
    if (plan == 2) {
        float* fq = reinterpret_cast<float*>(pk + NATINF_ATTN_BLOCK_OFF_FOLD_WQK); float* fv = reinterpret_cast<float*>(pk + NATINF_ATTN_BLOCK_OFF_FOLD_WVO);
        float* cq = reinterpret_cast<float*>(pk + NATINF_ATTN_BLOCK_OFF_FOLD_CQ); float* bo = reinterpret_cast<float*>(pk + NATINF_ATTN_BLOCK_OFF_FOLD_BO);
        bf16* wqf2 = reinterpret_cast<bf16*>(pk + NATINF_ATTN_BLOCK_OFF_WQK_PACKED); bf16* wvof2 = reinterpret_cast<bf16*>(pk + NATINF_ATTN_BLOCK_OFF_WVO_PACKED);
        pack_attn_fold(w, w + WW, w + 2 * WW, w + 3 * WW, bias, bias + 512, bias + 768, fq, cq, fv, bo, wqf2, wvof2, s);
        a.wqf2 = wqf2; a.cq2 = cq; a.wvof2 = wvof2; a.bo2 = bo;
    } else {
        bf16* wqkvf = reinterpret_cast<bf16*>(pk + NATINF_ATTN_BLOCK_OFF_WQKV); bf16* w3f = reinterpret_cast<bf16*>(pk + NATINF_ATTN_BLOCK_OFF_W3);
        pack_attn_qkv_w(w, w + WW, w + 2 * WW, wqkvf, s);
        pack_attn_w3(w + 3 * WW, w3f, s);
        a.wqkvf = wqkvf; a.bqk = bias; a.bv = bias + 512; a.w3f = w3f; a.b3 = bias + 768;
        a.qk = reinterpret_cast<bf16*>(scratch); a.vT = a.qk + (int64_t)B * 256 * 512;
        if (plan == 0) launch_attn_qkv256(a, s);
    }
    launch_attn_blk256(a, s);
    return hipGetLastError() == hipSuccess ? NATINF_OK : NATINF_ELAUNCH;
}

int natinf_debug_quant_fp8_rows(const float* w, void* q, float* row_scale, int rows, int cols, natinf_stream_t stream) {
    if (!w || !q || !row_scale || rows <= 0 || cols <= 0 || cols % 2) return NATINF_EINVAL;
    hipLaunchKernelGGL(k_pack_fp8_rows, dim3((unsigned)((rows + 3) / 4)), dim3(256), 0, (hipStream_t)stream, w, (uint8_t*)q, row_scale, rows, cols);
    return hipGetLastError() == hipSuccess ? NATINF_OK : NATINF_ELAUNCH;
}

int natinf_debug_gemm_fp8(int M, int N, int K, const void* a8, const float* a_scale, const void* a_mx, const void* b8, const float* b_scale,
                          const float* bias_n, void* c, void* c_mx, int c_mode, int iters, natinf_stream_t stream) {
    if (!a8 || !b8 || !c || M <= 0 || N <= 0 || K <= 0 || K % 128 || N % 8 || iters <= 0) return NATINF_EINVAL;
    static bool configured = false;
    if (!configured) { if (!configure_gemm_kernels()) return NATINF_ENODEV; configured = true; }
    GemmArgs g = gemm_defaults();
    g.a0 = (const bf16*)a8; g.a0_C = K; g.a0_ld = K; g.M = M; g.N = N; g.b = (const bf16*)b8; g.b_ld = K;
    const int act = c_mode >> 8; c_mode &= 0xff;
    if (act != ACT_NONE && act != ACT_GELU_TANH) return NATINF_EINVAL;
    g.deq_m = a_scale; g.deq_n = b_scale; g.bias_n = bias_n; g.c = c; g.c_ld = N; g.c_mode = c_mode; g.act = act;
    g.a_mx = (const uint8_t*)a_mx; g.a_mx_ld = M; g.c_mx = (uint8_t*)c_mx; g.c_mx_ld = M;
    if ((c_mode == OUT_FP8_MX && (!c_mx || N % 32)) || c_mode < 0 || c_mode > OUT_FP8_MX || c_mode == OUT_F32_NCHW) return NATINF_EINVAL;
    for (int i = 0; i < iters; ++i) launch_gemm_fp8(g, (hipStream_t)stream);
    return hipGetLastError() == hipSuccess ? NATINF_OK : NATINF_ELAUNCH;
}

int natinf_debug_timestamps(void* dev_buf16) {
#ifdef NATINF_DEV
    g_dbg_ts = reinterpret_cast<unsigned long long*>(dev_buf16); return NATINF_OK;
#else
    (void)dev_buf16; return NATINF_ESTATE;
#endif
}

int natinf_set_gemm_raster(int rows) { g_raster_g = rows; return NATINF_OK; }
int natinf_set_fuse_gn(int on) { g_fuse_gn = on != 0; return NATINF_OK; }
int natinf_set_fuse_gn8(int on) { g_fuse_gn8 = on != 0; return NATINF_OK; }
int natinf_set_attn256(int on) { return on ? NATINF_OK : NATINF_ESTATE; }
int natinf_set_conv_gn_warm(int mask) { if (mask < 0 || mask > 15) return NATINF_EINVAL; g_cg_warm = mask; return NATINF_OK; }
int natinf_set_attn_block(int on) { g_attn_blk = on < 0 ? ATTN_BLK_DEFAULT : (on > 2 ? 2 : on); return NATINF_OK; }
int natinf_set_attn_qkv(int on) { g_attn_qkv = on != 0; return NATINF_OK; }
int natinf_set_attn_waves8(int on) { g_attn_w8 = on != 0; return NATINF_OK; }
int natinf_set_attn_proj(int on) { g_attn_proj = on != 0; return NATINF_OK; }
int natinf_set_fuse_fin(int on) {
    if (on < 0 || on > 3) return NATINF_EINVAL;
    static const int mask[4] = {0, 3, 1, 2};
    g_fuse_fin = mask[on];
    return NATINF_OK;
}
int natinf_set_gemm_round_model(int on) { g_round_model = on != 0; g_round_model_w128 = on >= 10 ? on : 13; return NATINF_OK; }
int natinf_set_gemm_w128(int on) { g_w128 = on < 0 ? 0 : (on > 2 ? 2 : on); return NATINF_OK; }
int natinf_set_fuse_gn4(int on) { g_fuse_gn4 = on != 0; return NATINF_OK; }
int natinf_set_conv_gn8_tile(int one_image) { return one_image ? NATINF_OK : NATINF_ESTATE; }
int natinf_set_fuse_head(int on) { g_fuse_head = on != 0; return NATINF_OK; }
int natinf_set_conv_gn_w128(int mask) { if (mask < 0 || mask > 7) return NATINF_EINVAL; g_cg3 = mask; return NATINF_OK; }
int natinf_set_conv_gn_w128_min_k(int shape, int k) { if (shape < 0 || shape > 2 || k < 0) return NATINF_EINVAL; g_cg3_min_k[shape] = k; return NATINF_OK; }
int natinf_set_conv_gn_wide(int mask) { if (mask < 0 || mask > 3) return NATINF_EINVAL; g_cg_wide = mask; return NATINF_OK; }
int natinf_set_conv_gn_regw(int on) { return on ? NATINF_OK : NATINF_ESTATE; }
int natinf_set_fuse_up(int on) { g_fuse_up = on != 0; return NATINF_OK; }
int natinf_set_gemm_splitk(int on) { g_splitk = on != 0; return NATINF_OK; }
int natinf_debug_set_splitk_workspace(float* ws, int max_slices) { g_dbg_splitk_ws = ws; g_dbg_splitk_max = ws ? max_slices : 0; return NATINF_OK; }
int natinf_set_gemm_half_issue(int on) { return on ? NATINF_OK : NATINF_ESTATE; }
int natinf_set_gemm_pref512(int on) { g_pref_512 = on != 0; return NATINF_OK; }
int natinf_set_gemm_epilogue(int fp32_slab) { g_epi_fp32_slab = fp32_slab != 0; return NATINF_OK; }

int natinf_set_gemm_variant(int variant) {
    if (variant < 0 || variant >= V_COUNT) return NATINF_EINVAL;
    if (!variant_shipped(variant) || variant == V_CONV_GN || variant == V_FP8_256x256) return NATINF_ESTATE;
    g_force_variant = variant;
    return NATINF_OK;
}

int natinf_gemm_profile(int enable) { g_gemm_prof.on = enable != 0; return NATINF_OK; }
int natinf_gemm_profile_read(char* buf, int cap) {
    if (!buf || cap <= 0) return NATINF_EINVAL;
    std::map<std::string, std::pair<double, int64_t>> by;
    std::vector<std::string> order;
    int rc = NATINF_OK;
    for (auto& e : g_gemm_prof.ev) {
        float ms = 0.f;
        if (hipEventSynchronize(e.b) != hipSuccess || hipEventElapsedTime(&ms, e.a, e.b) != hipSuccess) { (void)hipGetLastError(); rc = NATINF_ELAUNCH; }
        else {
            auto it = by.find(e.tag);
            if (it == by.end()) { order.push_back(e.tag); it = by.emplace(e.tag, std::make_pair(0.0, (int64_t)0)).first; }
            it->second.first += ms; it->second.second += 1;
        }
        g_gemm_prof.pool.emplace_back(e.a, e.b);
    }
    g_gemm_prof.ev.clear();
    if (rc != NATINF_OK) return rc;
    std::string out;
    for (auto& t : order) {
        char tail[64];
        snprintf(tail, sizeof(tail), " %lld %.6f\n", (long long)by[t].second, by[t].first);
        out += t + tail;
    }
    if ((int)out.size() + 1 > cap) return NATINF_EINVAL;
    memcpy(buf, out.c_str(), out.size() + 1);
    return (int)out.size();
}
int natinf_ncsnpp_profile(natinf_ncsnpp_t h, int enable) {
    if (!h) return NATINF_EINVAL;
    h->prof = enable != 0;
    return NATINF_OK;
}

int natinf_ncsnpp_profile_read(natinf_ncsnpp_t h, double* ms_by_class, int64_t* launches_by_class) {
    if (!h || !ms_by_class || !launches_by_class) return NATINF_EINVAL;
    for (int i = 0; i < N_CLS; ++i) { ms_by_class[i] = 0.0; launches_by_class[i] = 0; }
    for (const auto& r : h->recs) {
        float ms = 0.f;
        if (hipEventSynchronize(r.b) != hipSuccess || hipEventElapsedTime(&ms, r.a, r.b) != hipSuccess) {
            (void)hipGetLastError();
            return NATINF_ELAUNCH;
        }
        ms_by_class[r.cls] += ms; launches_by_class[r.cls] += 1;
        h->pool.push_back(r.a); h->pool.push_back(r.b);
    }
    h->recs.clear();
    return NATINF_OK;
}

int natinf_ncsnpp_debug_tap(natinf_ncsnpp_t h, int module_idx, float* out, int64_t capacity_elems, natinf_stream_t stream) {
    if (!h || !out) return NATINF_EINVAL;
    if (!(h->flags & NATINF_NCSNPP_KEEP_ACTIVATIONS) || !h->last_ws) return NATINF_ESTATE;
    auto it = h->taps.find(module_idx);
    if (it == h->taps.end()) return NATINF_EINVAL;
    const TRef& t = it->second;
    const int HW = t.res * t.res;
    const int64_t total = (int64_t)h->last_B * t.C * HW;
    if (capacity_elems < total) return NATINF_EINVAL;
    const bf16* src = reinterpret_cast<const bf16*>(h->last_ws + t.off * h->last_B) + t.coff;
    hipLaunchKernelGGL(k_nhwc_to_nchw_f32, dim3(grid1d(total, 256, 1 << 30)), dim3(256), 0, (hipStream_t)stream, src, t.ld, t.C, HW, out, total);
    return hipGetLastError() == hipSuccess ? NATINF_OK : NATINF_ELAUNCH;
}

}
#include "dit_engine.inc"
#include "mmdit_engine.inc"
#include "vae_engine.inc"
#include "inception_engine.inc"
```

Before: 3482 images/s.

## Fold nearest-upsample into conv weights as four-phase 2x2 conv at low resolution

For the up-sampling ResNet blocks at 32x32 with 256 output channels, the nearest-neighbour 2x upsample followed by a 3x3 conv is rewritten as four 2x2 convs evaluated on the 16x16 input. One conv runs per output phase, using pre-summed folded weights, and the epilogue scatters rows into the interleaved high-resolution output and per-phase GroupNorm partials. This cuts the K dimension from 9*Cin to 4*Cin and removes the upsampled activation reads. It adds a new kernel family, a fold packing kernel and an extra GN-apply pass on the low-res input, and the folded weights are summed before bf16 rounding, which slightly changes numerics.

```diff
diff --git a/include/natinf_ncsnpp.h b/include/natinf_ncsnpp.h
--- a/include/natinf_ncsnpp.h
+++ b/include/natinf_ncsnpp.h
@@ -73,6 +73,10 @@
 int natinf_set_conv_gn_w128_min_k(int shape, int k);
 int natinf_set_conv_gn_regw(int on);
 int natinf_set_fuse_up(int on);
+int natinf_set_fuse_up_fold(int on);
+int natinf_debug_fold_up_weights(const float* w, int N, int cin, float w_mul, float* out_f32, void* out_packed, natinf_stream_t stream);
+int natinf_debug_conv_up_fold(int B, int N, int cin, const void* x, const float* scale, const float* shift, const float* w, void* w_packed, void* h_scratch,
+                              const float* bias_n, const float* rowvec, float out_scale, void* out, float* gn_part, int iters, natinf_stream_t stream);
 int natinf_set_fuse_head(int on);
 int natinf_set_fuse_gn8(int on);
 int natinf_set_fuse_gn4(int on);
diff --git a/naturaldiffusion_amd/_lib.py b/naturaldiffusion_amd/_lib.py
--- a/naturaldiffusion_amd/_lib.py
+++ b/naturaldiffusion_amd/_lib.py
@@ -80,6 +80,9 @@
     "natinf_set_conv_gn_w128_min_k": (C.c_int, [_i32, _i32]),
     "natinf_set_conv_gn_regw": (C.c_int, [_i32]),
     "natinf_set_fuse_up": (C.c_int, [_i32]),
+    "natinf_set_fuse_up_fold": (C.c_int, [_i32]),
+    "natinf_debug_fold_up_weights": (C.c_int, [_p, _i32, _i32, _f32, _p, _p, _p]),
+    "natinf_debug_conv_up_fold": (C.c_int, [_i32, _i32, _i32, _p, _p, _p, _p, _p, _p, _p, _p, _f32, _p, _p, _i32, _p]),
     "natinf_set_fuse_head": (C.c_int, [_i32]),
     "natinf_set_fuse_gn8": (C.c_int, [_i32]),
     "natinf_set_fuse_gn4": (C.c_int, [_i32]),
diff --git a/naturaldiffusion_amd/csrc/gemm_dma.h b/naturaldiffusion_amd/csrc/gemm_dma.h
--- a/naturaldiffusion_amd/csrc/gemm_dma.h
+++ b/naturaldiffusion_amd/csrc/gemm_dma.h
@@ -57,23 +57,25 @@
 __device__ __forceinline__ uint4 gload_u4(const void* p) { const gu32x4 t = *as_global(reinterpret_cast<const gu32x4*>(p)); return make_uint4(t[0], t[1], t[2], t[3]); }
 __device__ __forceinline__ float4 gload_f4(const void* p) { const gf32x4 t = *as_global(reinterpret_cast<const gf32x4*>(p)); return make_float4(t[0], t[1], t[2], t[3]); }
 __device__ __forceinline__ void gstore_u4(void* p, uint4 v) { *as_global(reinterpret_cast<gu32x4*>(p)) = gu32x4{v.x, v.y, v.z, v.w}; }
-template <int SW, int NSW, int RPS, int PROW, bool EDGE>
+template <int SW, int NSW, int RPS, int PROW, bool EDGE, int DSTEP = RPS>
 struct SlabCopy {
     template <class T>
     static __device__ __forceinline__ void run(const unsigned char* src, T* dst, int64_t ld, int m, int M) {
         const uint4 v = *reinterpret_cast<const uint4*>(src + SW * RPS * PROW);
-        SlabCopy<SW + 1, NSW, RPS, PROW, EDGE>::run(src, dst, ld, m, M);
-        if (!EDGE || m + SW * RPS < M) gstore_u4(dst + (int64_t)(SW * RPS) * ld, v);
+        SlabCopy<SW + 1, NSW, RPS, PROW, EDGE, DSTEP>::run(src, dst, ld, m, M);
+        if (!EDGE || m + SW * RPS < M) gstore_u4(dst + (int64_t)(SW * DSTEP) * ld, v);
     }
 };
-template <int NSW, int RPS, int PROW, bool EDGE>
-struct SlabCopy<NSW, NSW, RPS, PROW, EDGE> {
+template <int NSW, int RPS, int PROW, bool EDGE, int DSTEP>
+struct SlabCopy<NSW, NSW, RPS, PROW, EDGE, DSTEP> {
     template <class T> static __device__ __forceinline__ void run(const unsigned char*, T*, int64_t, int, int) {}
 };
-template <int WM, int WN, int TM, int TN, class Cfg, int ACT, bool GN, bool RES, bool DEQ = false, bool OUT8 = false, int NSAMP = 1, bool FIN = false, bool PAIR = false, bool SCALE_ALWAYS = false>
+template <int WM, int WN, int TM, int TN, class Cfg, int ACT, bool GN, bool RES, bool DEQ = false, bool OUT8 = false, int NSAMP = 1, bool FIN = false, bool PAIR = false, bool SCALE_ALWAYS = false, int UPW = 0>
 __device__ __forceinline__ void packed_tile_epilogue(const GemmArgs& g, unsigned char* smem, f32x4 (&acc)[TM][TN],
                                                      int m0, int n0, int z, int tid, int lane, int wm, int wn)
 {
+    const int phase = UPW > 0 ? z : 0;
+    if constexpr (UPW > 0) z = 0;
     constexpr int BN_ = WN * TN * 16, BM_ = WM * TM * 16, THREADS = WM * WN * 64, PROW = OUT8 ? BN_ + 16 : Cfg::PROW;
     static_assert(!OUT8 || (!GN && !RES && TN % 2 == 0), "fp8 output: plain column terms only");
     static_assert(!PAIR || (TN % 2 == 0 && !OUT8 && !DEQ), "interleaved n-tile pairs: bf16 output");
@@ -288,6 +290,10 @@
             uint8_t* dst = reinterpret_cast<uint8_t*>(g.c) + (int64_t)z * g.c_bs + (int64_t)(m0 + rsub) * g.c_ld + n;
             if (m0 + BM_ <= g.M) SlabCopy<0, NSW, RPS, PROW, false>::run(src, dst, g.c_ld, m0 + rsub, g.M);
             else SlabCopy<0, NSW, RPS, PROW, true>::run(src, dst, g.c_ld, m0 + rsub, g.M);
+        } else if constexpr (UPW > 0) {
+            static_assert(RPS == UPW && BM_ == UPW * UPW && NSAMP == 1 && !RES && !FIN, "up-fold epilogue: one UPW x UPW image per tile, one image row per sweep");
+            bf16* dst = reinterpret_cast<bf16*>(g.c) + ((int64_t)(m0 / BM_) * (4 * BM_) + (phase >> 1) * (2 * UPW) + (phase & 1) + 2 * rsub) * g.c_ld + n;
+            SlabCopy<0, NSW, RPS, PROW, false, 4 * UPW>::run(src, dst, g.c_ld, 0, 0);
         } else {
             bf16* dst = reinterpret_cast<bf16*>(g.c) + (int64_t)z * g.c_bs + (int64_t)(m0 + rsub) * g.c_ld + n;
             if (m0 + BM_ <= g.M) SlabCopy<0, NSW, RPS, PROW, false>::run(src, dst, g.c_ld, m0 + rsub, g.M);
@@ -306,7 +312,7 @@
                 float s = 0.f, qq = 0.f;
 #pragma unroll
                 for (int w = 0; w < WM; ++w) { s += sred[w * (BN_ / 4) + tid].x; qq += sred[w * (BN_ / 4) + tid].y; }
-                reinterpret_cast<float2*>(g.gn_part)[(int64_t)(m0 / BM_) * g.gn_quads + (n0 >> 2) + tid] = make_float2(s, qq);
+                reinterpret_cast<float2*>(g.gn_part)[(int64_t)(UPW > 0 ? (m0 / BM_) * 4 + phase : m0 / BM_) * g.gn_quads + (n0 >> 2) + tid] = make_float2(s, qq);
             }
         }
         if constexpr (FIN) {
@@ -654,17 +660,18 @@
     if constexpr (GUARD) stream_guard_commit(ga, g.stream_guard);
 }
 
-template <int WM, int WN, int TM, int TN, class Cfg, int EPI, int NSAMP = 1, bool FIN = false, bool PAIR = false>
+template <int WM, int WN, int TM, int TN, class Cfg, int EPI, int NSAMP = 1, bool FIN = false, bool PAIR = false, int UPW = 0>
 __device__ __forceinline__ void tile_epilogue(const GemmArgs& g, unsigned char* smem, f32x4 (&acc)[TM][TN],
                                               int m0, int n0, int z, int tid, int lane, int wm, int wn)
 {
+    static_assert(UPW == 0 || EPI == 1 || EPI == 2, "up-fold tiles: the plain packed epilogue, with or without GroupNorm partials");
     if constexpr (EPI == 0) dma_tile_epilogue<WM, WN, TM, TN, Cfg>(g, smem, acc, m0, n0, z, tid, lane, wm, wn);
     else if constexpr (EPI == 7) direct_f32_epilogue<WM, WN, TM, TN>(g, acc, m0, n0, z, lane, wm, wn);
     else if constexpr (EPI == 10) direct_f32_epilogue<WM, WN, TM, TN, false, 0, true>(g, acc, m0, n0, z, lane, wm, wn);
     else {
         static_assert(Cfg::PACK_OK, "packed epilogue needs the whole bf16 tile in LDS");
         NATINF_TS(2);
-        packed_tile_epilogue<WM, WN, TM, TN, Cfg, EPI == 3 ? ACT_SILU : (EPI == 4 ? ACT_GELU_TANH : ACT_NONE), EPI == 2 || EPI == 6, EPI == 5 || EPI == 6, EPI == 8, false, NSAMP, FIN && (EPI == 2 || EPI == 6), PAIR>(
+        packed_tile_epilogue<WM, WN, TM, TN, Cfg, EPI == 3 ? ACT_SILU : (EPI == 4 ? ACT_GELU_TANH : ACT_NONE), EPI == 2 || EPI == 6, EPI == 5 || EPI == 6, EPI == 8, false, NSAMP, FIN && (EPI == 2 || EPI == 6), PAIR, false, UPW>(
             g, smem, acc, m0, n0, z, tid, lane, wm, wn);
     }
 }
@@ -708,12 +715,14 @@
     }
 };
 
-template <int WM, int WN, int TM, int TN, int SPREAD = 0, int EPI = 0>
-__global__ __launch_bounds__(WM * WN * 64, 2) void k_gemm_dma(const GemmArgs g)
+template <int WM, int WN, int TM, int TN, int SPREAD, int EPI, int UPW>
+__device__ __forceinline__ void gemm_dma_tile(const GemmArgs& g)
 {
     static_assert(SPREAD == 2 || SPREAD == 6, "the shipped K loops: hand pipeline (2), one issuing wave per SIMD (6)");
     using Cfg = DmaCfg<WM, WN, TM, TN>;
     constexpr int BM_ = Cfg::BM_, BN_ = Cfg::BN_, THREADS = Cfg::THREADS;
+    constexpr bool UPF = UPW > 0;
+    static_assert(!UPF || BM_ == UPW * UPW, "up-fold: a tile is one low-resolution image");
     extern __shared__ __attribute__((aligned(16))) unsigned char smem[];
     lds_poison();
     const int tid = threadIdx.x, lane = tid & 63;
@@ -726,6 +735,7 @@
     tile_coords(tile, nM, nN, g.raster_g, mt_, nt_);
     const int m0 = mt_ * BM_, n0 = nt_ * BN_;
     const int z = blockIdx.z;
+    const int up_a = UPF ? (nt_ >> 1) & 1 : 0, up_b = UPF ? nt_ & 1 : 0;
 
     const bf16* a0 = g.a0 + (int64_t)z * g.a_bs;
     const bf16* a1 = g.a1 ? g.a1 + (int64_t)z * g.a_bs : nullptr;
@@ -739,14 +749,14 @@
     const bool issuer = !HALF || wave < Cfg::NW / 2;
     uint64_t a_row[PAI], a_delta[PAI], b_row[PBI];
     typedef __attribute__((address_space(3))) void lds_void;
-    const int64_t ashift0 = g.taps == 9 ? (int64_t)(-Wp - 1) * g.a0_ld * 2 : 0;
+    const int64_t ashift0 = UPF ? (int64_t)((up_a - 1) * Wp + up_b - 1) * g.a0_ld * 2 : (g.taps == 9 ? (int64_t)(-Wp - 1) * g.a0_ld * 2 : 0);
 #pragma unroll
     for (int j = 0; j < PAI; ++j) {
         const int r = (wave * PAI + j) * 8 + (lane >> 3);
         const int lchunk = ((lane & 7) ^ ((r >> 1) & 7)) << 3;
         const int m = min(m0 + r, g.M - 1);
         int64_t off0;
-        if (g.taps == 9) {
+        if (UPF || g.taps == 9) {
             const int b = m >> g.logHW, p = m & ((1 << g.logHW) - 1), y = p >> g.logW, x = p & ((1 << g.logW) - 1);
             off0 = ((int64_t)(b * Hp + y + 1) * Wp + x + 1) * g.a0_ld;
         } else {
@@ -787,8 +797,9 @@
         int64_t ashiftn; int kkn;
         if (seg0n) {
             int tap = 0, c0 = kn * BK;
-            if (g.taps == 9) { const int cch = kn / 9; tap = kn - 9 * cch; c0 = cch * BK; }
-            const int dy = g.taps == 9 ? tap / 3 - 1 : 0, dx = g.taps == 9 ? tap % 3 - 1 : 0;
+            if (UPF) { tap = kn & 3; c0 = (kn >> 2) * BK; }
+            else if (g.taps == 9) { const int cch = kn / 9; tap = kn - 9 * cch; c0 = cch * BK; }
+            const int dy = UPF ? up_a - 1 + (tap >> 1) : (g.taps == 9 ? tap / 3 - 1 : 0), dx = UPF ? up_b - 1 + (tap & 1) : (g.taps == 9 ? tap % 3 - 1 : 0);
             ashiftn = ((int64_t)(dy * Wp + dx) * g.a0_ld + c0) * 2; kkn = kn * BK;
         } else {
             ashiftn = (int64_t)(kn - nk0) * BK * 2; kkn = K0 + (kn - nk0) * BK;
@@ -825,8 +836,11 @@
         asm volatile("s_waitcnt vmcnt(0)" ::: "memory");
         __syncthreads();
     }
-    tile_epilogue<WM, WN, TM, TN, typename Cfg::Epi, EPI>(g, smem, acc, m0, n0, z, tid, lane, wm, wn);
-}
+    if constexpr (UPF) tile_epilogue<WM, WN, TM, TN, typename Cfg::Epi, EPI, 1, false, false, UPW>(g, smem, acc, m0, 0, 2 * up_a + up_b, tid, lane, wm, wn);
+    else tile_epilogue<WM, WN, TM, TN, typename Cfg::Epi, EPI>(g, smem, acc, m0, n0, z, tid, lane, wm, wn);
+}
+template <int WM, int WN, int TM, int TN, int SPREAD = 0, int EPI = 0>
+__global__ __launch_bounds__(WM * WN * 64, 2) void k_gemm_dma(const GemmArgs g) { gemm_dma_tile<WM, WN, TM, TN, SPREAD, EPI, 0>(g); }
 
 
 template <int WM, int WN, int TM, int TN, int NS>
diff --git a/naturaldiffusion_amd/csrc/gemm_launch.h b/naturaldiffusion_amd/csrc/gemm_launch.h
--- a/naturaldiffusion_amd/csrc/gemm_launch.h
+++ b/naturaldiffusion_amd/csrc/gemm_launch.h
@@ -23,6 +23,7 @@
 namespace ncsn_sg { bool configure(); bool has_tile(int variant); void launch_tile(const void* gemm_args, int variant, int raster, void* stream);
                     void launch_fp8(const void* gemm_args, int mxa, int w128, int raster, void* stream); void launch_splitk_reduce(const void* gemm_args, int slices, void* stream);
                     void launch_patch_embed(const float* z, const float* Wt, const float* bias, const float* pos, float* x, int C, int g, int D, int64_t rows, int x_f16, uint32_t* guard, void* stream); }
+namespace ncsn_upf { bool configure(); void launch(const void* gemm_args, int epi, void* stream); void fold(const float* w, void* dst_bf16, float* dst_f32, int N, int Cin, float wmul, void* stream); }
 namespace ncsn_cg3 { bool configure(); int tile_rows(int shape); int tile_cols(int shape); void launch(const void* gemm_args, int shape, int epi, void* stream); }
 
 namespace {
@@ -150,6 +151,8 @@
     ((S::takes(res, bm) && (launch_family<S>(e, g, s), true)) || ...);
 }
 
+constexpr int UPFOLD_W = 16, UPFOLD_BM = UPFOLD_W * UPFOLD_W, UPFOLD_BN = 256;
+
 constexpr unsigned EPI_FP8 = 0xF;
 template <bool MXA> struct FamF8     { using Cfg = CfgD256x256; static constexpr unsigned EPI = EPI_FP8; template <int E> static constexpr auto kernel() { return &k_gemm_fp8<MXA, E>; } };
 template <bool MXA> struct FamF8W128 { using Cfg = W128F8Cfg;   static constexpr unsigned EPI = EPI_FP8; template <int E> static constexpr auto kernel() { return &k_gemm_w128_fp8<MXA, E>; } };
@@ -159,7 +162,7 @@
     bool ok = hipFuncSetAttribute(reinterpret_cast<const void*>(&k_gemm_bf16), hipFuncAttributeMaxDynamicSharedMemorySize,
                                   GEMM_LDS_BYTES) == hipSuccess;
     ok = ok && set_lds<CfgR128x128>(&k_gemm_ring<2, 2, 4, 4, 4, 9>) && set_lds<W128Cfg>(&k_gemm_w128<9>) &&
-         configure_families(GemmFamilies{}) && configure_families(ConvGnShapes{}) && configure_families(Fp8Families{}) &&
+         configure_families(GemmFamilies{}) && configure_families(ConvGnShapes{}) && ncsn_upf::configure() && configure_families(Fp8Families{}) &&
          ncsn_cg3::configure() && ncsn_sg::configure() && ::configure_conv_ring() && configure_ncsnpp_kernels() && configure_dit_attention() && configure_flash_attention();
     if (!ok) (void)hipGetLastError();
     return ok;
@@ -335,7 +338,21 @@
     g_gemm_prof.end(r, s);
     return bm;
 }
+inline int up_fold_epi(const GemmArgs& g) {
+    if (g.taps != 4 || !g.a0_padded || g.a1 || g.gn_scale || g.batch != 1 || g.logW != 4 || g.logHW != 8 || g.log_rows_per_sample != 8 || g.a0_C <= 0 || g.a0_C % BK ||
+        g.N != 4 * UPFOLD_BN || g.M <= 0 || g.M % UPFOLD_BM || g.b_ld != 4 * g.a0_C || g.resid || g.c_ld % 8) return 0;
+    GemmArgs t = g; t.epi_fp32_slab = 0;
+    const int e = packed_epi(t, UPFOLD_BM);
+    return (e == 1 || e == 2) ? e : 0;
+}
 int launch_gemm_run(const GemmArgs& g0, hipStream_t s) {
+    if (g0.taps == 4) {
+        const int e = up_fold_epi(g0);
+        if (!e) { if (g_record) record_gemm(g0, "invalid_conv_gn_upfold", 0); else g_launch_error = 1; return 256; }
+        if (g_record) { record_gemm(g0, "conv_gn_upfold", e); return 256; }
+        ncsn_upf::launch(&g0, e, (void*)s);
+        return 256;
+    }
     if (g_force_variant == V_AUTO) {
         const int S8 = w128_splitk_slices(g0);
         if (S8 > 1) {
diff --git a/naturaldiffusion_amd/csrc/ncsnpp.hip b/naturaldiffusion_amd/csrc/ncsnpp.hip
--- a/naturaldiffusion_amd/csrc/ncsnpp.hip
+++ b/naturaldiffusion_amd/csrc/ncsnpp.hip
@@ -42,6 +42,8 @@
 int g_fuse_fin = 3;
 int g_fuse_gn4 = 1;
 int g_fuse_gn = 1;
+constexpr int UP_FOLD_DEFAULT = 1;
+int g_fuse_up_fold = UP_FOLD_DEFAULT;
 int g_fuse_up = 1;
 
 }
@@ -146,6 +148,11 @@
                                reinterpret_cast<bf16*>(p.packed + dst), N, ld, cin, c1);
         });
     }
+    void pack_fold_up(int64_t src, int64_t dst, int N, int Cin, float wmul) {
+        E.packs.push_back([=](const PackCtx& p) {
+            ncsn_upf::fold(p.params + src, p.packed + dst, nullptr, N, Cin, wmul, (void*)p.stream);
+        });
+    }
     void pack_transpose(int64_t src, int64_t dst, int K, int N, int dst_ld) {
         E.packs.push_back([=](const PackCtx& p) {
             hipLaunchKernelGGL(k_pack_transpose, dim3(grid1d((int64_t)K * N, 256, 1 << 30)), dim3(256), 0, p.stream,
@@ -201,11 +208,13 @@
         const bool fusable_res = g_fuse_gn && (ro == 32 || ro == 16 || (ro == 8 && g_fuse_gn8 && cout % 256 == 0) || (ro == 4 && g_fuse_gn4 && cout % 256 == 0));
         const bool fuse1 = fusable_res && cout % BK == 0;
         const bool fuse_up = fuse1 && ro > 8 && g_fuse_up && m.up && cin % BK == 0 && cout % 128 == 0;
-        const bool fuse = (fusable_res && !m.up && !m.down && cin % BK == 0) || fuse_up;
+        const bool fold_up = fuse_up && g_fuse_up_fold && !ddpm && ro == 2 * UPFOLD_W && cout == UPFOLD_BN;
+        const bool fuse = (fusable_res && !m.up && !m.down && cin % BK == 0) || (fuse_up && !fold_up);
         const float LOG2E = 1.4426950408889634f, LN2 = 0.6931471805599453f;
         const float gn_mul = fuse ? -LOG2E : 1.0f, w_mul = fuse ? -LN2 : 1.0f, gn_mul1 = fuse1 ? -LOG2E : 1.0f, w_mul1 = fuse1 ? -LN2 : 1.0f;
-        const int64_t w0 = wres((int64_t)cout * K0a * 2), w1 = wres((int64_t)cout * K1tot * 2);
-        pack_conv(p_c0w, w0, cout, cin, 9, K0a, 0, cin, w_mul);
+        const int64_t w0 = wres((int64_t)cout * (fold_up ? 16 * cin : K0a) * 2), w1 = wres((int64_t)cout * K1tot * 2);
+        if (fold_up) pack_fold_up(p_c0w, w0, cout, cin, w_mul);
+        else pack_conv(p_c0w, w0, cout, cin, 9, K0a, 0, cin, w_mul);
         pack_conv(p_c1w, w1, cout, cout, 9, K1tot, 0, cout, w_mul1);
         if (shortcut && !ddpm) pack_conv(p_c2w, w1, cout, cin, 1, K1tot, 9 * cout, cin);
         if (shortcut && ddpm) pack_transpose(p_c2w, w1 + (int64_t)9 * cout * 2, cin, cout, K1tot);
@@ -222,7 +231,10 @@
         int64_t sc = own_sc, sh = own_sh;
         emit_gn_stats(x, gn0, sc, sh, gn_mul);
         TRef h, xr;
-        if (!fuse) {
+        if (fold_up) {
+            h = new_act(m.res, cin, 1);
+            emit_gn_apply(x, sc, sh, h, nullptr, ACT_SILU, RS_NONE);
+        } else if (!fuse) {
             h = new_act(ro, cin, 1);
             if (m.up || m.down) xr = new_act(ro, cin);
             emit_gn_apply(x, sc, sh, h, (m.up || m.down) ? &xr : nullptr, ACT_SILU, m.up ? RS_UP : (m.down ? RS_DOWN : RS_NONE));
@@ -234,8 +246,18 @@
         const Part pt = register_output(t, fuse);
         const int logW = ilog2(ro), logHW = 2 * logW, HWo = ro * ro;
         const int dtotal = dense_total; const int64_t dout = dense_out;
-        op(fuse ? (ro <= 8 ? CLS_CONV_GN8 : CLS_CONV_GN) : CLS_GEMM, [=](const Ctx& c) {
+        op((fuse || fold_up) ? (ro <= 8 ? CLS_CONV_GN8 : CLS_CONV_GN) : CLS_GEMM, [=](const Ctx& c) {
             GemmArgs g = gemm_defaults();
+            if (fold_up) {
+                g.a0 = c.act(h); g.a0_ld = h.ld; g.a0_padded = 1; g.a0_C = cin; g.taps = 4; g.logW = logW - 1; g.logHW = logHW - 2;
+                g.M = c.B * (HWo / 4); g.N = 4 * cout; g.b = c.w<bf16>(w0); g.b_ld = 4 * cin; g.bias_n = c.w<float>(b0);
+                g.rowvec = c.at<float>(dout) + drow; g.rowvec_ld = dtotal; g.log_rows_per_sample = logHW - 2;
+                g.c = c.act(t); g.c_ld = t.ld;
+                if (pt.valid) { g.gn_part = c.at<float>(pt.off); g.gn_quads = pt.quads; }
+                const int bm = launch_gemm(g, c.stream);
+                if (pt.valid) c.part_bm[pt.id] = bm;
+                return;
+            }
             if (fuse) { g.a0 = c.act(x); g.a0_ld = x.ld; g.gn_scale = c.at<float>(sc); g.gn_shift = c.at<float>(sh); g.gn_ld = cin; g.gn_folded = 1; g.a0_up = fuse_up; }
             else { g.a0 = c.act(h); g.a0_ld = h.ld; g.a0_padded = 1; }
             g.a0_C = cin; g.taps = 9; g.logW = logW; g.logHW = logHW;
@@ -815,7 +837,10 @@
         int saved[sizeof(knobs) / sizeof(knobs[0])];
         for (size_t i = 0; i < sizeof(knobs) / sizeof(knobs[0]); ++i) { saved[i] = *knobs[i]; *knobs[i] = 1; }
         g_fuse_fin = 3;
+        const int saved_fold = g_fuse_up_fold;
+        g_fuse_up_fold = 0;
         natinf_ncsnpp* r = make_engine(0);
+        g_fuse_up_fold = saved_fold;
         for (size_t i = 0; i < sizeof(knobs) / sizeof(knobs[0]); ++i) *knobs[i] = saved[i];
         return r;
     }();
@@ -839,7 +864,7 @@
 
 static uint64_t plan_signature() {
     const int k[] = {g_fuse_head, g_attn_qkv, g_attn_w8, g_attn_proj, g_fuse_gn8, g_fuse_fin, g_fuse_gn4, g_fuse_gn, g_cg_wide, g_fuse_up,
-                     g_attn_blk , g_cg3 };
+                     g_attn_blk , g_fuse_up_fold, g_cg3 };
     uint64_t h = 1469598103934665603ull;
     for (int v : k) h = (h ^ (uint64_t)(v & 0xff)) * 1099511628211ull;
     return h;
@@ -1038,6 +1063,33 @@
     return hipGetLastError() == hipSuccess ? NATINF_OK : NATINF_ELAUNCH;
 }
 
+int natinf_debug_fold_up_weights(const float* w, int N, int cin, float w_mul, float* out_f32, void* out_packed, natinf_stream_t stream) {
+    if (!w || N <= 0 || cin <= 0 || (!out_f32 && !out_packed) || (out_packed && cin % 64)) return NATINF_EINVAL;
+    ncsn_upf::fold(w, out_packed, out_f32, N, cin, w_mul, stream);
+    return hipGetLastError() == hipSuccess ? NATINF_OK : NATINF_ELAUNCH;
+}
+int natinf_debug_conv_up_fold(int B, int N, int cin, const void* x, const float* scale, const float* shift, const float* w, void* w_packed, void* h_scratch,
+                              const float* bias_n, const float* rowvec, float out_scale, void* out, float* gn_part, int iters, natinf_stream_t stream) {
+    if (B <= 0 || N != UPFOLD_BN || cin <= 0 || cin % 64 || !x || !scale || !shift || !w || !w_packed || !h_scratch || !out || iters <= 0) return NATINF_EINVAL;
+    static bool configured = false;
+    if (!configured) { if (!configure_gemm_kernels()) return NATINF_ENODEV; configured = true; }
+    hipStream_t s = (hipStream_t)stream;
+    constexpr int W = UPFOLD_W, logW = 4;
+    ncsn_upf::fold(w, w_packed, nullptr, N, cin, 1.0f, stream);
+    hipLaunchKernelGGL(k_gn_apply, dim3((unsigned)((W + 2 + GN_ROWS - 1) / GN_ROWS), (unsigned)B), dim3(256), 0, s, (const bf16*)x, cin, cin, logW, 2 * logW, scale, shift,
+                       (bf16*)h_scratch, (bf16*)nullptr, ACT_SILU, RS_NONE, 1);
+    GemmArgs g = gemm_defaults();
+    g.a0 = (const bf16*)h_scratch; g.a0_ld = cin; g.a0_padded = 1; g.a0_C = cin; g.taps = 4; g.logW = logW; g.logHW = 2 * logW;
+    g.M = B * W * W; g.N = 4 * N; g.b = (const bf16*)w_packed; g.b_ld = 4 * cin; g.bias_n = bias_n;
+    g.rowvec = rowvec; g.rowvec_ld = N; g.log_rows_per_sample = 2 * logW; g.scale = out_scale;
+    g.c = out; g.c_ld = N; g.gn_part = gn_part; g.gn_quads = N / 4;
+    if (!up_fold_epi(g)) return NATINF_EINVAL;
+    g_launch_error = 0;
+    for (int i = 0; i < iters; ++i) launch_gemm(g, s);
+    if (g_launch_error) { g_launch_error = 0; return NATINF_EINVAL; }
+    return hipGetLastError() == hipSuccess ? NATINF_OK : NATINF_ELAUNCH;
+}
+
 int natinf_debug_attn_block(int plan, int B, const void* x, int x_ld, const float* scale, const float* shift, const float* w, const float* bias,
                             void* packed, void* scratch, void* out, int o_ld, float out_scale, float* gn_part, natinf_stream_t stream) {
     if (plan < 0 || plan > 2 || B < 1 || !x || !scale || !shift || !w || !bias || !packed || !out || x_ld < 256 || x_ld % 8 || o_ld < 256 || o_ld % 8 ||
@@ -1123,6 +1175,7 @@
 int natinf_set_conv_gn_wide(int mask) { if (mask < 0 || mask > 3) return NATINF_EINVAL; g_cg_wide = mask; return NATINF_OK; }
 int natinf_set_conv_gn_regw(int on) { return on ? NATINF_OK : NATINF_ESTATE; }
 int natinf_set_fuse_up(int on) { g_fuse_up = on != 0; return NATINF_OK; }
+int natinf_set_fuse_up_fold(int on) { g_fuse_up_fold = on < 0 ? UP_FOLD_DEFAULT : on != 0; return NATINF_OK; }
 int natinf_set_gemm_splitk(int on) { g_splitk = on != 0; return NATINF_OK; }
 int natinf_debug_set_splitk_workspace(float* ws, int max_slices) { g_dbg_splitk_ws = ws; g_dbg_splitk_max = ws ? max_slices : 0; return NATINF_OK; }
 int natinf_set_gemm_half_issue(int on) { return on ? NATINF_OK : NATINF_ESTATE; }
diff --git a/naturaldiffusion_amd/csrc/up_fold.h b/naturaldiffusion_amd/csrc/up_fold.h
--- /dev/null
+++ b/naturaldiffusion_amd/csrc/up_fold.h
@@ -0,0 +1,41 @@
+#pragma once
+#include "gemm_dma.h"
+
+namespace ncsn {
+
+__global__ void k_fold_up_conv(const float* __restrict__ src, bf16* __restrict__ dst, float* __restrict__ dst32, int N, int Cin, float wmul)
+{
+    const int64_t i = (int64_t)blockIdx.x * blockDim.x + threadIdx.x;
+    if (i >= (int64_t)N * Cin) return;
+    const int c = (int)(i % Cin), n = (int)(i / Cin);
+    float w[9];
+#pragma unroll
+    for (int t = 0; t < 9; ++t) w[t] = src[i * 9 + t];
+#pragma unroll
+    for (int a = 0; a < 2; ++a) {
+        float R[2][3];
+#pragma unroll
+        for (int kx = 0; kx < 3; ++kx) {
+            R[0][kx] = a == 0 ? w[kx] : w[kx] + w[3 + kx];
+            R[1][kx] = a == 0 ? w[3 + kx] + w[6 + kx] : w[6 + kx];
+        }
+#pragma unroll
+        for (int b = 0; b < 2; ++b)
+#pragma unroll
+            for (int ty = 0; ty < 2; ++ty)
+#pragma unroll
+                for (int tx = 0; tx < 2; ++tx) {
+                    const float f = b == 0 ? (tx == 0 ? R[ty][0] : R[ty][1] + R[ty][2]) : (tx == 0 ? R[ty][0] + R[ty][1] : R[ty][2]);
+                    const float v = f * wmul;
+                    const int ph = 2 * a + b;
+                    if (dst) dst[((int64_t)ph * N + n) * (4 * Cin) + ((c >> 6) * 4 + 2 * ty + tx) * 64 + (c & 63)] = (bf16)v;
+                    if (dst32) dst32[(((int64_t)ph * N + n) * Cin + c) * 4 + 2 * ty + tx] = v;
+                }
+    }
+}
+
+template <int EPI>
+__global__ __launch_bounds__(512, 2) void k_conv_gn_upfold(const GemmArgs g) { gemm_dma_tile<2, 4, 8, 4, 6, EPI, 16>(g); }
+using UpFoldCfg = DmaCfg<2, 4, 8, 4>;
+
+}
diff --git a/naturaldiffusion_amd/csrc/up_fold.hip b/naturaldiffusion_amd/csrc/up_fold.hip
--- /dev/null
+++ b/naturaldiffusion_amd/csrc/up_fold.hip
@@ -0,0 +1,28 @@
+#include <hip/hip_runtime.h>
+#include <stdint.h>
+#include <string.h>
+
+namespace {
+#include "up_fold.h"
+}
+using namespace ncsn;
+
+namespace ncsn_upf {
+__attribute__((visibility("hidden"))) bool configure() {
+    return hipFuncSetAttribute(reinterpret_cast<const void*>(&k_conv_gn_upfold<1>), hipFuncAttributeMaxDynamicSharedMemorySize, UpFoldCfg::LDS_BYTES) == hipSuccess &&
+           hipFuncSetAttribute(reinterpret_cast<const void*>(&k_conv_gn_upfold<2>), hipFuncAttributeMaxDynamicSharedMemorySize, UpFoldCfg::LDS_BYTES) == hipSuccess;
+}
+__attribute__((visibility("hidden"))) void launch(const void* gemm_args, int epi, void* stream) {
+    GemmArgs g;
+    memcpy(&g, gemm_args, sizeof(g));
+    g.raster_g = 0;
+    const dim3 grid((unsigned)((g.M / UpFoldCfg::BM_) * (g.N / UpFoldCfg::BN_)));
+    hipStream_t s = reinterpret_cast<hipStream_t>(stream);
+    if (epi == 2) hipLaunchKernelGGL((k_conv_gn_upfold<2>), grid, dim3(UpFoldCfg::THREADS), UpFoldCfg::LDS_BYTES, s, g);
+    else hipLaunchKernelGGL((k_conv_gn_upfold<1>), grid, dim3(UpFoldCfg::THREADS), UpFoldCfg::LDS_BYTES, s, g);
+}
+__attribute__((visibility("hidden"))) void fold(const float* w, void* dst_bf16, float* dst_f32, int N, int Cin, float wmul, void* stream) {
+    const int64_t n = (int64_t)N * Cin;
+    hipLaunchKernelGGL(k_fold_up_conv, dim3((unsigned)((n + 255) / 256)), dim3(256), 0, reinterpret_cast<hipStream_t>(stream), w, reinterpret_cast<bf16*>(dst_bf16), dst_f32, N, Cin, wmul);
+}
+}
```

Measured after the change: 3545 images/s (median of 6 runs). 1.8% higher.
